# thomasdeppisch/eMagLS

Measured on AMD Instinct MI355X. Metric: eMagLS filter sets/s (N=4, 2702 dirs, 512 taps), higher is better.
Workload: dtype f64; 1 GPU; BASELINE config 3: getEMagLsFilters em32 r=4.2cm N=4 complex-SH, 2702 dirs, 512 taps, 48 kHz; one filter set per step, inputs resident in HBM; dirs=2702, taps=512, sim_order=19, bins=512, k_cut=43, designs_resident_per_gpu=128, designs_per_batch=32, batches_in_flight=4, distinct_hrir_sets_resident=20, parallelism=independent jobs per GPU, one RCCL gather

## Files before the change

emagls_amd/_lib.py:

```python
from __future__ import annotations

import ctypes as C
import os

_HERE = os.path.dirname(os.path.abspath(__file__))
LIB_PATH = os.environ.get("EMAGLS_LIB_PATH") or os.path.join(_HERE, "lib", "libemagls.so")

OK, ERR_ARG, ERR_UNSUPPORTED, ERR_HIP, ERR_NUMERIC = 0, 1, 2, 3, 4
BASIS = {"real": 0, "complex": 1}
KIND_LS, KIND_MAGLS, KIND_EMAGLS, KIND_EMAGLS2, KIND_FROM_ATF, KIND_EMA_CH, KIND_MAGLS_2D, KIND_EMA_SH = range(8)
RADIAL = {"tikhonov": 0, "softlimit": 1, "full": 2, "none": 3}
LAYOUT = {"sh": 0, "ch": 1}
MODEL = {"sh": 0, "emagls": 1, "emagls2": 2, "atf": 3, "ema_ch": 5, "ema_sh": 6}

c_dp = C.POINTER(C.c_double)
c_i64 = C.c_int64


class DesignDesc(C.Structure):
    _fields_ = [("kind", C.c_int), ("basis", C.c_int), ("order", C.c_int), ("fs", C.c_double), ("len", c_i64),
                ("nsamp", c_i64), ("ndirs", c_i64), ("mic_radius", C.c_double), ("nmics", c_i64),
                ("f_trans", C.c_double), ("atf_taps", c_i64), ("natf", c_i64), ("custom_basis", C.c_int),
                ("diffuseness", C.c_int), ("sim_order_pad", C.c_int)]

# ... 31 lines not shown
    "emagls_version": (C.c_int, []),
    "emagls_device_count": (C.c_int, [C.POINTER(C.c_int)]),
    "emagls_set_device": (C.c_int, [C.c_int]),
    "emagls_cache_clear": (C.c_int, []),
    "emagls_cache_release_designs": (C.c_int, []),
    "emagls_fp64_peak_tflops": (C.c_int, [C.c_int, C.POINTER(C.c_double)]),
    "emagls_fp64_peak_tflops_ex": (C.c_int, [C.c_int, C.c_int, C.POINTER(C.c_double), C.POINTER(C.c_double)]),
    "emagls_self_test": (C.c_int, [C.c_int, C.POINTER(C.c_double)]),
    "emagls_debug_synth_operand": (C.c_int, [C.c_void_p, C.c_int, C.c_int, C.c_void_p, c_i64, C.c_int, C.c_void_p, C.c_void_p]),
    "emagls_debug_synth_cosines": (C.c_int, [C.c_void_p, C.c_void_p, c_i64, C.c_void_p, C.c_void_p, C.c_int, C.c_void_p]),
    "emagls_debug_factor": (C.c_int, [C.POINTER(DebugFactorArgs)]),
    "emagls_debug_factor_gram": (C.c_int, [C.c_void_p, C.c_int, C.c_int, C.c_void_p, C.c_int, C.c_double, C.c_double, C.c_void_p, C.c_void_p,
                                           C.c_void_p, C.c_void_p]),
    "emagls_debug_twiddles": (C.c_int, [C.c_int, C.c_void_p]),
    "emagls_debug_filter_epilogue": (C.c_int, [C.c_void_p, C.c_int, C.c_int, C.c_int, C.c_void_p, C.c_int, C.c_int, C.c_int, C.c_int, C.c_int,
                                               C.c_double, C.c_void_p, C.c_void_p]),
    "emagls_debug_hrir_spectra": (C.c_int, [C.c_void_p, C.c_void_p, c_i64, c_i64, c_i64, C.c_void_p, C.c_int, C.c_int, C.c_int, C.c_int, C.c_void_p,
                                            c_i64, C.c_int, C.c_void_p, C.c_void_p, C.c_void_p, C.c_void_p, C.c_void_p]),
    "emagls_debug_real_spectra": (C.c_int, [C.c_void_p, c_i64, c_i64, c_i64, C.c_void_p, C.c_int, c_i64, c_i64, c_i64, C.c_void_p]),
    "emagls_sh_basis": (C.c_int, [C.c_int, c_i64, C.c_void_p, C.c_void_p, C.c_int, C.c_void_p]),
    "emagls_sh_basis_device": (C.c_int, [C.c_int, c_i64, C.c_void_p, C.c_void_p, C.c_int, C.c_void_p, C.c_void_p]),
    "emagls_modal_bn": (C.c_int, [C.c_int, c_i64, C.c_void_p, C.c_void_p]),
    "emagls_get_ls_filters": (C.c_int, [C.c_void_p, C.c_void_p, c_i64, c_i64, C.c_void_p, C.c_void_p, C.c_int, C.c_int,
                                        C.c_void_p, C.c_void_p]),
    "emagls_get_magls_filters": (C.c_int, [C.c_void_p, C.c_void_p, c_i64, c_i64, C.c_void_p, C.c_void_p, C.c_int,
                                           C.c_double, c_i64, C.c_int, C.c_void_p, C.c_void_p]),
    "emagls_get_emagls_filters": (C.c_int, [C.c_void_p, C.c_void_p, c_i64, c_i64, C.c_void_p, C.c_void_p, C.c_double,
                                            C.c_void_p, C.c_void_p, c_i64, C.c_int, C.c_double, c_i64, C.c_int,
                                            C.c_void_p, C.c_void_p]),
    "emagls_get_emagls2_filters": (C.c_int, [C.c_void_p, C.c_void_p, c_i64, c_i64, C.c_void_p, C.c_void_p, C.c_double,
                                             C.c_void_p, C.c_void_p, c_i64, C.c_int, C.c_double, c_i64, C.c_int,
                                             C.c_void_p, C.c_void_p]),
    "emagls_get_emagls_filters_ema_in_ch": (C.c_int, [C.c_void_p, C.c_void_p, c_i64, c_i64, C.c_void_p, C.c_void_p, C.c_double,
                                                      C.c_void_p, c_i64, C.c_int, C.c_double, c_i64, C.c_int, C.c_void_p, C.c_void_p]),
    "emagls_get_emagls_filters_ema_in_sh": (C.c_int, [C.c_void_p, C.c_void_p, c_i64, c_i64, C.c_void_p, C.c_void_p, C.c_double,
                                                      C.c_void_p, c_i64, C.c_int, C.c_double, c_i64, C.c_int, C.c_void_p, C.c_void_p]),
    "emagls_get_emagls_filters_from_atf": (C.c_int, [C.c_void_p, C.c_void_p, c_i64, c_i64, C.c_void_p, C.c_void_p,
                                                     C.c_void_p, c_i64, c_i64, c_i64, C.c_void_p, C.c_void_p,
                                                     C.c_double, c_i64, C.c_double, C.c_void_p, C.c_void_p,
                                                     C.POINTER(C.c_double)]),
    "emagls_simulation_order": (C.c_int, [C.c_int, C.c_int, C.c_double, C.c_double]),
    "emagls_get_ls_filters_with_basis": (C.c_int, [C.c_void_p, C.c_void_p, c_i64, c_i64, C.c_void_p, C.c_int, C.c_int, C.c_void_p, C.c_void_p]),
    "emagls_get_magls_filters_with_basis": (C.c_int, [C.c_void_p, C.c_void_p, c_i64, c_i64, C.c_void_p, C.c_int, C.c_double, c_i64, C.c_int,
                                                      C.c_void_p, C.c_void_p]),
    "emagls_get_emagls_filters_with_basis": (C.c_int, [C.c_void_p, C.c_void_p, c_i64, c_i64, C.c_void_p, C.c_double, C.c_void_p, c_i64, C.c_int,
                                                       C.c_double, c_i64, C.c_int, C.c_void_p, C.c_void_p]),
    "emagls_get_emagls2_filters_with_basis": (C.c_int, [C.c_void_p, C.c_void_p, c_i64, c_i64, C.c_void_p, C.c_double, C.c_void_p, c_i64, C.c_int,
                                                        C.c_double, c_i64, C.c_int, C.c_void_p, C.c_void_p]),
    "emagls_plan_set_basis": (C.c_int, [C.c_void_p, C.c_void_p, C.c_void_p]),
    "emagls_binaural_decode": (C.c_int, [C.c_void_p, c_i64, c_i64, C.c_void_p, C.c_void_p, c_i64, C.c_int, C.c_void_p]),
    "emagls_binaural_decode_complex": (C.c_int, [C.c_void_p, C.c_int, c_i64, c_i64, C.c_void_p, C.c_void_p, C.c_int, c_i64, C.c_int,
                                                 C.c_void_p, C.c_void_p]),
    "emagls_binaural_decode_device": (C.c_int, [C.c_void_p, C.c_int, c_i64, c_i64, C.c_void_p, C.c_void_p, C.c_int, c_i64, C.c_void_p,
                                                C.c_void_p, C.c_void_p]),
    "emagls_rotate_yaw": (C.c_int, [C.c_void_p, C.c_int, c_i64, c_i64, C.c_int, C.c_int, C.c_void_p, c_i64, C.c_void_p]),
    "emagls_binaural_decode_render": (C.c_int, [C.c_void_p, C.c_int, c_i64, c_i64, C.c_void_p, C.c_void_p, C.c_int, c_i64, C.c_int,
                                                C.c_int, C.c_int, C.c_void_p, c_i64, C.c_void_p, c_i64, C.c_void_p, C.c_void_p]),
    "emagls_binaural_decode_render_device": (C.c_int, [C.c_void_p, C.c_int, c_i64, c_i64, C.c_void_p, C.c_void_p, C.c_int, c_i64,
                                                       C.c_int, C.c_int, C.c_void_p, c_i64, C.c_void_p, c_i64, C.c_void_p, C.c_void_p,
                                                       C.c_void_p]),
    "emagls_sh_rotation_matrix": (C.c_int, [C.c_int, C.c_int, C.c_double, C.c_double, C.c_double, C.c_void_p]),
    "emagls_rotate_sh": (C.c_int, [C.c_void_p, C.c_int, c_i64, c_i64, C.c_int, C.c_void_p, c_i64, C.c_void_p, c_i64, C.c_void_p, c_i64,
                                   C.c_void_p]),
    "emagls_binaural_decode_render_ypr": (C.c_int, [C.c_void_p, C.c_int, c_i64, c_i64, C.c_void_p, C.c_void_p, C.c_int, c_i64, C.c_int,
                                                    C.c_int, C.c_int, C.c_void_p, c_i64, C.c_void_p, c_i64, C.c_void_p, c_i64,
                                                    C.c_void_p, c_i64, C.c_void_p, C.c_void_p]),
    "emagls_binaural_decode_render_ypr_device": (C.c_int, [C.c_void_p, C.c_int, c_i64, c_i64, C.c_void_p, C.c_void_p, C.c_int, c_i64,
                                                           C.c_int, C.c_int, C.c_void_p, c_i64, C.c_void_p, c_i64, C.c_void_p, c_i64,
                                                           C.c_void_p, c_i64, C.c_void_p, C.c_void_p, C.c_void_p]),
    "emagls_resample_length": (c_i64, [c_i64, c_i64, c_i64]),
    "emagls_resample": (C.c_int, [C.c_void_p, C.c_int, c_i64, c_i64, c_i64, c_i64, C.c_void_p]),
    "emagls_resample_device": (C.c_int, [C.c_void_p, C.c_int, c_i64, c_i64, c_i64, c_i64, C.c_void_p, C.c_void_p]),
    "emagls_binaural_decode_render_fs": (C.c_int, [C.c_void_p, C.c_int, c_i64, c_i64, C.c_void_p, C.c_void_p, C.c_int, c_i64, C.c_int,
                                                   C.c_int, C.c_int, C.c_void_p, c_i64, C.c_void_p, c_i64, C.c_void_p, c_i64,
                                                   C.c_void_p, c_i64, C.c_double, C.c_double, C.c_double, C.c_void_p, C.c_void_p]),
    "emagls_binaural_decode_render_fs_device": (C.c_int, [C.c_void_p, C.c_int, c_i64, c_i64, C.c_void_p, C.c_void_p, C.c_int, c_i64,
                                                          C.c_int, C.c_int, C.c_void_p, c_i64, C.c_void_p, c_i64, C.c_void_p, c_i64,
                                                          C.c_void_p, c_i64, C.c_double, C.c_double, C.c_double, C.c_void_p,
                                                          C.c_void_p, C.c_void_p]),
    "emagls_decode_stream_create": (C.c_int, [c_i64, C.c_void_p, C.c_void_p, C.c_int, c_i64, C.c_int, C.c_int, C.c_int, c_i64,
                                              C.POINTER(C.c_void_p)]),
    "emagls_decode_stream_push": (C.c_int, [C.c_void_p, C.c_void_p, c_i64, C.c_void_p, c_i64, C.c_void_p, c_i64, C.c_void_p, c_i64,
                                            C.c_void_p]),
    "emagls_decode_stream_push_device": (C.c_int, [C.c_void_p, C.c_void_p, c_i64, C.c_void_p, c_i64, C.c_void_p, c_i64, C.c_void_p, c_i64,
                                                   C.c_void_p, C.c_void_p]),
    "emagls_decode_stream_reset": (C.c_int, [C.c_void_p]),
    "emagls_decode_stream_info": (C.c_int, [C.c_void_p, C.POINTER(c_i64), C.POINTER(c_i64), C.POINTER(c_i64), C.POINTER(c_i64),
                                            C.POINTER(C.c_int)]),
    "emagls_decode_stream_destroy": (C.c_int, [C.c_void_p]),
    "emagls_decode_stream_create_bank": (C.c_int, [c_i64, c_i64, C.c_void_p, C.c_void_p, C.c_int, c_i64, C.c_int, C.c_int, C.c_int, c_i64,
                                                   C.POINTER(C.c_void_p)]),
    "emagls_decode_stream_push_sets": (C.c_int, [C.c_void_p, C.c_void_p, c_i64, C.c_void_p, c_i64, C.c_void_p, c_i64, C.c_void_p, c_i64,
                                                 C.c_void_p, c_i64, C.c_void_p]),
    "emagls_decode_stream_push_sets_device": (C.c_int, [C.c_void_p, C.c_void_p, c_i64, C.c_void_p, c_i64, C.c_void_p, c_i64, C.c_void_p,
                                                        c_i64, C.c_void_p, c_i64, C.c_void_p, C.c_void_p]),
    "emagls_decode_stream_sets": (C.c_int, [C.c_void_p, C.POINTER(c_i64)]),
    "emagls_decode_group_create": (C.c_int, [c_i64, c_i64, C.c_void_p, C.c_void_p, C.c_int, c_i64, C.c_int, C.c_int, C.c_int, c_i64, c_i64,
                                             C.POINTER(C.c_void_p)]),
    "emagls_decode_group_push": (C.c_int, [C.c_void_p, C.c_void_p, c_i64, C.c_void_p, c_i64, C.c_void_p, c_i64, C.c_void_p, c_i64,
                                           C.c_void_p, c_i64, C.c_void_p]),
    "emagls_decode_group_push_device": (C.c_int, [C.c_void_p, C.c_void_p, c_i64, C.c_void_p, c_i64, C.c_void_p, c_i64, C.c_void_p, c_i64,
                                                  C.c_void_p, c_i64, C.c_void_p, C.c_void_p]),
    "emagls_decode_group_reset": (C.c_int, [C.c_void_p, c_i64]),
    "emagls_decode_group_info": (C.c_int, [C.c_void_p, C.POINTER(c_i64), C.POINTER(c_i64), C.POINTER(c_i64), C.POINTER(c_i64),
                                           C.POINTER(c_i64), C.POINTER(C.c_int)]),
    "emagls_decode_group_destroy": (C.c_int, [C.c_void_p]),
    "emagls_decode_stream_create_encoded": (C.c_int, [c_i64, C.c_void_p, C.c_int, c_i64, c_i64, C.c_void_p, C.c_void_p, C.c_int, c_i64, C.c_int,
                                                      C.c_int, c_i64, C.POINTER(C.c_void_p)]),
    "emagls_decode_group_create_encoded": (C.c_int, [c_i64, C.c_void_p, C.c_int, c_i64, c_i64, C.c_void_p, C.c_void_p, C.c_int, c_i64, C.c_int,
                                                     C.c_int, c_i64, c_i64, C.POINTER(C.c_void_p)]),
    "emagls_field_stream_create": (C.c_int, [c_i64, c_i64, C.c_void_p, C.c_int, c_i64, c_i64, C.POINTER(C.c_void_p)]),
    "emagls_field_stream_push": (C.c_int, [C.c_void_p, C.c_void_p, c_i64, C.c_void_p]),
    "emagls_field_stream_push_device": (C.c_int, [C.c_void_p, C.c_void_p, c_i64, C.c_void_p, C.c_void_p]),
    "emagls_field_stream_reset": (C.c_int, [C.c_void_p]),
    "emagls_field_stream_info": (C.c_int, [C.c_void_p, C.POINTER(c_i64), C.POINTER(c_i64), C.POINTER(c_i64), C.POINTER(c_i64),
                                           C.POINTER(C.c_int)]),
    "emagls_field_stream_destroy": (C.c_int, [C.c_void_p]),
    "emagls_get_magls_filters_dc": (C.c_int, [C.c_void_p, C.c_void_p, c_i64, c_i64, C.c_void_p, C.c_void_p, C.c_int,
                                              C.c_double, c_i64, C.c_int, C.c_int, C.c_void_p, C.c_void_p]),
    "emagls_get_emagls_filters_dc": (C.c_int, [C.c_void_p, C.c_void_p, c_i64, c_i64, C.c_void_p, C.c_void_p, C.c_double,
                                               C.c_void_p, C.c_void_p, c_i64, C.c_int, C.c_double, c_i64, C.c_int, C.c_int,
                                               C.c_void_p, C.c_void_p]),
    "emagls_get_emagls2_filters_dc": (C.c_int, [C.c_void_p, C.c_void_p, c_i64, c_i64, C.c_void_p, C.c_void_p, C.c_double,
                                                C.c_void_p, C.c_void_p, c_i64, C.c_int, C.c_double, c_i64, C.c_int, C.c_int,
                                                C.c_void_p, C.c_void_p]),
    "emagls_get_magls_filters_2d": (C.c_int, [C.c_void_p, C.c_void_p, c_i64, c_i64, C.c_void_p, C.c_int, C.c_double, c_i64, C.c_int,
                                              C.c_void_p, C.c_void_p]),
    "emagls_get_radial_filter": (C.c_int, [C.c_int, C.c_double, C.c_double, c_i64, C.c_int, C.c_int, C.c_double, C.c_double, C.c_void_p]),
    "emagls_apply_radial_filter_rows": (c_i64, [c_i64, c_i64, C.c_int]),
    "emagls_apply_radial_filter": (C.c_int, [C.c_void_p, c_i64, C.c_int, C.c_double, C.c_double, c_i64, C.c_int, C.c_int, C.c_double,
                                             C.c_double, C.c_void_p]),
    "emagls_sh_encode": (C.c_int, [C.c_void_p, c_i64, c_i64, C.c_void_p, C.c_void_p, C.c_int, C.c_int, C.c_void_p]),
    "emagls_ch_basis": (C.c_int, [C.c_int, c_i64, C.c_void_p, C.c_int, C.c_void_p]),
    "emagls_get_smair_matrix": (C.c_int, [C.c_int, C.c_double, c_i64, C.c_int, C.c_double, C.c_void_p, C.c_void_p, c_i64, C.c_int, C.c_int,
                                          C.c_int, C.c_double, C.c_double, C.c_void_p, C.POINTER(C.c_int)]),
    "emagls_rendered_hrtfs": (C.c_int, [C.c_int, C.c_void_p, C.c_void_p, C.c_int, c_i64, c_i64, c_i64, C.c_void_p, C.c_void_p, c_i64, C.c_double,
                                        C.c_int, C.c_int, C.c_double, C.c_void_p, C.c_void_p, c_i64, C.c_void_p, c_i64, c_i64, C.c_void_p,
                                        C.c_void_p, c_i64, c_i64, C.c_void_p, C.c_void_p, C.c_void_p, C.c_void_p, C.c_void_p, C.c_void_p]),
    "emagls_eq_filter_nfft": (c_i64, [c_i64]),
    "emagls_get_magls_spherical_head_filter": (C.c_int, [C.c_double, C.c_int, C.c_double, c_i64, C.c_void_p, C.c_void_p]),
    "emagls_get_magls_array_diffuse_filter": (C.c_int, [C.c_double, C.c_void_p, C.c_void_p, c_i64, C.c_int, C.c_double, c_i64, C.c_int,
                                                        C.c_void_p, C.c_void_p]),
    "emagls_plan_create": (C.c_int, [C.POINTER(DesignDesc), C.POINTER(C.c_void_p)]),
    "emagls_plan_destroy": (C.c_int, [C.c_void_p]),
    "emagls_plan_set_hrir_grid": (C.c_int, [C.c_void_p, C.c_void_p, C.c_void_p]),
    "emagls_plan_set_mic_grid": (C.c_int, [C.c_void_p, C.c_void_p, C.c_void_p]),
    "emagls_plan_set_hrirs": (C.c_int, [C.c_void_p, C.c_void_p, C.c_void_p]),
    "emagls_plan_set_atfs": (C.c_int, [C.c_void_p, C.c_void_p, C.c_void_p, C.c_void_p]),
    "emagls_plan_execute": (C.c_int, [C.c_void_p]),
    "emagls_plan_synchronize": (C.c_int, [C.c_void_p]),
    "emagls_plan_get_filters": (C.c_int, [C.c_void_p, C.c_void_p, C.c_void_p]),
    "emagls_plan_get_info": (C.c_int, [C.c_void_p, C.POINTER(PlanInfo)]),
    "emagls_plan_sweep_form_in_batch": (C.c_int, [C.c_void_p, C.c_int, C.POINTER(C.c_int)]),
    "emagls_plan_set_profiling": (C.c_int, [C.c_void_p, C.c_int]),
    "emagls_plan_set_streams": (C.c_int, [C.c_void_p, C.c_int]),
    "emagls_plan_num_stages": (C.c_int, [C.c_void_p]),
    "emagls_plan_stage_name": (C.c_char_p, [C.c_void_p, C.c_int]),
    "emagls_plan_stage_times": (C.c_int, [C.c_void_p, c_dp, C.c_int]),
    "emagls_plan_sweep_kernel_time": (C.c_int, [C.c_void_p, c_dp, C.POINTER(C.c_int)]),
    "emagls_plan_debug_buffer": (C.c_int, [C.c_void_p, C.c_char_p, C.c_void_p, C.POINTER(C.c_size_t)]),
    "emagls_plan_stream": (C.c_void_p, [C.c_void_p]),
    "emagls_batch_create": (C.c_int, [C.POINTER(C.c_void_p), C.c_int, C.POINTER(C.c_void_p)]),
    "emagls_batch_execute": (C.c_int, [C.c_void_p]),
    "emagls_batch_synchronize": (C.c_int, [C.c_void_p]),
    "emagls_batch_get_filters": (C.c_int, [C.c_void_p, C.POINTER(C.c_void_p), C.POINTER(C.c_void_p)]),
    "emagls_batch_set_profiling": (C.c_int, [C.c_void_p, C.c_int]),
    "emagls_batch_lane_mode": (C.c_int, [C.c_void_p, C.POINTER(C.c_int)]),
    "emagls_batch_set_stream": (C.c_int, [C.c_void_p, C.c_void_p]),
    "emagls_set_batch_max": (C.c_int, [C.c_int, C.POINTER(C.c_int)]),
    "emagls_batch_shares_atf_side": (C.c_int, [C.c_void_p, C.POINTER(C.c_int)]),
    "emagls_design_hrir_sets": (C.c_int, [C.c_int, C.c_void_p, C.c_void_p, C.c_int64, C.c_int64, C.c_int64, C.c_void_p, C.c_void_p, C.c_double,
                                          C.c_void_p, C.c_void_p, C.c_int64, C.c_int, C.c_double, C.c_int64, C.c_int, C.c_void_p, C.c_void_p]),
    "emagls_from_atf_hrir_sets": (C.c_int, [C.c_void_p, C.c_void_p, C.c_int64, C.c_int64, C.c_int64, C.c_void_p, C.c_void_p, C.c_void_p, C.c_int64,
                                            C.c_int64, C.c_int64, C.c_void_p, C.c_void_p, C.c_double, C.c_int64, C.c_double, C.c_void_p, C.c_void_p,
                                            C.POINTER(C.c_double)]),
    "emagls_jobs_run": (C.c_int, [C.POINTER(Job), C.c_int64, C.c_int, C.c_int, C.c_int]),
    "emagls_design_out_shape": (C.c_int, [C.POINTER(DesignDesc), C.POINTER(c_i64), C.POINTER(c_i64), C.POINTER(C.c_int)]),
    "emagls_jobs_shard": (C.c_int, [C.POINTER(Job), C.c_int64, C.c_int, C.c_int, C.POINTER(C.c_int), C.POINTER(C.c_int), C.POINTER(C.c_int)]),
    "emagls_jobs_run_devices": (C.c_int, [C.POINTER(Job), C.c_int64, C.POINTER(C.c_int), C.c_int, C.c_int, C.c_int, C.c_int]),
    "emagls_jobs_set_profiling": (C.c_int, [C.c_int]),
    "emagls_jobs_sweep_times": (C.c_int, [C.POINTER(C.c_double), C.POINTER(C.c_int), C.c_int, C.POINTER(C.c_int)]),
    "emagls_batch_set_geometry_sharing": (C.c_int, [C.c_void_p, C.c_int]),
    "emagls_batch_shares_geometry": (C.c_int, [C.c_void_p, C.POINTER(C.c_int)]),
    "emagls_batch_geometry_runs": (C.c_int, [C.c_void_p, C.POINTER(C.c_longlong), C.POINTER(C.c_longlong)]),
    "emagls_jobs_geometry_runs": (C.c_int, [C.POINTER(C.c_longlong), C.POINTER(C.c_longlong), C.POINTER(C.c_longlong)]),
    "emagls_jobs_would_share_geometry": (C.c_int, [C.c_void_p, C.c_int, C.POINTER(C.c_int)]),
    "emagls_batch_set_side_stream": (C.c_int, [C.c_void_p, C.c_void_p]),
    "emagls_batch_set_streams": (C.c_int, [C.c_void_p, C.c_int]),
    "emagls_batch_set_stage_order": (C.c_int, [C.c_void_p, C.c_int]),
    "emagls_batch_sweep_time": (C.c_int, [C.c_void_p, C.POINTER(C.c_double)]),
    "emagls_batch_destroy": (C.c_int, [C.c_void_p]),
}


class EmaglsError(RuntimeError):
    def __init__(self, code, msg):
        super().__init__("emagls error %d: %s" % (code, msg))
        self.code = code


_lib = None


def load():
    global _lib
    if _lib is not None:
        return _lib
    if not os.path.exists(LIB_PATH):
        raise ImportError("HIP library not built: %s is missing (run `python -m emagls_amd.build`)" % LIB_PATH)
    lib = C.CDLL(LIB_PATH, mode=C.RTLD_GLOBAL)
    for name, (res, args) in SYMBOLS.items():
        fn = getattr(lib, name)
        fn.restype = res
        fn.argtypes = args
    _lib = lib
    return lib


def check(rc):
    if rc != OK:
        raise EmaglsError(rc, load().emagls_last_error().decode("utf-8", "replace"))
```

emagls_amd/csrc/batch_run.hip:

```cpp
#include "host_internal.hpp"

void emagls_batch_forget(emagls_batch* b, emagls_plan* p) {
    for (auto& q : b->plans) if (q == p) q = nullptr;
}

namespace {
void batch_sweep_stage(emagls_batch& b) {
    const int nb = (int)b.plans.size();
    std::vector<HalfSweepArgs> ha((size_t)nb);
    for (int j = 0; j < nb; ++j) ha[j] = emagls_half_args(*b.plans[j]);
    if (b.atf_share || b.geo_share)
        for (int j = 1; j < nb; ++j) {
            ha[j].G = ha[0].G; ha[j].Yri = ha[0].Yri; ha[j].Mw = ha[0].Mw; ha[j].cond_ok = ha[0].cond_ok;
            ha[j].bsc = ha[0].bsc; ha[j].smap = ha[0].smap;
            ha[j].skip_flag = ha[0].skip_flag;
        }
    const bool reg = b.plans[0]->sweep_persist && reg_sweep_wanted(b.plans.data(), nb);
    for (auto* q : b.plans) q->reg_sweep = reg;
    if (!reg && nb > SWEEP_MULTI_MAX) throw Error(EMAGLS_ERR_UNSUPPORTED, "internal: more than 16 designs in a batch need the register-resident sweep");
    HalfSweepMulti h{};
    h.n = std::min(nb, SWEEP_MULTI_MAX);
    for (int j = 0; j < h.n; ++j) h.a[j] = ha[j];
    emagls_plan& q0 = *b.plans[0];
    const int kk0 = std::max(q0.kcut0, 1);
    if (kk0 >= q0.P) return;
    if (q0.sweep_persist) {
        hipStream_t ss = b.stream;
        {
            SweepGate gate(ss, reg ? reg_sweep_gate_cost((int)q0.D, nb) : 0);
            if (b.lanes) { BatchScope sc(nb, b.stride); launch_zero(q0.get("ll"), q0.bufs["ll"].bytes, ss); }
            else for (auto* q : b.plans) launch_zero(q->get("ll"), q->bufs["ll"].bytes, ss);
            if (reg) {
                if (!b.sweep_args_dev) HIP_CHECK(hipMalloc(&b.sweep_args_dev, sizeof(HalfSweepArgs) * (size_t)REG_SWEEP_MAX));
                reg_args_upload(ha.data(), nb, b.sweep_args_dev, b.sweep_args_last, ss);
            }
            if (b.prof_level >= 1) HIP_CHECK(hipEventRecord(b.sweep_ev[0], ss));
            if (reg) launch_sweep_reg(static_cast<const HalfSweepArgs*>(b.sweep_args_dev), ha[0], nb, ss);
            else if (q0.synth) launch_sweep_synth(h, ss); else launch_sweep_persist(h, ss);
            if (b.prof_level >= 1) HIP_CHECK(hipEventRecord(b.sweep_ev[1], ss));
        }
        if (ss != b.stream) b.depend(b.stream, ss);
        return;
    }
    for (int kb = kk0; kb < q0.P; ++kb) launch_sweep_half(h, kb, b.stream);
    launch_sweep_half_finalize(h, q0.P - 1, b.stream);
}

bool batch_defers_hh(const emagls_batch& b) {
    if (!b.lanes || !(b.alone || sw_int<Sw::DEFER_HH>() == 2) || b.geo_share || b.atf_share) return false;
    for (const emagls_plan* p : b.plans) if (!p || !plan_defers_hh_route(*p)) return false;
    return true;
}
void batch_lanes_part(emagls_batch& b, int part, int first, int count, hipStream_t st, int group = 0) {
    emagls_plan& p0 = *b.plans[first];
    const int ns = (part == 0 && b.groups == 1) ? b.nstreams : 1;
    int order = 0;
    if (part == 0 && ns == 1 && sw_on<Sw::STAGGER>()) order = b.groups > 1 ? 1 + group % 2 : (b.order_hint ? 1 + (b.order_hint - 1) % 2 : 0);
    Scoped stream(p0.stream, st);
    Scoped nstreams(p0.nstreams, ns);
    Scoped stage_order(p0.stage_order, order);
    Scoped side0(p0.side[0], ns > 1 ? b.side[0] : p0.side[0]), side1(p0.side[1], ns > 1 ? b.side[1] : p0.side[1]),
        side2(p0.side[2], ns > 1 ? b.side[2] : p0.side[2]);
    Scoped pre_phase(p0.pre_phase, part == 3 ? 2 : (part == 0 && b.defer_hh) ? 1 : 0);
    BatchScope sc(count, b.stride);
    if (part == 0) plan_pre_stage(p0); else if (part == 3) emagls_pre_sweep(p0); else emagls_post_sweep(p0);
}
void mark_executed(emagls_batch& b, int launches) {
    for (auto* p : b.plans) { p->executed = true; p->sweep_launches = launches; }
}
int sweep_launch_count(const emagls_plan& p0) { return p0.sweep_persist ? 1 : p0.P - std::max(p0.kcut0, 1); }
int batch_group_first(const emagls_batch& b, int g) { const int n = (int)b.plans.size(), h = (n + b.groups - 1) / b.groups; return std::min(n, g * h); }
void batch_execute_lanes(emagls_batch& b) {
    const bool replay = b.use_graph && b.eager_runs >= 1 && !(b.groups == 1 && b.nstreams > 1);
    const int n = (int)b.plans.size();
    const int ng = b.groups;
    for (int g = 1; g < ng; ++g) if (!b.side[g - 1]) b.side[g - 1] = emagls::pool_stream_take();
    hipStream_t gs[4] = {b.stream, b.stream, b.stream, b.stream};
    for (int g = 1; g < ng; ++g) gs[g] = b.side[g - 1];
    if (!replay || !b.group[0]) b.defer_hh = batch_defers_hh(b);
    const bool defer = b.defer_hh;
    if (defer) for (int g = 0; g < ng; ++g) if (!b.hh_stream[g]) b.hh_stream[g] = emagls::pool_stream_take();
    if (replay && !b.group[0]) {
        for (int g = 0; g < ng; ++g) {
            const int f = batch_group_first(b, g), c = batch_group_first(b, g + 1) - f;
            b.group[g].capture(gs[g], [&] { batch_lanes_part(b, 0, f, c, gs[g], g); });
            if (defer) b.group_hh[g].capture(b.hh_stream[g], [&] { batch_lanes_part(b, 3, f, c, b.hh_stream[g], g); });
        }
        b.post.capture(b.stream, [&] { batch_lanes_part(b, 2, 0, n, b.stream); });
    }
    b.used = 0;
    for (int g = 1; g < ng; ++g) b.depend(gs[g], b.stream);
    if (replay && ng > 1) {
        hipError_t err[4] = {hipSuccess, hipSuccess, hipSuccess, hipSuccess};
        const int dev = b.device;
        std::vector<std::thread> th;
        for (int g = 1; g < ng; ++g)
            th.emplace_back([&, g] { err[g] = hipSetDevice(dev); if (err[g] == hipSuccess) err[g] = hipGraphLaunch(b.group[g].exec, gs[g]); });
        err[0] = hipGraphLaunch(b.group[0].exec, gs[0]);
        for (auto& t : th) t.join();
        for (int g = 0; g < ng; ++g) HIP_CHECK(err[g]);
    } else {
        for (int g = 0; g < ng; ++g) {
            const int f = batch_group_first(b, g), c = batch_group_first(b, g + 1) - f;
            if (replay) b.group[g].launch(gs[g]); else batch_lanes_part(b, 0, f, c, gs[g], g);
        }
    }
    if (defer) for (int g = 0; g < ng; ++g) b.depend(b.hh_stream[g], gs[g]);
    for (int g = 1; g < ng; ++g) b.depend(b.stream, gs[g]);
    batch_sweep_stage(b);
    if (defer) {
        for (int g = 0; g < ng; ++g) {
            const int f = batch_group_first(b, g), c = batch_group_first(b, g + 1) - f;
            if (replay) b.group_hh[g].launch(b.hh_stream[g]); else batch_lanes_part(b, 3, f, c, b.hh_stream[g], g);
            b.depend(b.stream, b.hh_stream[g]);
        }
    }
    if (replay) b.post.launch(b.stream); else batch_lanes_part(b, 2, 0, n, b.stream);
    mark_executed(b, sweep_launch_count(*b.plans[0]));
    if (!replay) ++b.eager_runs;
}

bool batch_inputs_same(emagls_batch& b, std::initializer_list<const char*> names, uint64_t& checked_version, bool& same) {
    uint64_t ver = 0;
    for (auto* p : b.plans) ver = ver * 1000003ull + p->atf_side_version;
    if (ver == checked_version) return same;
    if (!b.cmp_flag) HIP_CHECK(hipMalloc(&b.cmp_flag, 16));
    HIP_CHECK(hipStreamSynchronize(b.stream));
    HIP_CHECK(hipMemsetAsync(b.cmp_flag, 0, 16, b.stream));
    emagls_plan& p0 = *b.plans[0];
    for (size_t j = 1; j < b.plans.size(); ++j)
        for (const char* name : names) launch_compare_words(p0.get(name), b.plans[j]->get(name), p0.bufs[name].bytes, b.cmp_flag, b.stream);
    int differ = 0;
    HIP_CHECK(hipMemcpyAsync(&differ, b.cmp_flag, sizeof differ, hipMemcpyDeviceToHost, b.stream));
    HIP_CHECK(hipStreamSynchronize(b.stream));
    checked_version = ver;
    return same = differ == 0;
}
void batch_set_sharing(emagls_batch& b, bool& field, bool share) {
    if (share == field) return;
    for (auto* p : b.plans) drop_plan_graphs(*p);
    drop_batch_graphs(b);
    if (&field == &b.geo_share) batch_geo_forget(b);
    field = share;
}
void batch_run_two_graphs(emagls_batch& b, CapturedGraph& pre, void (*stage)(emagls_batch&, int), int pre_part, int launches) {
    const bool replay = b.use_graph && b.eager_runs >= 1;
    if (replay && !pre) pre.capture(b.stream, [&] { stage(b, pre_part); });
    if (replay && !b.post) b.post.capture(b.stream, [&] { stage(b, 2); });
    b.used = 0;
    if (replay) pre.launch(b.stream); else stage(b, pre_part);
    batch_sweep_stage(b);
    if (replay) b.post.launch(b.stream); else stage(b, 2);
    mark_executed(b, launches);
    if (!replay) ++b.eager_runs;
}
template <typename Pre> void batch_run_per_plan(emagls_batch& b, bool replay, Pre pre, void (*post)(emagls_plan&), int launches) {
    emagls_plan& p0 = *b.plans[0];
    if (replay && !p0.pre) {
        for (auto* p : b.plans) p->pre.capture(p->stream, [&] { pre(*p); });
        if (!p0.sweep_persist) b.group[0].capture(b.stream, [&] { batch_sweep_stage(b); });
    }
    b.used = 0;
    for (auto* p : b.plans) b.depend(p->stream, b.stream);
    for (auto* p : b.plans) {
        if (replay) p->pre.launch(p->stream); else pre(*p);
        b.depend(b.stream, p->stream);
    }
    if (b.atf_share)
        for (size_t j = 1; j < b.plans.size(); ++j) from_atf_ls_rows(*b.plans[j], p0, b.stream);
    if (p0.sweep_persist) batch_sweep_stage(b);
    else if (replay) b.group[0].launch(b.stream); else batch_sweep_stage(b);
    for (auto* p : b.plans) {
        b.depend(p->stream, b.stream);
        post(*p);
        b.depend(b.stream, p->stream);
    }
    mark_executed(b, launches);
    if (!replay) ++b.eager_runs;
}

void batch_atf_decide_sharing(emagls_batch& b) {
    const bool same = batch_inputs_same(b, {"atf", "atf_azi", "atf_zen", "hrir_azi", "hrir_zen"}, b.atf_checked_version, b.atf_inputs_same);
    bool routes_ok = true;
    for (auto* p : b.plans) routes_ok = routes_ok && p->gram_from == 1 && p->sweep_persist == b.plans[0]->sweep_persist;
    batch_set_sharing(b, b.atf_share, same && routes_ok && b.plans.size() > 1);
}
void from_atf_subject_pre_stage(emagls_plan& p) {
    subject_reset(p, p.stream);
    from_atf_subject_stage(p);
}
// ... 424 lines not shown
```

emagls_amd/csrc/capi.hip:

```cpp
#include "host_internal.hpp"

namespace {

struct CachedPlan {
    std::unique_ptr<emagls_plan> plan;
    emagls_design_desc desc{};
    int device = 0;
    bool busy = false;
    uint64_t last_use = 0;
};
std::mutex g_cache_mu;
std::vector<CachedPlan> g_cache;
uint64_t g_cache_tick = 0;

int one_shot(const emagls_design_desc& desc, const double* hL, const double* hR, const double* azi, const double* zen,
             const double* mic_azi, const double* mic_zen, const double* atf, const double* atf_azi, const double* atf_zen,
             void* wL, void* wR, double* mean_dev, const void* Y_hrir = nullptr, const void* Y_mic = nullptr) {
    return guarded([&] {
        int dev = 0;
        HIP_CHECK(hipGetDevice(&dev));
        emagls_plan* p = nullptr;
        std::unique_ptr<emagls_plan> fresh;
        bool cached = false;
        {
// ... 213 lines not shown
int emagls_modal_bn(int order, int64_t nfreq, const double* kr, void* bn) {
    return guarded([&] {
        if (order < 0 || nfreq < 0 || !kr || !bn) throw Error(EMAGLS_ERR_ARG, "invalid argument");
        if (nfreq == 0) return;
        double* d_kr = nullptr;
        void* d_bn = nullptr;
        auto cleanup = [&] { hipFree(d_kr); hipFree(d_bn); };
        try {
            HIP_CHECK(hipMalloc(&d_kr, sizeof(double) * nfreq));
            HIP_CHECK(hipMalloc(&d_bn, sizeof(cplx) * nfreq * (order + 1)));
            HIP_CHECK(hipMemcpy(d_kr, kr, sizeof(double) * nfreq, hipMemcpyDefault));
            launch_modal_bn(order, nfreq, d_kr, 1.0, 1.0, d_bn, 1, nfreq, nullptr);
            HIP_CHECK(hipDeviceSynchronize());
            HIP_CHECK(hipMemcpy(bn, d_bn, sizeof(cplx) * nfreq * (order + 1), hipMemcpyDefault));
        } catch (...) { cleanup(); throw; }
        cleanup();
    });
}

int emagls_plan_create(const emagls_design_desc* desc, emagls_plan** plan) {
    return guarded([&] {
        if (!desc || !plan) throw Error(EMAGLS_ERR_ARG, "null pointer");
        std::unique_ptr<emagls_plan> p(new emagls_plan);
        p->d = *desc;
        plan_setup(*p);
        *plan = p.release();
    });
}
int emagls_plan_destroy(emagls_plan* plan) {
    return guarded([&] {
        DeviceGuard dg(plan ? plan->device : -1);
        delete plan;
    });
}
int emagls_plan_set_hrir_grid(emagls_plan* p, const double* azi, const double* zen) {
    return guarded([&] {
        DeviceGuard dg(p ? p->device : -1);
        if (!p || !azi) throw Error(EMAGLS_ERR_ARG, "null pointer");
        std::vector<double> equator;
        if (p->d.kind == EMAGLS_KIND_MAGLS_2D) { equator.assign((size_t)p->d.ndirs, kPi / 2.0); zen = equator.data(); }
        if (!zen) throw Error(EMAGLS_ERR_ARG, "null pointer");
        p->upload("hrir_azi", azi, sizeof(double) * p->d.ndirs);
        p->upload("hrir_zen", zen, sizeof(double) * p->d.ndirs);
        HIP_CHECK(hipStreamSynchronize(p->stream));
        p->have_hrir_grid = true;
        ++p->atf_side_version;
    });
}
int emagls_plan_set_mic_grid(emagls_plan* p, const double* azi, const double* zen) {
    return guarded([&] {
        DeviceGuard dg(p ? p->device : -1);
        if (!p || !azi) throw Error(EMAGLS_ERR_ARG, "null pointer");
        if (!p->has("mic_azi")) throw Error(EMAGLS_ERR_ARG, "this design kind has no microphone grid");
        std::vector<double> equator;
        if (p->d.kind == EMAGLS_KIND_EMA_CH || p->d.kind == EMAGLS_KIND_EMA_SH) { equator.assign((size_t)p->d.nmics, kPi / 2.0); zen = equator.data(); }
        if (!zen) throw Error(EMAGLS_ERR_ARG, "null pointer");
        p->upload("mic_azi", azi, sizeof(double) * p->d.nmics);
        p->upload("mic_zen", zen, sizeof(double) * p->d.nmics);
        if (p->has("smap")) {
            int smap[34];
            synth_pairing(azi, zen, (int)p->d.nmics, smap);
            p->upload("smap", smap, sizeof smap);
            p->synth_units = smap[32] + smap[33];
            HIP_CHECK(hipStreamSynchronize(p->stream));
        }
        std::vector<double> kr(p->P);
        for (int k = 0; k < p->P; ++k) {
            const double f = (double)k * (p->d.fs / 2.0) / (double)(p->P - 1);
            kr[k] = 2.0 * kPi * f / C_SOUND * p->d.mic_radius;
        }
        p->upload("kr", kr.data(), sizeof(double) * p->P);
        HIP_CHECK(hipStreamSynchronize(p->stream));
        p->have_mic_grid = true;
        ++p->atf_side_version;
    });
}
int emagls_plan_set_basis(emagls_plan* p, const void* Y_hrir, const void* Y_mic) {
    return guarded([&] {
        DeviceGuard dg(p ? p->device : -1);
        if (!p || !Y_hrir) throw Error(EMAGLS_ERR_ARG, "null pointer");
        if (!p->custom_basis) throw Error(EMAGLS_ERR_ARG, "the plan was not created with custom_basis = 1");
        const size_t es = esz(p->cplx_basis);
        HIP_CHECK(hipMemcpy2DAsync(p->get("Ycm"), (size_t)p->ldD * es, Y_hrir, (size_t)p->D * es, (size_t)p->D * es, (size_t)p->S, hipMemcpyDefault,
                                   p->stream));
        if (array_kind(p->d.kind)) {
            if (!Y_mic) throw Error(EMAGLS_ERR_ARG, "the array designs need the SH matrix of the microphone grid too");
            p->upload("Ymic_cm", Y_mic, es * (size_t)p->S * p->d.nmics);
            std::vector<double> kr(p->P);
            for (int k = 0; k < p->P; ++k) kr[k] = 2.0 * kPi * ((double)k * (p->d.fs / 2.0) / (double)(p->P - 1)) / C_SOUND * p->d.mic_radius;
            p->upload("kr", kr.data(), sizeof(double) * p->P);
        }
        HIP_CHECK(hipStreamSynchronize(p->stream));
        p->have_basis = true;
    });
}
int emagls_plan_set_hrirs(emagls_plan* p, const double* hL, const double* hR) {
    return guarded([&] {
        DeviceGuard dg(p ? p->device : -1);
        if (!p || !hL || !hR) throw Error(EMAGLS_ERR_ARG, "null pointer");
        p->upload("hL", hL, sizeof(double) * p->d.nsamp * p->d.ndirs);
        p->upload("hR", hR, sizeof(double) * p->d.nsamp * p->d.ndirs);
        HIP_CHECK(hipStreamSynchronize(p->stream));
        p->have_hrirs = true;
    });
}
int emagls_plan_set_atfs(emagls_plan* p, const double* atf, const double* azi, const double* zen) {
    return guarded([&] {
        DeviceGuard dg(p ? p->device : -1);
        if (!p || !atf || !azi || !zen) throw Error(EMAGLS_ERR_ARG, "null pointer");
        if (!p->has("atf")) throw Error(EMAGLS_ERR_ARG, "this design kind has no ATFs");
        p->upload("atf", atf, sizeof(double) * p->d.atf_taps * p->d.nmics * p->d.natf);
        p->upload("atf_azi", azi, sizeof(double) * p->d.natf);
        p->upload("atf_zen", zen, sizeof(double) * p->d.natf);
        HIP_CHECK(hipStreamSynchronize(p->stream));
        p->have_atfs = true;
        ++p->atf_side_version;
    });
}
int emagls_plan_execute(emagls_plan* p) {
    return guarded([&] {
        DeviceGuard dg(p ? p->device : -1);
        if (!p) throw Error(EMAGLS_ERR_ARG, "null pointer");
        plan_execute(*p);
    });
}
int emagls_plan_synchronize(emagls_plan* p) {
    return guarded([&] {
        DeviceGuard dg(p ? p->device : -1);
        if (!p) throw Error(EMAGLS_ERR_ARG, "null pointer");
        HIP_CHECK(hipStreamSynchronize(p->sync_stream ? p->sync_stream : p->stream));
    });
}
int emagls_plan_get_filters(emagls_plan* p, void* wL, void* wR) {
    return guarded([&] {
        DeviceGuard dg(p ? p->device : -1);
        if (!p || !wL || !wR) throw Error(EMAGLS_ERR_ARG, "null pointer");
        if (!p->executed) throw Error(EMAGLS_ERR_ARG, "plan has not been executed");
        HIP_CHECK(hipStreamSynchronize(p->sync_stream ? p->sync_stream : p->stream));
        plan_check_flags(*p);
        const size_t bytes = (p->out_cplx ? sizeof(cplx) : sizeof(double)) * (size_t)p->out_rows * p->out_cols;
        HIP_CHECK(hipMemcpy(wL, p->get("wL"), bytes, hipMemcpyDefault));
        HIP_CHECK(hipMemcpy(wR, p->get("wR"), bytes, hipMemcpyDefault));
    });
}
int emagls_plan_sweep_form_in_batch(emagls_plan* p, int designs, int* form) {
    return guarded([&] {
        DeviceGuard dg(p ? p->device : -1);
        if (!p || !form || designs < 1 || designs > REG_SWEEP_MAX) throw Error(EMAGLS_ERR_ARG, "emagls_plan_sweep_form_in_batch: null pointer or designs outside 1..32");
        std::vector<emagls_plan*> same((size_t)designs, p);
        const bool reg = p->synth && reg_sweep_wanted(same.data(), designs);
        *form = p->d.kind == EMAGLS_KIND_LS ? 0 : (p->synth ? (reg ? 3 : 2) : (p->sweep_persist ? 1 : 0));
    });
}
int emagls_plan_get_info(emagls_plan* p, emagls_plan_info* info) {
    return guarded([&] {
        DeviceGuard dg(p ? p->device : -1);
        if (!p || !info) throw Error(EMAGLS_ERR_ARG, "null pointer");
        std::memset(info, 0, sizeof *info);
        info->nfft = p->nfft; info->num_pos_freqs = p->P; info->k_cut = p->k_cut; info->sim_order = p->simOrder;
        info->num_sh_sim = p->S; info->num_channels = p->C; info->out_is_complex = p->out_cplx;
        info->out_rows = p->out_rows; info->out_cols = p->out_cols; info->num_sweep_launches = p->sweep_launches;
        info->device_bytes = p->total_bytes;
        info->gram_from = p->gram_from; info->hh_end = p->hh_end; info->hh_orders = p->n_h + 1; info->g_first = p->g0;
        info->sim_order_own = array_kind(p->d.kind) ? p->simOrderOwn : p->simOrder;
        bool reg = false;
        if (p->synth) {
            bool whole = p->owner != nullptr;
            if (whole) for (auto* q : p->owner->plans) whole = whole && q != nullptr;
            reg = whole ? reg_sweep_wanted(p->owner->plans.data(), (int)p->owner->plans.size()) : reg_sweep_wanted(&p, 1);
        }
        info->sweep_form = p->d.kind == EMAGLS_KIND_LS ? 0 : (p->synth ? (reg ? 3 : 2) : (p->sweep_persist ? 1 : 0));
        info->sweep_units = p->synth ? p->synth_units : 0;
        if (p->executed) {
            HIP_CHECK(hipStreamSynchronize(p->stream));
            double g[2];
            HIP_CHECK(hipMemcpy(g, p->get("grpd"), sizeof g, hipMemcpyDeviceToHost));
            info->grp_delay_l = g[0]; info->grp_delay_r = g[1];
            if (p->has("mean_dev")) HIP_CHECK(hipMemcpy(&info->mean_grid_dev_deg, p->get("mean_dev"), sizeof(double), hipMemcpyDeviceToHost));
        }
    });
}
int emagls_plan_set_profiling(emagls_plan* p, int level) {
    return guarded([&] {
        DeviceGuard dg(p ? p->device : -1);
        if (!p) throw Error(EMAGLS_ERR_ARG, "null pointer");
        p->prof_level = level;
    });
}
int emagls_plan_set_streams(emagls_plan* p, int nstreams) {
    return guarded([&] {
        DeviceGuard dg(p ? p->device : -1);
        if (!p) throw Error(EMAGLS_ERR_ARG, "null pointer");
        if (nstreams < 1 || nstreams > 4) throw Error(EMAGLS_ERR_ARG, "nstreams must be 1..4");
        HIP_CHECK(hipStreamSynchronize(p->stream));
        drop_plan_graphs(*p);
        p->nstreams = nstreams;
    });
}
int emagls_plan_num_stages(emagls_plan* p) { return p ? (int)p->stage_names.size() : 0; }
const char* emagls_plan_stage_name(emagls_plan* p, int i) {
    if (!p || i < 0 || i >= (int)p->stage_names.size()) return "";
    return p->stage_names[i].c_str();
}
int emagls_plan_stage_times(emagls_plan* p, double* ms, int n) {
    return guarded([&] {
        DeviceGuard dg(p ? p->device : -1);
        if (!p || !ms) throw Error(EMAGLS_ERR_ARG, "null pointer");
        HIP_CHECK(hipStreamSynchronize(p->stream));
        const int ns = (int)p->stage_names.size();
        for (int i = 0; i < n; ++i) {
            ms[i] = 0.0;
            if (i >= 1 && i < ns) {
                float t = 0.f;
                HIP_CHECK(hipEventElapsedTime(&t, p->stage_events[i - 1], p->stage_events[i]));
                ms[i] = t;
            }
        }
    });
}
int emagls_plan_sweep_kernel_time(emagls_plan* p, double* total_ms, int* launches) {
    return guarded([&] {
        DeviceGuard dg(p ? p->device : -1);
        if (!p || !total_ms || !launches) throw Error(EMAGLS_ERR_ARG, "null pointer");
        HIP_CHECK(hipStreamSynchronize(p->stream));
        double tot = 0.0;
        int n = 0;
        if (p->prof_level >= 2) {
            for (int i = 0; i < p->sweep_launches && 2 * (size_t)i + 1 < p->sweep_events.size(); ++i) {
                float t = 0.f;
                HIP_CHECK(hipEventElapsedTime(&t, p->sweep_events[2 * i], p->sweep_events[2 * i + 1]));
                tot += t;
                ++n;
            }
        }
        *total_ms = tot;
        *launches = n;
    });
}
int emagls_plan_debug_buffer(emagls_plan* p, const char* name, void* dst, size_t* nbytes) {
    return guarded([&] {
        DeviceGuard dg(p ? p->device : -1);
        if (!p || !name || !nbytes) throw Error(EMAGLS_ERR_ARG, "null pointer");
        auto it = p->bufs.find(name);
        if (it == p->bufs.end()) throw Error(EMAGLS_ERR_ARG, std::string("unknown buffer ") + name);
        if (!dst) { *nbytes = it->second.bytes; return; }
        HIP_CHECK(hipStreamSynchronize(p->stream));
        const size_t n = std::min(*nbytes, it->second.bytes);
        HIP_CHECK(hipMemcpy(dst, it->second.p, n, hipMemcpyDeviceToHost));
        *nbytes = n;
    });
}
void* emagls_plan_stream(emagls_plan* p) { return p ? (void*)p->stream : nullptr; }

int emagls_batch_create(emagls_plan** plans, int nplans, emagls_batch** batch) {
    return guarded([&] {
        if (!plans || !batch || nplans < 1) throw Error(EMAGLS_ERR_ARG, "invalid argument");
        const int batch_max = std::max(g_batch_max.load(), g_batch_max_override);
        if (nplans > batch_max)
            throw Error(EMAGLS_ERR_UNSUPPORTED, batch_max >= REG_SWEEP_MAX ? "at most 32 designs per batch"
                                                                             : "at most 8 designs per batch (emagls_set_batch_max(16) / EMAGLS_BATCH_MAX=16 allows 16)");
        std::unique_ptr<emagls_batch> b(new emagls_batch);
        for (int j = 0; j < nplans; ++j) {
            emagls_plan* p = plans[j];
            if (!p) throw Error(EMAGLS_ERR_ARG, "null plan");
            if (!array_kind(p->d.kind) && p->d.kind != EMAGLS_KIND_FROM_ATF && !magls_kind(p->d.kind) && p->d.kind != EMAGLS_KIND_LS)
                throw Error(EMAGLS_ERR_UNSUPPORTED, "batches take eMagLS / eMagLS2 / EMAinCH / EMAinSH plans, LS / MagLS / MagLS-2D plans, or FromAtf plans "
                                                    "(subjects of one ATF set)");
            if ((p->d.kind == EMAGLS_KIND_LS) != (plans[0]->d.kind == EMAGLS_KIND_LS) ||
                (p->d.kind == EMAGLS_KIND_LS && (p->cplx_basis != plans[0]->cplx_basis || p->d.order != plans[0]->d.order || p->d.nsamp != plans[0]->d.nsamp)))
                throw Error(EMAGLS_ERR_ARG, "LS plans share a batch only with LS plans of the same order, basis and HRIR length");
            if ((p->d.kind == EMAGLS_KIND_FROM_ATF) != (plans[0]->d.kind == EMAGLS_KIND_FROM_ATF))
                throw Error(EMAGLS_ERR_ARG, "FromAtf plans cannot share a batch with array designs");
            if (magls_kind(p->d.kind) != magls_kind(plans[0]->d.kind) || (magls_kind(p->d.kind) && p->d.kind != plans[0]->d.kind))
                throw Error(EMAGLS_ERR_ARG, "MagLS plans share a batch only with MagLS plans of the same kind");
            if (magls_kind(p->d.kind) && (p->diffuse != plans[0]->diffuse || p->cplx_basis != plans[0]->cplx_basis || p->d.order != plans[0]->d.order))
                throw Error(EMAGLS_ERR_ARG, "all designs of a batch must have the same shape (order, basis, constraint)");
            if (p->wide) throw Error(EMAGLS_ERR_UNSUPPORTED, "designs with more than 32 channels run one at a time");
            if (p->owner) throw Error(EMAGLS_ERR_ARG, "a plan belongs to another batch (destroy that batch first)");
            if (p->device != plans[0]->device) throw Error(EMAGLS_ERR_ARG, "the plans of a batch must live on one device");
            for (int i = 0; i < j; ++i) if (plans[i] == p) throw Error(EMAGLS_ERR_ARG, "the same plan appears twice in the batch");
            const emagls_plan* q = plans[0];
            if (p->P != q->P || p->kcut0 != q->kcut0 || p->C != q->C || p->nWG_dense != q->nWG_dense || p->D != q->D || p->sweep_persist != q->sweep_persist ||
                p->Dm != q->Dm || p->d.natf != q->d.natf || p->d.atf_taps != q->d.atf_taps || p->d.len != q->d.len)
                throw Error(EMAGLS_ERR_ARG, "all designs of a batch must have the same shape (directions, channels, bins, k_cut)");
            b->plans.push_back(p);
        }
        b->device = b->plans[0]->device;
        DeviceGuard dg(b->device);
        b->stream = StreamPool::get().take();
        b->use_graph = !sw_on<Sw::NO_GRAPH>();
        const bool array_batch = b->plans[0]->d.kind != EMAGLS_KIND_FROM_ATF && !magls_kind(b->plans[0]->d.kind) && b->plans[0]->d.kind != EMAGLS_KIND_LS;
        for (auto* p : b->plans) HIP_CHECK(hipStreamSynchronize(p->stream));
        trace_mark("batch create: plans synchronised");
        if (array_batch) batch_unify_synth(*b);
        trace_mark("batch create: sweep form unified");
        batch_decide_residency(*b);
        trace_mark("batch create: residency decided");
        if (nplans > SWEEP_MULTI_MAX && !(b->plans[0]->synth && b->plans[0]->sweep_persist && reg_sweep_wanted(b->plans.data(), nplans)))
            throw Error(EMAGLS_ERR_UNSUPPORTED, "more than 16 designs per batch: only array designs that take the register-resident sweep (built-in SH basis, "
                                                "microphone grids set, at most 18 antipodal pairs + single microphones, a launch the device can hold)");
        for (auto* p : b->plans) {
            p->nstreams = 1;
            p->prof_level = 0;
            p->sync_stream = b->stream;
            p->owner = b.get();
        }
// ... 338 lines not shown
```

emagls_amd/csrc/host_internal.hpp:

```cpp
#pragma once
#include <atomic>
#include <chrono>
#include <cstdlib>
#include <cstring>
#include <deque>
#include <map>
#include <memory>
#include <mutex>
#include <shared_mutex>
#include <string>
#include <thread>
#include <utility>
#include <vector>

#include "../../include/emagls.h"
#include "kernels.hpp"

using namespace emagls;

struct emagls_batch;
void emagls_batch_forget(emagls_batch* b, emagls_plan* p);

namespace emagls {

// ... 203 lines not shown
    int64_t out_rows = 0, out_cols = 0;
    int nWG = 0, nWG_dense = 0;
    bool gram_route = true;
    int gram_from = 0, gram_floor = 0, hh_end = 0, n_h = 0, S_h = 0, ldS_h = 0, g0 = 0, nb_gram = 0;
    int nh_floor = 0;
    bool persist_suspended = false;
    bool sweep_persist = true;
    bool synth_want = false, synth = false;
    int synth_units = 0;
    bool reg_sweep = false;
    std::vector<char> sweep_args_last;
    bool synth_block = false;
    const emagls_plan* geo_from = nullptr;
    emagls_batch* owner = nullptr;
    bool have_hrir_grid = false, have_mic_grid = false, have_hrirs = false, have_atfs = false, have_basis = false;
    uint64_t atf_side_version = 0;
    bool diffuse = false;
    bool custom_basis = false;
    bool wide = false;
    int prof_level = 0;
    std::vector<std::string> stage_names;
    std::vector<hipEvent_t> stage_events;
    std::vector<double> stage_ms;
    std::vector<hipEvent_t> sweep_events;
    int sweep_launches = 0;
    bool executed = false;
    CapturedGraph graph;
    int eager_runs = 0;
    bool use_graph = true;
    CapturedGraph pre;
    int nstreams = 1;
    int stage_order = 0;
    int pre_phase = 0;
    bool geo_keep = false;
    bool geo_skip = false;
    uint64_t geo_done_version = ~0ull;
    uint64_t geo_run_version = ~0ull;
    uint64_t solo_runs = 0;
    bool defer_hh = false;
    bool alone = false;
    hipStream_t hh_stream = nullptr;
    hipStream_t sync_stream = nullptr;
    hipStream_t side[3] = {nullptr, nullptr, nullptr};
    bool owns_stream = true;
    void need_sides(int n) { for (int i = 0; i < n - 1 && i < 3; ++i) if (!side[i]) side[i] = StreamPool::get().take(); }
    std::vector<hipEvent_t> sync_events;
    size_t sync_used = 0;
    hipEvent_t next_sync_event() {
        if (sync_used == sync_events.size()) {
            hipEvent_t e;
            HIP_CHECK(hipEventCreateWithFlags(&e, hipEventDisableTiming));
            sync_events.push_back(e);
        }
        return sync_events[sync_used++];
    }
    void depend(hipStream_t waiter, hipStream_t signaller) {
        if (waiter == signaller) return;
        hipEvent_t e = next_sync_event();
        HIP_CHECK(hipEventRecord(e, signaller));
        HIP_CHECK(hipStreamWaitEvent(waiter, e, 0));
    }

    ~emagls_plan() {
        if (owner) emagls_batch_forget(owner, this);
        if (stream) hipStreamSynchronize(stream);
        for (auto st : side) if (st) hipStreamSynchronize(st);
        if (hh_stream) hipStreamSynchronize(hh_stream);
        (void)hipGetLastError();
        for (auto& kv : bufs) if (kv.second.p && kv.second.owned) hipFree(kv.second.p);
        release_slabs();
        for (auto e : stage_events) hipEventDestroy(e);
        for (auto e : sweep_events) hipEventDestroy(e);
        for (auto e : sync_events) hipEventDestroy(e);
        for (auto st : side) StreamPool::get().give(st);
        StreamPool::get().give(hh_stream);
        if (owns_stream) StreamPool::get().give(stream);
    }
    void* alloc(const std::string& name, size_t bytes, bool zero = true) {
        if (bytes == 0) bytes = 16;
        auto it = bufs.find(name);
        if (it != bufs.end()) {
            if (it->second.bytes >= bytes) {
                total_bytes -= (int64_t)(it->second.bytes - bytes);
                it->second.bytes = bytes;
                return it->second.p;
            }
            if (it->second.owned) HIP_CHECK(hipFree(it->second.p));
            total_bytes -= (int64_t)it->second.bytes;
        }
        DevBuf b;
        b.p = slab_take((bytes + 15) / 16 * 16);
        b.bytes = bytes;
        b.owned = false;
        if (zero && !slab_zeroed) HIP_CHECK(hipMemsetAsync(b.p, 0, bytes, stream));
        bufs[name] = b;
        total_bytes += (int64_t)bytes;
        return b.p;
    }
    template <typename T = void> T* get(const std::string& name) {
        auto it = bufs.find(name);
        if (it == bufs.end()) throw Error(EMAGLS_ERR_ARG, "internal: unknown buffer " + name);
        return reinterpret_cast<T*>(it->second.p);
    }
    bool has(const std::string& name) const { return bufs.count(name) != 0; }
    void upload(const std::string& name, const void* src, size_t bytes) {
        auto it = bufs.find(name);
        if (it == bufs.end() || it->second.bytes < bytes) throw Error(EMAGLS_ERR_ARG, "internal: upload size mismatch for " + name);
        HIP_CHECK(hipMemcpyAsync(it->second.p, src, bytes, hipMemcpyDefault, stream));
    }
    void mark(const char* name) {
        if (prof_level < 1) return;
        const size_t i = stage_names.size();
        stage_names.push_back(name);
        if (stage_events.size() <= i) {
            hipEvent_t e;
            HIP_CHECK(hipEventCreate(&e));
            stage_events.push_back(e);
        }
        HIP_CHECK(hipEventRecord(stage_events[i], stream));
    }
};

struct emagls_batch {
    std::vector<emagls_plan*> plans;
    int device = -1;
    bool lanes = false;
    size_t stride = 0;
    hipStream_t stream = nullptr;
    bool own_stream = true;
    bool atf = false, atf_share = false, atf_inputs_same = false;
    uint64_t atf_checked_version = ~0ull;
    bool magls = false;
    bool geo_want = false, geo_share = false, geo_inputs_same = false;
    uint64_t geo_checked_version = ~0ull;
    uint64_t geo_kept_version = ~0ull;
    uint64_t geo_ran_version = ~0ull;
    bool geo_cold_pending = false;
    CapturedGraph warm;
    int last_form = 0;
    long long geo_cold_runs = 0, geo_warm_runs = 0;
    int* cmp_flag = nullptr;
    int nstreams = 1;
    hipStream_t side[3] = {nullptr, nullptr, nullptr};
    CapturedGraph group[4];
    int prof_level = 0;
    hipEvent_t sweep_ev[2] = {nullptr, nullptr};
    CapturedGraph post;
    bool side0_external = false;
    int order_hint = 0;
    int groups = 1;
    CapturedGraph group_hh[4];
    hipStream_t hh_stream[4] = {nullptr, nullptr, nullptr, nullptr};
    bool defer_hh = false;
    bool alone = true;
    int eager_runs = 0;
    bool use_graph = true;
    void* sweep_args_dev = nullptr;
    std::vector<char> sweep_args_last;
    std::vector<hipEvent_t> events;
    size_t used = 0;
    hipEvent_t next_event() {
        if (used == events.size()) {
            hipEvent_t e;
            HIP_CHECK(hipEventCreateWithFlags(&e, hipEventDisableTiming));
            events.push_back(e);
        }
        return events[used++];
    }
    void depend(hipStream_t waiter, hipStream_t signaller) {
        hipEvent_t e = next_event();
        HIP_CHECK(hipEventRecord(e, signaller));
        HIP_CHECK(hipStreamWaitEvent(waiter, e, 0));
    }
    ~emagls_batch() {
        if (stream) hipStreamSynchronize(stream);
        for (auto e : events) hipEventDestroy(e);
        for (int i = 0; i < 4; ++i)
            if (hh_stream[i]) { hipStreamSynchronize(hh_stream[i]); emagls::pool_stream_give(hh_stream[i]); }
        for (auto e : sweep_ev) if (e) hipEventDestroy(e);
        if (stream && own_stream) emagls::pool_stream_give(stream);
        for (int i = 0; i < 3; ++i) if (side[i] && !(i == 0 && side0_external)) { hipStreamSynchronize(side[i]); emagls::pool_stream_give(side[i]); }
        if (cmp_flag) hipFree(cmp_flag);
        if (sweep_args_dev) hipFree(sweep_args_dev);
        for (auto* p : plans) if (p) { p->sync_stream = nullptr; p->owner = nullptr; }
    }
};

namespace emagls {

struct StreamLoan {
    const std::vector<emagls_plan*>& plans;
    std::vector<hipStream_t> keep;
    StreamLoan(const std::vector<emagls_plan*>& ps, hipStream_t st) : plans(ps) {
        keep.reserve(ps.size());
        for (auto* p : ps) { keep.push_back(p->stream); p->stream = st; }
    }
    StreamLoan(const StreamLoan&) = delete;
    StreamLoan& operator=(const StreamLoan&) = delete;
    ~StreamLoan() { for (size_t j = 0; j < keep.size(); ++j) plans[j]->stream = keep[j]; }
};

template <typename F> int guarded(F&& f) {
    return guarded_call([&] { f(); });
}

constexpr double GRAM_COND_EST = 3.0e3;

inline bool forks_streams(const emagls_plan& p) { return p.nstreams >= 2; }

extern thread_local hipStream_t g_plan_stream_shared;
void plan_routes(emagls_plan& p);
void synth_pairing(const double* azi, const double* zen, int M, int* smap);
void plan_alloc_routes(emagls_plan& p);
void plan_setup(emagls_plan& p);

void stage_prologue(emagls_plan& p, int mode, const int64_t* didx, int64_t Dh);
void execute_ls(emagls_plan& p);
void magls_post_sweep(emagls_plan& p);
bool plan_defers_hh_route(const emagls_plan& p);
void hrir_spectra(emagls_plan& h, const emagls_plan& g, hipStream_t st);
FactorArgs hh_factor_args(emagls_plan& h, emagls_plan& g, int* sweeps_out, double* cond_ok);
void hrir_hh_rows(emagls_plan& h, emagls_plan& g, hipStream_t st);
void hrir_hh_back(const FactorArgs& fa, const emagls_plan& g, hipStream_t st);
void hrir_gram_ls_rows(emagls_plan& h, emagls_plan& g, const emagls_plan& src, bool lanes_share, hipStream_t st);
void subject_reset(emagls_plan& p, hipStream_t st);
void emagls_pre_sweep(emagls_plan& p);
HalfSweepArgs emagls_half_args(emagls_plan& p);
struct SweepGate {
    struct Entry { hipEvent_t ev; int slots; };
    struct State { std::deque<Entry> inflight; std::vector<hipEvent_t> pool; int capacity = 0; };
    static std::mutex& mutex();
    static State& state();
    std::unique_lock<std::mutex> lock;
    hipStream_t st;
    int slots;
    SweepGate(hipStream_t s, int slots_per_xcd);
    ~SweepGate();
};
bool reg_sweep_wanted(emagls_plan* const* plans, int n);
void reg_args_upload(const HalfSweepArgs* host, int n, void* dev, std::vector<char>& last, hipStream_t st);
void emagls_post_sweep(emagls_plan& p);
void from_atf_subject_stage(emagls_plan& p);
void from_atf_ls_rows(emagls_plan& p, emagls_plan& sh, hipStream_t st);
void from_atf_post_sweep(emagls_plan& p);
void plan_pre_stage(emagls_plan& p);
void plan_execute(emagls_plan& p);
void drop_plan_graphs(emagls_plan& p);
bool plan_recover(emagls_plan& p, const int* flag, bool apply);
void throw_fatal_flags(const int* flag);

void batch_geo_forget(emagls_batch& b);
bool batch_geo_next_is_warm(const emagls_batch& b);
void batch_execute(emagls_batch& b);
void drop_batch_graphs(emagls_batch& b);
void batch_unify_synth(emagls_batch& b);
void batch_decide_residency(emagls_batch& b);
void batch_try_lanes(emagls_batch& b);
void batch_redo(emagls_batch& b, const std::vector<int>& flags);
void plan_check_flags(emagls_plan& p);

bool same_desc(const emagls_design_desc& a, const emagls_design_desc& b);
extern thread_local int g_batch_max_override;

}
```

emagls_amd/csrc/jobs.hip:

```cpp
#include "host_internal.hpp"

extern "C" {

namespace {
struct SetsCache {
    emagls_design_desc desc{};
    int device = -1, n = 0;
    std::vector<emagls_plan*> plans;
    emagls_batch* batch = nullptr;
    std::vector<double> grid[4];
    void release() {
        for (auto& g : grid) g.clear();
        if (batch) { emagls_batch_destroy(batch); batch = nullptr; }
        for (auto* p : plans) emagls_plan_destroy(p);
        plans.clear();
        n = 0; device = -1;
    }
};
std::mutex g_sets_mu;
SetsCache g_sets[3];
}
void emagls_sets_cache_clear_internal() {
    std::lock_guard<std::mutex> lk(g_sets_mu);
    for (auto& c : g_sets) c.release();
// ... 18 lines not shown
        Pending pend[3];
        size_t out_bytes = 0;
        auto collect = [&](Pending& q) {
            if (!q.c) return;
            SetsCache* c = q.c;
            q.c = nullptr;
            const int n = c->n;
            if (n == 1 || !c->batch) {
                for (int j = 0; j < n; ++j)
                    req(emagls_plan_get_filters(c->plans[(size_t)j], (char*)wL + (q.first + j) * out_bytes, (char*)wR + (q.first + j) * out_bytes));
            } else {
                std::vector<void*> pl((size_t)n), pr((size_t)n);
                for (int j = 0; j < n; ++j) { pl[(size_t)j] = (char*)wL + (q.first + j) * out_bytes; pr[(size_t)j] = (char*)wR + (q.first + j) * out_bytes; }
                req(emagls_batch_get_filters(c->batch, pl.data(), pr.data()));
            }
        };
        try {
            int64_t k = 0;
            for (int64_t first = 0; first < nsets; ++k) {
                const bool wide_kind = ((kind == EMAGLS_KIND_MAGLS_2D || kind == EMAGLS_KIND_EMA_CH) ? 2 * order + 1 : kind == EMAGLS_KIND_EMAGLS2 ? (int)nmics : (order + 1) * (order + 1)) > 32;
                const int chunk_max = wide_kind ? ((kind == EMAGLS_KIND_EMAGLS || kind == EMAGLS_KIND_EMAGLS2) ? 1 : 4) : kind == EMAGLS_KIND_EMA_SH ? 4 : SWEEP_MULTI_MAX;
                const int n = (int)std::min<int64_t>(chunk_max, nsets - first);
                const int slot = n == chunk_max ? (int)(k % 2) : 2;
                SetsCache* c = &g_sets[slot];
                collect(pend[slot]);
                if (!(c->n == n && c->device == dev && same_desc(c->desc, d))) {
                    c->release();
                    try {
                        for (int j = 0; j < n; ++j) {
                            emagls_plan* p = nullptr;
                            req(emagls_plan_create(&d, &p));
                            p->geo_keep = true;
                            c->plans.push_back(p);
                        }
                        if (n > 1 && !c->plans[0]->wide && kind != EMAGLS_KIND_EMA_SH) {
                            int r;
                            { Scoped limit(g_batch_max_override, SWEEP_MULTI_MAX); r = emagls_batch_create(c->plans.data(), n, &c->batch); }
                            req(r);
                            req(emagls_batch_set_geometry_sharing(c->batch, 1));
                        }
                    } catch (...) { c->release(); throw; }
                    c->desc = d; c->device = dev; c->n = n;
                }
                auto same = [](const std::vector<double>& have, const double* now, size_t cnt) {
                    return now ? (have.size() == cnt && std::memcmp(have.data(), now, cnt * sizeof(double)) == 0) : have.empty();
                };
                const bool hgrid_same = same(c->grid[0], hrir_azi, (size_t)ndirs) && same(c->grid[1], hrir_zen, (size_t)ndirs) && !c->grid[0].empty();
                const bool mgrid_same = !arr || (same(c->grid[2], mic_azi, (size_t)nmics) && same(c->grid[3], mic_zen, (size_t)nmics) && !c->grid[2].empty());
                for (int j = 0; j < n; ++j) {
                    emagls_plan* p = c->plans[(size_t)j];
                    if (!hgrid_same) req(emagls_plan_set_hrir_grid(p, hrir_azi, hrir_zen));
                    if (arr && !mgrid_same) req(emagls_plan_set_mic_grid(p, mic_azi, mic_zen));
                    req(emagls_plan_set_hrirs(p, hL + (first + j) * nsamp * ndirs, hR + (first + j) * nsamp * ndirs));
                }
                auto keep = [](std::vector<double>& dst, const double* src, size_t cnt) { if (src) dst.assign(src, src + cnt); else dst.clear(); };
                keep(c->grid[0], hrir_azi, (size_t)ndirs); keep(c->grid[1], hrir_zen, (size_t)ndirs);
                if (arr) { keep(c->grid[2], mic_azi, (size_t)nmics); keep(c->grid[3], mic_zen, (size_t)nmics); }
                emagls_plan_info info;
                req(emagls_plan_get_info(c->plans[0], &info));
                out_bytes = (info.out_is_complex ? sizeof(cplx) : sizeof(double)) * (size_t)info.out_rows * info.out_cols;
                if (n > 1 && c->batch) req(emagls_batch_execute(c->batch));
                else for (int j = 0; j < n; ++j) req(emagls_plan_execute(c->plans[(size_t)j]));
                pend[slot].c = c;
                pend[slot].first = first;
                first += n;
            }
            for (auto& q : pend) collect(q);
        } catch (...) {
            for (auto& c : g_sets) c.release();
            throw;
        }
    });
}

namespace {
std::mutex g_atfsets_mu;
SetsCache g_atfsets[2];
}
void emagls_atfsets_cache_clear_internal() {
    std::lock_guard<std::mutex> lk(g_atfsets_mu);
    for (auto& c : g_atfsets) c.release();
}

namespace {
struct JobSlot {
    std::string key;
    std::string shape;
    int device = -1;
    std::vector<emagls_plan*> plans;
    emagls_batch* batch = nullptr;
    std::vector<std::vector<double>> grids;
    uint64_t last_use = 0, last_call = 0;
    int runs = 0;
    hipStream_t stream = nullptr;
    ~JobSlot() {
        if (batch) emagls_batch_destroy(batch);
        for (auto* p : plans) emagls_plan_destroy(p);
        if (stream) emagls::pool_stream_give(stream);
    }
};
std::mutex g_jobs_mu;
std::vector<std::unique_ptr<JobSlot>> g_jobs_free;
std::atomic<int> g_jobs_prof{0};
std::shared_timed_mutex g_jobs_warm_mu;
uint64_t g_jobs_tick = 0;
std::atomic<size_t> g_jobs_resident_max{8 * REG_SWEEP_MAX};

void check_rc(int rc) { if (rc != EMAGLS_OK) throw Error(rc, g_last_error); }
bool is_device_pointer(const void* p) {
    hipPointerAttribute_t at{};
    if (!p || hipPointerGetAttributes(&at, p) != hipSuccess) { (void)hipGetLastError(); return false; }
    return at.type == hipMemoryTypeDevice;
}
void job_shape(const emagls_design_desc& d, std::string& out) {
    emagls_design_desc k = d;
    if (array_kind(d.kind) && d.sim_order_pad > 0) {
        const int own = std::max(d.kind == EMAGLS_KIND_EMAGLS2 ? SMAIR_DEFAULT_ORDER : d.order, (int)std::ceil(d.fs * kPi * d.mic_radius / C_SOUND));
        if (own <= d.sim_order_pad) k.mic_radius = 0.0;
    }
    out.assign(reinterpret_cast<const char*>(&k), sizeof k);
}
bool slot_will_capture(const JobSlot& s) {
    if (s.batch) {
        const emagls_batch& b = *s.batch;
        if (!b.use_graph || b.eager_runs < 1) return false;
        if (b.geo_share && !b.atf && !b.magls) return !b.post || !(batch_geo_next_is_warm(b) ? b.warm : b.group[0]);
        return !b.group[0] && !(b.plans.size() && b.plans[0]->pre);
    }
    for (const emagls_plan* p : s.plans)
        if (p->use_graph && p->prof_level == 0 && p->eager_runs >= 1 && !p->pre && !p->graph) return true;
    return false;
}
std::atomic<long long> g_jobs_geo_runs[3];
bool jobs_chunk_shares_geometry(const emagls_job* jobs, int n) {
    if (!jobs || n < 2) return false;
    const emagls_design_desc& d0 = jobs[0].desc;
    if (d0.kind != EMAGLS_KIND_EMAGLS && d0.kind != EMAGLS_KIND_EMAGLS2 && d0.kind != EMAGLS_KIND_EMA_CH) return false;
    if (d0.custom_basis || d0.diffuseness || d0.ndirs <= 0 || d0.nmics <= 0) return false;
    const int64_t ch = d0.kind == EMAGLS_KIND_EMAGLS2 ? d0.nmics : d0.kind == EMAGLS_KIND_EMA_CH ? 2 * (int64_t)d0.order + 1 : (int64_t)(d0.order + 1) * (d0.order + 1);
    if (ch > 32) return false;
    auto same = [](const double* a, const double* b, int64_t m) {
        if (a == b) return true;
        return a && b && memcmp(a, b, sizeof(double) * (size_t)m) == 0;
    };
    if (!jobs[0].hrir_azi || !jobs[0].mic_azi) return false;
    for (int j = 1; j < n; ++j) {
        const emagls_job& x = jobs[j];
        if (memcmp(&x.desc, &d0, sizeof d0) != 0) return false;
        if (!same(x.hrir_azi, jobs[0].hrir_azi, d0.ndirs) || !same(x.hrir_zen, jobs[0].hrir_zen, d0.ndirs) ||
            !same(x.mic_azi, jobs[0].mic_azi, d0.nmics) || !same(x.mic_zen, jobs[0].mic_zen, d0.nmics)) return false;
    }
    return true;
}
void jobs_run_chunk(const emagls_job* jobs, int n, int device, int flags, bool solo, uint64_t call) {
    DeviceGuard dg(device);
    const bool trace = sw_on<Sw::JOBS_TRACE>();
    const auto t_begin = std::chrono::steady_clock::now();
    auto lap = [&](const char* what) {
        if (trace) fprintf(stderr, "emagls jobs: chunk of %d, %s at %.3f ms\n", n, what,
                           std::chrono::duration<double, std::milli>(std::chrono::steady_clock::now() - t_begin).count());
    };
    std::string key(solo ? "S" : "P"), shape(solo ? "S" : "P"), one;
    for (int j = 0; j < n; ++j) {
        key.append(reinterpret_cast<const char*>(&jobs[j].desc), sizeof(emagls_design_desc));
        job_shape(jobs[j].desc, one);
        shape.append(one);
    }
    std::unique_ptr<JobSlot> slot, recycled;
    {
        std::lock_guard<std::mutex> lk(g_jobs_mu);
        for (size_t i = 0; i < g_jobs_free.size(); ++i)
            if (g_jobs_free[i]->device == device && g_jobs_free[i]->key == key) { slot = std::move(g_jobs_free[i]); g_jobs_free.erase(g_jobs_free.begin() + i); break; }
        if (!slot)
            for (size_t i = 0; i < g_jobs_free.size(); ++i)
                if (g_jobs_free[i]->device == device && g_jobs_free[i]->shape == shape && g_jobs_free[i]->last_call != call) {
                    recycled = std::move(g_jobs_free[i]); g_jobs_free.erase(g_jobs_free.begin() + i); break;
                }
    }
    recycled.reset();
    const bool was_resident = slot != nullptr;
    std::shared_lock<std::shared_timed_mutex> shared(g_jobs_warm_mu, std::defer_lock);
    std::unique_lock<std::shared_timed_mutex> alone(g_jobs_warm_mu, std::defer_lock);
    shared.lock();
    if (!slot) {
        slot.reset(new JobSlot);
        slot->key = key; slot->shape = shape; slot->device = device;
        slot->grids.resize((size_t)n);
        slot->stream = emagls::pool_stream_take();
        struct SharedStream { SharedStream(hipStream_t st) { g_plan_stream_shared = st; } ~SharedStream() { g_plan_stream_shared = nullptr; } } shared_stream(slot->stream);
        for (int j = 0; j < n; ++j) {
            emagls_plan* p = nullptr;
            check_rc(emagls_plan_create(&jobs[j].desc, &p));
            slot->plans.push_back(p);
            if (j == 0) lap("first plan created");
        }
        lap("plans created");
    }
    for (int j = 0; j < n; ++j) {
        const emagls_job& jb = jobs[j];
        emagls_plan* p = slot->plans[(size_t)j];
        const emagls_design_desc& d = jb.desc;
        std::vector<double> g;
        auto app = [&](const double* a, int64_t m) { if (a) g.insert(g.end(), a, a + m); else g.push_back(-1e300); };
        const bool has_mics = array_kind(d.kind);
        app(jb.hrir_azi, d.ndirs); app(jb.hrir_zen, d.ndirs);
        if (has_mics) { app(jb.mic_azi, d.nmics); app(jb.mic_zen, d.nmics); }
        if (g != slot->grids[(size_t)j]) {
            if (!jb.hrir_azi) throw Error(EMAGLS_ERR_ARG, "job without an HRIR grid");
            check_rc(emagls_plan_set_hrir_grid(p, jb.hrir_azi, jb.hrir_zen));
            if (has_mics) {
                if (!jb.mic_azi) throw Error(EMAGLS_ERR_ARG, "array design without a microphone grid");
                check_rc(emagls_plan_set_mic_grid(p, jb.mic_azi, jb.mic_zen));
            }
            slot->grids[(size_t)j] = std::move(g);
        }
        if (d.kind == EMAGLS_KIND_FROM_ATF) {
            if (!jb.atf || !jb.atf_azi || !jb.atf_zen) throw Error(EMAGLS_ERR_ARG, "FromAtf job without its ATF set");
            check_rc(emagls_plan_set_atfs(p, jb.atf, jb.atf_azi, jb.atf_zen));
        }
        if (!jb.hL || !jb.hR || !jb.wL || !jb.wR) throw Error(EMAGLS_ERR_ARG, "job without HRIRs or without room for its filters");
        if (!slot->batch && n > 1 && !slot->runs) check_rc(emagls_plan_set_hrirs(p, jb.hL, jb.hR));
    }
    lap("inputs set");
    if (n > 1 && !slot->batch && !slot->runs) {
        int rc;
        { Scoped limit(g_batch_max_override, REG_SWEEP_MAX); rc = emagls_batch_create(slot->plans.data(), n, &slot->batch); }
        if (rc != EMAGLS_OK && rc != EMAGLS_ERR_UNSUPPORTED) check_rc(rc);
        if (rc != EMAGLS_OK) slot->batch = nullptr;
        if (slot->batch && solo && slot->batch->lanes) {
            if (const int fork = sw_int<Sw::JOBS_FORK>(); fork >= 2) {
                if (slot->batch->groups != 1) { HIP_CHECK(hipStreamSynchronize(slot->batch->stream)); drop_batch_graphs(*slot->batch); slot->batch->groups = 1; }
                check_rc(emagls_batch_set_streams(slot->batch, fork));
            }
        }
        if (slot->batch) {
            slot->batch->alone = solo;
            if (!solo && slot->batch->group[0]) { HIP_CHECK(hipStreamSynchronize(slot->batch->stream)); drop_batch_graphs(*slot->batch); }
        }
        lap("batch created");
    } else if (slot->batch) {
        bool gathered = false;
        if (2 * n <= 64) {
            bool all_dev = true;
            for (int j = 0; j < n && all_dev; ++j) all_dev = is_device_pointer(jobs[j].hL) && is_device_pointer(jobs[j].hR);
            if (all_dev) {
                LanePtrs src{}, dst{};
                const emagls_plan& q0 = *slot->plans[0];
                const size_t bytes = sizeof(double) * (size_t)q0.d.nsamp * (size_t)q0.d.ndirs;
                for (int j = 0; j < n; ++j) {
                    emagls_plan& q = *slot->plans[(size_t)j];
                    src.p[2 * j] = const_cast<double*>(jobs[j].hL); src.p[2 * j + 1] = const_cast<double*>(jobs[j].hR);
                    dst.p[2 * j] = q.get("hL"); dst.p[2 * j + 1] = q.get("hR");
                    q.have_hrirs = true;
                }
                launch_gather_buffers(src, dst, 2 * n, bytes, slot->batch->stream);
                gathered = true;
            }
        }
        for (int j = 0; j < n && !gathered; ++j) {
            emagls_plan& q = *slot->plans[(size_t)j];
            const size_t bytes = sizeof(double) * (size_t)q.d.nsamp * (size_t)q.d.ndirs;
            int src = -1;
            for (int i = 0; i < j && src < 0; ++i)
                if (jobs[i].hL == jobs[j].hL && jobs[i].hR == jobs[j].hR && slot->plans[(size_t)i]->d.nsamp == q.d.nsamp && slot->plans[(size_t)i]->d.ndirs == q.d.ndirs) src = i;
            const void* sl = src >= 0 ? slot->plans[(size_t)src]->get("hL") : jobs[j].hL;
            const void* sr = src >= 0 ? slot->plans[(size_t)src]->get("hR") : jobs[j].hR;
            HIP_CHECK(hipMemcpyAsync(q.get("hL"), sl, bytes, hipMemcpyDefault, slot->batch->stream));
            HIP_CHECK(hipMemcpyAsync(q.get("hR"), sr, bytes, hipMemcpyDefault, slot->batch->stream));
            q.have_hrirs = true;
        }
    } else {
        for (int j = 0; j < n; ++j) check_rc(emagls_plan_set_hrirs(slot->plans[(size_t)j], jobs[j].hL, jobs[j].hR));
    }
    if (slot->batch) {
        const int kind = jobs[0].desc.kind;
        bool want = false;
        if (flags & EMAGLS_JOBS_SHARE_GEOMETRY) want = kind != EMAGLS_KIND_FROM_ATF && kind != EMAGLS_KIND_EMA_SH;
        else if (sw_on<Sw::JOBS_AUTO_SHARE>() && !(flags & EMAGLS_JOBS_INDEPENDENT)) want = jobs_chunk_shares_geometry(jobs, n);
        if (want != slot->batch->geo_want) check_rc(emagls_batch_set_geometry_sharing(slot->batch, want ? 1 : 0));
    }
    if (!slot->batch) for (auto* q : slot->plans) q->geo_keep = (flags & EMAGLS_JOBS_SHARE_GEOMETRY) != 0;
    const bool capturing = was_resident && slot_will_capture(*slot);
    {
        if (slot->batch) {
            std::vector<void*> wl((size_t)n), wr((size_t)n);
            for (int j = 0; j < n; ++j) { wl[(size_t)j] = jobs[j].wL; wr[(size_t)j] = jobs[j].wR; }
            if (slot->batch->prof_level != g_jobs_prof.load()) check_rc(emagls_batch_set_profiling(slot->batch, g_jobs_prof.load()));
            if (capturing) { shared.unlock(); alone.lock(); }
            check_rc(emagls_batch_execute(slot->batch));
            if (capturing) { alone.unlock(); shared.lock(); }
            ++g_jobs_geo_runs[slot->batch->last_form];
            check_rc(emagls_batch_get_filters(slot->batch, wl.data(), wr.data()));
        } else {
            ++g_jobs_geo_runs[0];
            if (capturing) { shared.unlock(); alone.lock(); }
            for (int j = 0; j < n; ++j) check_rc(emagls_plan_execute(slot->plans[(size_t)j]));
            if (capturing) { alone.unlock(); shared.lock(); }
            for (int j = 0; j < n; ++j) check_rc(emagls_plan_get_filters(slot->plans[(size_t)j], jobs[j].wL, jobs[j].wR));
        }
        ++slot->runs;
    }
    lap("executed and collected");
    std::lock_guard<std::mutex> lk(g_jobs_mu);
    slot->last_use = ++g_jobs_tick;
    slot->last_call = call;
    g_jobs_free.push_back(std::move(slot));
    size_t resident = 0;
    for (auto& f : g_jobs_free) resident += f->plans.size();
    while (resident > g_jobs_resident_max.load() && g_jobs_free.size() > 1) {
        size_t old = 0;
        for (size_t i = 1; i < g_jobs_free.size(); ++i) if (g_jobs_free[i]->last_use < g_jobs_free[old]->last_use) old = i;
        resident -= g_jobs_free[old]->plans.size();
        g_jobs_free.erase(g_jobs_free.begin() + old);
    }
}
}
void emagls_jobs_cache_clear_internal() {
    std::lock_guard<std::mutex> lk(g_jobs_mu);
    g_jobs_free.clear();
    for (auto& c : g_jobs_geo_runs) c.store(0);
}
int emagls_jobs_geometry_runs(long long* independent, long long* cold, long long* warm) {
    return guarded([&] {
        if (!independent || !cold || !warm) throw Error(EMAGLS_ERR_ARG, "null pointer");
        *independent = g_jobs_geo_runs[0].load(); *cold = g_jobs_geo_runs[1].load(); *warm = g_jobs_geo_runs[2].load();
    });
}
int emagls_jobs_would_share_geometry(const emagls_job* jobs, int njobs, int* share) {
    return guarded([&] {
        if (!jobs || !share || njobs < 0) throw Error(EMAGLS_ERR_ARG, "invalid argument");
        *share = jobs_chunk_shares_geometry(jobs, njobs) ? 1 : 0;
    });
}

int emagls_jobs_set_profiling(int level) {
    return guarded([&] { g_jobs_prof.store(level > 0 ? 1 : 0); });
}
int emagls_jobs_sweep_times(double* ms, int* designs, int capacity, int* count) {
    return guarded([&] {
        if (!count || capacity < 0 || (capacity > 0 && (!ms || !designs))) throw Error(EMAGLS_ERR_ARG, "invalid argument");
        std::lock_guard<std::mutex> lk(g_jobs_mu);
        int n = 0;
        for (auto& f : g_jobs_free) {
            if (!f->batch || f->batch->prof_level < 1 || !f->batch->sweep_ev[0] || f->batch->eager_runs < 1) continue;
            if (n < capacity) {
                DeviceGuard dg(f->device);
                float t = 0.f;
                if (hipEventElapsedTime(&t, f->batch->sweep_ev[0], f->batch->sweep_ev[1]) != hipSuccess) { (void)hipGetLastError(); continue; }
                ms[n] = t; designs[n] = (int)f->plans.size();
            }
            ++n;
        }
        *count = n;
    });
}

int emagls_jobs_run(const emagls_job* jobs, int64_t njobs, int batch_size, int in_flight, int flags) {
    return guarded([&] {
        if (!jobs || njobs < 0) throw Error(EMAGLS_ERR_ARG, "invalid argument");
        if (njobs == 0) return;
        if (batch_size <= 0) batch_size = REG_SWEEP_MAX;
        if (in_flight <= 0) in_flight = 4;
        batch_size = std::min(batch_size, REG_SWEEP_MAX);
        g_jobs_resident_max.store(std::max((size_t)8 * REG_SWEEP_MAX, (size_t)2 * batch_size * (size_t)in_flight));
        if (const int v = sw_int<Sw::JOBS_RESIDENT>(); v > 0) g_jobs_resident_max.store((size_t)v);
        int device = 0;
        HIP_CHECK(hipGetDevice(&device));
        std::vector<std::pair<int64_t, int>> chunks;
        for (int64_t first = 0; first < njobs;) {
            std::string shape, other;
            job_shape(jobs[first].desc, shape);
            int cap = array_kind(jobs[first].desc.kind) && !jobs[first].desc.custom_basis && !jobs[first].desc.diffuseness ? batch_size
                                                                                                                            : std::min(batch_size, SWEEP_MULTI_MAX);
            {
                const emagls_design_desc& d0 = jobs[first].desc;
                const int64_t ch = d0.kind == EMAGLS_KIND_EMAGLS2 ? d0.nmics : (int64_t)(d0.order + 1) * (d0.order + 1);
                if ((flags & EMAGLS_JOBS_SHARE_GEOMETRY) && (d0.kind == EMAGLS_KIND_EMAGLS || d0.kind == EMAGLS_KIND_EMAGLS2) && ch > 32) cap = 1;
            }
            int n = 1;
            while (first + n < njobs && n < cap && (job_shape(jobs[first + n].desc, other), other == shape)) ++n;
            chunks.emplace_back(first, n);
            first += n;
        }
        static std::atomic<uint64_t> g_jobs_call{0};
        const uint64_t call = ++g_jobs_call;
        std::atomic<size_t> next{0};
        std::mutex err_mu;
        int err_code = EMAGLS_OK;
        std::string err_msg;
        auto work = [&] {
            for (;;) {
                const size_t c = next.fetch_add(1);
                if (c >= chunks.size()) return;
                {
                    std::lock_guard<std::mutex> lk(err_mu);
                    if (err_code != EMAGLS_OK) return;
                }
                try {
                    try {
                        jobs_run_chunk(jobs + chunks[c].first, chunks[c].second, device, flags, chunks.size() == 1, call);
                    } catch (const Error& e) {
                        if (chunks[c].second <= SWEEP_MULTI_MAX || e.code != EMAGLS_ERR_UNSUPPORTED || !strstr(e.what(), "more than 16 designs")) throw;
                        const int h = (chunks[c].second + 1) / 2;
                        jobs_run_chunk(jobs + chunks[c].first, h, device, flags, false, call);
                        jobs_run_chunk(jobs + chunks[c].first + h, chunks[c].second - h, device, flags, false, call);
                    }
                } catch (const Error& e) {
                    std::lock_guard<std::mutex> lk(err_mu);
                    if (err_code == EMAGLS_OK) { err_code = e.code; err_msg = e.what(); }
                } catch (const std::exception& e) {
                    std::lock_guard<std::mutex> lk(err_mu);
                    if (err_code == EMAGLS_OK) { err_code = EMAGLS_ERR_HIP; err_msg = e.what(); }
                }
            }
        };
        const int nthreads = (int)std::min<size_t>((size_t)in_flight, chunks.size());
        std::vector<std::thread> th;
        for (int t = 1; t < nthreads; ++t) th.emplace_back(work);
        work();
        for (auto& t : th) t.join();
        if (err_code != EMAGLS_OK) throw Error(err_code, err_msg);
    });
}
namespace {
double shard_batch_cost(int n, int sim_order) {
    const double S = (double)(sim_order + 1) * (sim_order + 1), g = n / 8.0;
    if (sim_order < 19) return 5.6 + 7.2 * g;
    return (6.4 + 2.4 * g) + (1.67 + 1.93 * g) * 1e-3 * S;
}
std::vector<std::pair<int, int>> shard_padded_batches(const std::vector<int>& so_sorted, int max_batch) {
    const int n = (int)so_sorted.size();
    const int nb = (n + max_batch - 1) / max_batch;
    std::vector<std::pair<int, int>> out;
    if (nb <= 1) { out.emplace_back(0, n); return out; }
    auto cut = [&](double T, std::vector<std::pair<int, int>>& chunks) {
        chunks.clear();
        int pos = 0;
        while (pos < n) {
            if (shard_batch_cost(1, so_sorted[pos]) > T) return false;
            int size = 1;
            while (pos + size < n && size < 32 && shard_batch_cost(size + 1, so_sorted[pos + size]) <= T) ++size;
            chunks.emplace_back(pos, size);
            pos += size;
        }
        return true;
    };
    double lo = 0.0, hi = shard_batch_cost(32, so_sorted.back()) + 1.0;
    std::vector<std::pair<int, int>> c;
    for (int it = 0; it < 40; ++it) {
        const double mid = 0.5 * (lo + hi);
        if (cut(mid, c) && (int)c.size() <= nb) hi = mid; else lo = mid;
    }
    cut(hi, out);
    return out;
}
struct ShardUnit { std::vector<int> jobs; int pad = 0; double cost = 1.0; };
void shard_units(const emagls_job* jobs, int64_t njobs, int max_batch, std::vector<ShardUnit>& units) {
    std::map<std::string, std::vector<int>> fam;
    std::vector<std::string> fam_order;
    for (int64_t j = 0; j < njobs; ++j) {
        emagls_design_desc k = jobs[j].desc;
        const bool radius_family = (k.kind == EMAGLS_KIND_EMAGLS || k.kind == EMAGLS_KIND_EMAGLS2 || k.kind == EMAGLS_KIND_EMA_CH) && !k.custom_basis && k.nmics <= 32;
        if (radius_family) { k.mic_radius = 0.0; k.sim_order_pad = 0; }
        std::string key(reinterpret_cast<const char*>(&k), sizeof k);
        key.push_back(radius_family ? 'R' : 'E');
        if (!fam.count(key)) fam_order.push_back(key);
        fam[key].push_back((int)j);
    }
    for (const std::string& key : fam_order) {
        const std::vector<int>& idx = fam[key];
        if (key.back() == 'R' && idx.size() > 1) {
            std::vector<int> order(idx.size());
            for (size_t i = 0; i < idx.size(); ++i) order[i] = (int)i;
            auto so_of = [&](int i) { const emagls_design_desc& d = jobs[idx[(size_t)i]].desc; return emagls_simulation_order(d.kind, d.order, d.fs, d.mic_radius); };
            std::stable_sort(order.begin(), order.end(), [&](int a, int b) { return so_of(a) < so_of(b); });
            std::vector<int> so_sorted(order.size());
            for (size_t i = 0; i < order.size(); ++i) so_sorted[i] = so_of(order[i]);
            if (so_sorted.front() == so_sorted.back()) {
                for (int j : idx) { ShardUnit u; u.jobs.push_back(j); u.cost = 1.0; units.push_back(std::move(u)); }
                continue;
            }
            for (auto& fs : shard_padded_batches(so_sorted, max_batch)) {
                ShardUnit u;
                for (int i = fs.first; i < fs.first + fs.second; ++i) { u.jobs.push_back(idx[(size_t)order[(size_t)i]]); u.pad = std::max(u.pad, so_sorted[(size_t)i]); }
                u.cost = shard_batch_cost((int)u.jobs.size(), u.pad);
                units.push_back(std::move(u));
            }
        } else {
            for (int j : idx) { ShardUnit u; u.jobs.push_back(j); u.cost = 1.0; units.push_back(std::move(u)); }
        }
    }
}
}

int emagls_jobs_shard(const emagls_job* jobs, int64_t njobs, int world, int max_batch, int* rank_of_job, int* order_in_rank, int* sim_order_pad) {
    return guarded([&] {
        if (!jobs || njobs < 0 || world < 1 || !rank_of_job) throw Error(EMAGLS_ERR_ARG, "invalid argument");
        if (max_batch <= 0) max_batch = 16;
        if (max_batch > 32) throw Error(EMAGLS_ERR_ARG, "a batch holds 1..32 designs");
        std::vector<ShardUnit> units;
        shard_units(jobs, njobs, max_batch, units);
        std::vector<int> by_cost(units.size());
        for (size_t i = 0; i < units.size(); ++i) by_cost[i] = (int)i;
        std::stable_sort(by_cost.begin(), by_cost.end(), [&](int a, int b) { return units[(size_t)a].cost > units[(size_t)b].cost; });
        std::vector<double> load((size_t)world, 0.0);
        std::vector<std::vector<int>> mine((size_t)world);
        for (int u : by_cost) {
            int r = 0;
            for (int q = 1; q < world; ++q) if (load[(size_t)q] < load[(size_t)r]) r = q;
            mine[(size_t)r].push_back(u);
            load[(size_t)r] += units[(size_t)u].cost;
        }
        for (int r = 0; r < world; ++r) {
            std::stable_sort(mine[(size_t)r].begin(), mine[(size_t)r].end(), [&](int a, int b) {
                return units[(size_t)a].cost < units[(size_t)b].cost || (units[(size_t)a].cost == units[(size_t)b].cost && a < b); });
            int pos = 0;
            for (int u : mine[(size_t)r])
                for (int j : units[(size_t)u].jobs) {
                    rank_of_job[j] = r;
                    if (order_in_rank) order_in_rank[j] = pos;
                    if (sim_order_pad) sim_order_pad[j] = units[(size_t)u].pad;
                    ++pos;
                }
        }
    });
}

int emagls_jobs_run_devices(const emagls_job* jobs, int64_t njobs, const int* devices, int ndevices, int batch_size, int in_flight, int flags) {
    return guarded([&] {
        if (!jobs || njobs < 0 || !devices || ndevices < 1) throw Error(EMAGLS_ERR_ARG, "invalid argument");
        int avail = 0;
        HIP_CHECK(hipGetDeviceCount(&avail));
        for (int i = 0; i < ndevices; ++i) if (devices[i] < 0 || devices[i] >= avail) throw Error(EMAGLS_ERR_ARG, "no such device");
        if (njobs == 0) return;
        std::vector<int> rank((size_t)njobs), pos((size_t)njobs), pad((size_t)njobs);
        check_rc(emagls_jobs_shard(jobs, njobs, ndevices, std::min(batch_size > 0 ? batch_size : 16, 16), rank.data(), pos.data(), pad.data()));
        std::vector<std::vector<emagls_job>> share((size_t)ndevices);
        for (int r = 0; r < ndevices; ++r) {
            int64_t cnt = 0;
            for (int64_t j = 0; j < njobs; ++j) cnt += rank[(size_t)j] == r;
            share[(size_t)r].resize((size_t)cnt);
        }
        for (int64_t j = 0; j < njobs; ++j) {
            emagls_job jb = jobs[j];
            if (pad[(size_t)j] > 0 && jb.desc.sim_order_pad == 0) jb.desc.sim_order_pad = pad[(size_t)j];
            share[(size_t)rank[(size_t)j]][(size_t)pos[(size_t)j]] = jb;
        }
        std::vector<int> rc((size_t)ndevices, EMAGLS_OK);
        std::vector<std::string> msg((size_t)ndevices);
        auto work = [&](int r) {
            if (share[(size_t)r].empty()) return;
            if (hipSetDevice(devices[r]) != hipSuccess) { rc[(size_t)r] = EMAGLS_ERR_HIP; msg[(size_t)r] = "hipSetDevice failed"; return; }
            rc[(size_t)r] = emagls_jobs_run(share[(size_t)r].data(), (int64_t)share[(size_t)r].size(), batch_size > 0 ? batch_size : 32, in_flight, flags);
            if (rc[(size_t)r] != EMAGLS_OK) msg[(size_t)r] = g_last_error;
        };
        std::vector<std::thread> th;
        for (int r = 1; r < ndevices; ++r) th.emplace_back(work, r);
        int keep = 0;
// ... 78 lines not shown
```

emagls_amd/csrc/kernels.hpp:

```cpp
#pragma once
#include <algorithm>
#include <functional>

#include "common.hpp"

namespace emagls {

void launch_zero(void* p, size_t bytes, hipStream_t st);
void launch_compare_words(const void* a, const void* b, size_t bytes, int* differ, hipStream_t st);
void launch_broadcast_lanes(const void* src, size_t bytes, size_t stride, int nlanes, hipStream_t st);
struct LanePtrs { void* p[64]; };
void launch_scatter_lanes(const void* srcL, const void* srcR, size_t stride, size_t bytes, int n, const LanePtrs& dst, hipStream_t st);
void launch_gather_buffers(const LanePtrs& src, const LanePtrs& dst, int nbuf, size_t bytes, hipStream_t st);
struct BufferMoves { const void* src[96]; void* dst[96]; size_t bytes[96]; int n; };
void launch_move_buffers(const BufferMoves& m, hipStream_t st);
void launch_ch_basis(int N, int M, const double* azi, bool cplx_basis, void* out, int ld, hipStream_t st, bool out_real = false);
void launch_sh_coeff(int N, double* tab, hipStream_t st);
inline size_t esz(bool c) { return c ? sizeof(cplx) : sizeof(double); }
inline size_t sh_coeff_count(int N) { return (size_t)2 * (N + 1) * (N + 1) + 2 * (N + 1); }
void launch_sh_basis(int N, int64_t D, const double* azi, const double* zen, const double* tab, bool cplx_basis,
                     void* Y, int64_t ld, hipStream_t st);
void launch_transpose_conj(const void* Y, int64_t D, int64_t S, int64_t ldY, void* Yt, int64_t Dpad, int64_t ldYt,
                           bool is_cplx, bool conj_it, hipStream_t st);

void launch_modal_bn(int N, int64_t nfreq, const double* kr, double kr_scale, double out_scale, void* bn,
                     int64_t stride_k, int64_t stride_n, hipStream_t st, const int* n_valid = nullptr);

void launch_twiddles(int nfft, void* tw, hipStream_t st);
int hrir_dirsum_chunks(int64_t D);
void launch_hrir_grpdelay(const double* hL, const double* hR, int64_t L, int64_t D, int nfft, const void* tw,
                          double* partial, double* grpd, hipStream_t st);
void launch_hrir_fft(const double* hL, const double* hR, int64_t L, int64_t D, const int64_t* didx, int nfft,
                     const void* tw, const double* grpd, int mode, int n_c, int kabs0, void* Hc, double* Habs,
                     int64_t ldD, hipStream_t st, double* HcT = nullptr, int ldT = 0);
void launch_real_fft_gather(const double* x, int64_t L, int64_t ncols, const int64_t* colidx, int nfft, const void* tw,
                            void* out, int64_t ldo, int64_t inner, int64_t ld_inner, hipStream_t st);
void launch_filter_epilogue(const void* W, int C, int nfft, int len, const void* tw, const double* grpd, int conj_mode,
                            int dc_rule, int shift_mode, int out_cplx, void* outL, void* outR, hipStream_t st, int n_ears = 2,
                            double fade_rel = 0.15);
void twiddles_debug(int nfft, void* tw);
void filter_epilogue_debug(const void* W, int C, int nfft, int len, const double* grpd, int conj_mode, int dc_rule, int shift_mode, int out_cplx,
                           int n_ears, double fade_rel, void* outL, void* outR);
void hrir_spectra_debug(const double* hL, const double* hR, int64_t L, int64_t D_src, int64_t D, const int64_t* didx, int nfft, int mode, int n_c, int kabs0,
                        const double* grpd_in, int64_t ldD, int ldT, double* grpd_out, void* phs, void* Hc, double* Habs, double* HcT);
void real_spectra_debug(const double* x, int64_t L, int64_t ncols_src, int64_t ncols, const int64_t* colidx, int nfft, int64_t ldo, int64_t inner,
                        int64_t ld_inner, void* out);

int gram_ksplit(int64_t D, int S);
int64_t gram_dpad(int64_t D, int S);
void launch_gram(const void* Yc, int64_t D, int S, int64_t ld, bool is_cplx, void* Gp, void* G, void* R, int Sh, hipStream_t st);
void launch_cholesky(void* G, int S, bool is_cplx, int* flag, hipStream_t st);
void launch_qform(const void* Yc, const void* R, void* Rinv, int S, int64_t D, int64_t ld, bool is_cplx, void* Q, hipStream_t st);
void launch_zsolve_flagged(void* Z, int ldS, const void* R, const void* Rinv, const double* cond_ok, int S, int C, int P, int k0,
                           hipStream_t st);
void launch_tn(const void* R, const void* E, int S, int C, int ldE, int nOrders, bool is_cplx, void* Tn, int64_t ldS,
               hipStream_t st);
void launch_small_gemm(const void* A, int lda, bool a_cplx, const void* B, int ldb, bool b_cplx, void* Cm, int ldc,
                       bool c_cplx, int M, int N, int K, hipStream_t st);

void launch_magls_m(const void* R, int C, bool is_cplx, int P, void* Mw, double* cond_ok, int* status, hipStream_t st);

struct FactorArgs;
void launch_factor(const FactorArgs& a, int nbins, bool tn_cplx, hipStream_t st, int phases = 3);
void launch_factor_jacobi_gram(const FactorArgs& a, int nbins, hipStream_t st);

void launch_gram_kmat(const void* Gy, const void* E, int S, int ldE, int C, int nOrd, bool is_cplx, void* F, int64_t ldF, double* Kmat, int ldK,
                      hipStream_t st);
void launch_gram_gemm(const void* bn, int nOrd, int P, int kb0, int nbins, double* Cf, int ldC, const double* Kmat, int ldK, int C, double* Apk,
                      int ldA, hipStream_t st);
void launch_gram_solve(const double* Apk, int ldA, int C, int kb0, int nbins, double reg_c, void* Mw, void* R2w, double* sv, int* route,
                       int* sweeps_out, hipStream_t st);
size_t hy_mfma_workspace_doubles(int n_c, int S, bool y_cplx);
int hy_mfma_kpad(int D);
void launch_hy_conj_mfma(const double* HcT, int ldT, int n_c, const void* Yc, int64_t ldY, bool y_cplx, int D, int S, double* Pw, void* out,
                         int ldS, hipStream_t st);
void launch_ls_gram(const void* Hc, int64_t ldH, int n_c, const void* G, int64_t g_stride, int64_t ldD, const void* Mw, int D, int C, int P,
                    int kb_lo, int kb_hi, void* W, hipStream_t st);

struct DenseSweepArgs;
struct HalfSweepArgs;
struct HalfSweepMulti;
void launch_sweep_dense(const DenseSweepArgs& a, int kb, bool x_cplx, hipStream_t st);
int dense_sweep_nwg(int D, int C);
void launch_sweep_half(const HalfSweepMulti& m, int kb, hipStream_t st);
void launch_sweep_half_finalize(const HalfSweepMulti& m, int kb_last, hipStream_t st);
int persist_sweep_nwg(int D);
bool persist_sweep_supported(int D, int C);
size_t persist_sweep_ll_bytes(int D, int C);
void launch_sweep_persist(const HalfSweepMulti& m, hipStream_t st);
int persist_sweep_dpw(int D);
int sweep_cu_budget();
bool persist_sweep_fits(int D, int C, int ndesigns);
bool synth_sweep_fits(int D, int nmics, int nOrd, int ndesigns);
bool synth_sweep_supported(int D, int nmics, int nOrd);
int synth_nord_pad(int nOrd);
void launch_synth_prepare(const void* bn, int nOrd, int P, void* bsc, const void* Zlo, int ldZ, int nOut, int M, const int* smap, double* Pm, hipStream_t st);
void launch_synth_mt(const void* Mw, const double* Pm, int nOut, int M, int k0, int P, const void* W, void* Mt, void* Winit, hipStream_t st);
void launch_synth_winit(const void* W, const void* Pm, int nOut, int M, int k0, int P, void* Winit, hipStream_t st, bool shared_geometry);
void launch_synth_rows(const void* U, int nchunks, const void* Pm, const void* Mw, int nOut, int M, int k_lo, int k_hi, int P, void* W, hipStream_t st,
                       bool shared_geometry = false);
int synth_ls_chunks(int D);
void launch_synth_ls(const void* Hc, int64_t ldH, int n_c, const void* bsc, int nord_pad, const double* dir_azi, const double* dir_zen, const double* mic_azi,
                     const double* mic_zen, const int* smap, int D, int M, int P, int kb_lo, int kb_hi, void* Upart, hipStream_t st, bool shared_geometry = false);
void launch_sweep_synth(const HalfSweepMulti& m, hipStream_t st);
void synth_cosines_debug(const double* dir_azi, const double* dir_zen, int64_t ndirs, const double* mic_azi, const double* mic_zen, int nmics, double* x2);
void synth_operand_debug(const void* bsc, int nbins, int nord_pad, const double* x, int64_t nx, int gs, void* g_plus, void* g_minus);
int reg_sweep_max_units();
bool reg_sweep_supported(int D, int nmics, int nunits, int nOrd);
size_t reg_sweep_ll_bytes(int D, int nmics);
int reg_sweep_capacity(int D);
int reg_sweep_slots_per_xcd();
int reg_sweep_pick_waves(int D, int ndesigns);
int reg_sweep_gate_cost(int D, int ndesigns);
bool reg_sweep_fits(int D, int nmics, int nunits, int nOrd, int ndesigns);
void launch_sweep_reg(const HalfSweepArgs* args_dev, const HalfSweepArgs& a0, int n, hipStream_t st);
double reg_contract_selftest();
double gram_tile_selftest(bool four);
void store_sweep_args(const HalfSweepArgs* host, int n, HalfSweepArgs* dev, hipStream_t st);
void launch_sweep_finalize(const void* Wpart, void* W, int nWG, int C, int P, int kb_last, hipStream_t st);
void launch_hy_conj(const void* Hc, int64_t ldD, int nrows, const void* Yc, int64_t ldY, bool y_cplx, int D, int S, void* Pw, void* out,
                    int ldS, hipStream_t st);
size_t hy_workspace_elems(int nrows, int ldS);
void launch_ypinv(const void* Q, int64_t ldQ, bool q_cplx, const void* Zb, int ldS, int D, int S, int C, void* Ypinv,
                  int64_t ldD, hipStream_t st);
void launch_ls_apply(const void* Hc, int64_t ldH, int n_c, const void* Zf, bool z_cplx, int64_t ldD, int D, int C, int P,
                     int kb_lo, int kb_hi, void* W, hipStream_t st);
void launch_ls_filters(const double* hL, const double* hR, int64_t L, int D, const void* Yp, bool cplx_basis, int64_t ldD,
                       int C, void* wL, void* wR, hipStream_t st);
void launch_conj_copy(const void* in, void* out, int64_t n, bool is_cplx, hipStream_t st);
void launch_sh_rows_to_complex(void* W, int C, int nrows, int order, hipStream_t st);
void launch_widen(const void* in, int64_t ldi, bool in_cplx, void* out, int64_t ldo, int rows, int cols, bool transpose,
                  bool upper_only, hipStream_t st);

void launch_gram_inverse(const void* R, int S, bool is_cplx, void* M, int* status, hipStream_t st, void* work = nullptr);
void launch_ypinv_gram(const void* Ycm, int64_t ldD, bool is_cplx, const void* M, int S, int D, void* Ypinv, hipStream_t st);
void launch_sweep_wide(const DenseSweepArgs& a, int kb, bool x_cplx, hipStream_t st);
void launch_sweep_wide_finalize(const void* Wpart, void* W, int nWG, int C, int P, int kb_last, hipStream_t st);

void launch_wa_assemble(const void* Tn, const void* bn, int nOrd, int S, int C, int ldS, int P, int kb0, int nbins, void* B, hipStream_t st);
void launch_wa_factor(void* B, void* Vw, int S, int C, int ldS, int nbins, double reg_c, double* tauw, void* R2w, void* Nw, double* sv, int* sweeps,
                      void* Z, hipStream_t st);
struct WaTiling { int leaves, leaf_h, ldT; size_t off_stack, off_vt, off_zt, off_tau, bytes; };
WaTiling wa_tiling(int S, int C, int nbins);
void launch_wa_factor_tiled(void* B, void* Vw, int S, int C, int ldS, int nbins, double reg_c, double* tauw, void* R2w, void* Nw, double* sv,
                            int* sweeps, void* Z, void* ws, hipStream_t st);
void launch_wa_yri(const void* Q, int64_t ldQ, const void* Z, int S, int C, int ldS, int D, int64_t ldD, int nbins, void* Yri, hipStream_t st);
void launch_wa_ls(const void* Hc, int64_t ldH, int n_c, const void* Yri, int64_t ldD, int D, int C, int P, int kb_first, int kb_end, void* W, hipStream_t st);
void launch_wa_lo_gram(const void* Ycm, int M, int nOut, double* Ag, hipStream_t st);
void launch_wa_e(const void* Ycm, int M, int nOut, int S, const void* Minv, void* E, int ldE, hipStream_t st);

void launch_qt(const void* Yc, int64_t ldY, const void* E, int ldE, int D, int S, int C, int nOrders, bool is_cplx, void* QT,
               int64_t ldD, hipStream_t st);
void launch_dspace_g(const void* QT, int64_t ldD, bool is_cplx, const void* bn, int nOrders, int D, int C, int P, int k0, void* G,
                     hipStream_t st, int real_mode = 0, int sh_order = -1, int k_end = -1);
void launch_cond_flags(const double* sv, int C, int P, int hh_end, double* cond_ok, hipStream_t st);
void launch_yri_accurate(const void* Q, int64_t ldQ, bool is_cplx, const void* Z, int ldS, const double* cond_ok, int D, int S,
                         int C, int P, int k0, void* Yri, int64_t ldD, hipStream_t st, const void* Ycm = nullptr, int64_t ldYcm = 0);

void launch_grid_match(const double* aziA, const double* zenA, int64_t nA, const double* aziB, const double* zenB,
                       int64_t nB, double* cartB, int64_t* idx, double* dev_deg, double* mean_dev, hipStream_t st);
void launch_atf_colidx(const int64_t* idx, int64_t nA, int M, int64_t* colidx, hipStream_t st);

double measure_fp64_peak(int which, int reps, bool burst = false, double* mhz = nullptr);

void binaural_decode_real(const double* sig, int64_t n, int C, const double* wL, const double* wR, int64_t len,
                          double* out , hipStream_t st,
                          const cplx* sigc = nullptr );
bool decode_wave_form(int64_t len);
void binaural_decode_complex(const void* sig, bool sig_cplx, int64_t n, int C, const void* wL, const void* wR, bool w_cplx, int64_t len,
                             double* sig2, double* w2L, double* w2R, double* out, double* imag_abs, double* d_tmp, hipStream_t st,
                             int64_t imag_skip = 0 );
void decode_cache_clear();
void launch_abs_sum_cols(const double* x, int64_t n, int64_t skip, int ncols, double* out, hipStream_t st);

int rotate_order(int layout, int64_t C);
void launch_rotate_yaw(const void* in, bool in_cplx, int64_t n, int C, int layout, bool cplx_basis, const double* yaw, bool per_sample,
                       bool transpose, void* out, hipStream_t st, int64_t ld_in = 0, int64_t ld_out = 0, int L = 1, int64_t la = 0,
                       int64_t lo = 0);
int rotate3_max_order();
void launch_rotate3(const void* in, bool in_cplx, int64_t n, int C, bool cplx_basis, const double* yaw, bool yaw_ps, const double* pitch,
                    bool pitch_ps, const double* roll, bool roll_ps, bool transpose, void* out, hipStream_t st, int64_t ld_in = 0,
                    int64_t ld_out = 0, int L = 1, const int64_t* la = nullptr, int64_t lo = 0);
void launch_rotate3_matrix(int N, bool cplx_basis, double yaw, double pitch, double roll, void* out, hipStream_t st);
void rotate3_cache_clear();
struct EncodeBlock { const double* enc; bool enc_cplx; int M; const double* x; int64_t ldx; };
void launch_rotate_yaw_encoded(const EncodeBlock& e, int64_t n, int C, int layout, bool cplx_basis, const double* yaw, bool per_sample, void* out,
                               hipStream_t st, int64_t ld_out = 0, int L = 1, int64_t la = 0, int64_t lo = 0);
void launch_rotate3_encoded(const EncodeBlock& e, int64_t n, int C, bool cplx_basis, const double* yaw, bool yaw_ps, const double* pitch, bool pitch_ps,
                            const double* roll, bool roll_ps, void* out, hipStream_t st, int64_t ld_out = 0, int L = 1, const int64_t* la = nullptr,
                            int64_t lo = 0);
void launch_encode_block(const EncodeBlock& e, int64_t n, int C, void* out, int64_t ld_out, hipStream_t st);
constexpr int64_t kResampleMaxRatio = 65536;
int64_t resample_length(int64_t n, int64_t p, int64_t q);
void launch_resample(const void* in, bool cplx_in, int64_t n, int64_t nch, int64_t p, int64_t q, void* out, hipStream_t st);
void resample_cache_clear();

struct DecodeStreamState {
    int C = 0;
    bool planes2 = false;
    int B = 0, P = 0;
    int S = 1;
    int L = 1;
    cplx* Wf = nullptr;
    cplx* ring = nullptr;
    void* hist = nullptr;
    int* pos = nullptr;
};
bool decode_stream_block_ok(int64_t B);
void launch_decode_stream_filters(const double* wpl, int Cp, int64_t len, int B, int P, int64_t S, cplx* Wf, hipStream_t st);
void launch_partition_spectra(const double* wpl, int Cp, int64_t len, int B, int P, int64_t Z, cplx* Wf, hipStream_t st);
void launch_decode_stream_block(const DecodeStreamState& s, const void* x, bool x_cplx, int64_t ldx, const int* set, int standing, double* out,
                                int64_t ldo, hipStream_t st, int64_t lsx = 0, int lset = 0, int64_t lso = 0);

struct FieldStreamState {
    int nsrc = 0;
    int planes = 0;
    bool out_c = false;
    int B = 0, P = 0;
    cplx* Rf = nullptr;
    cplx* ring = nullptr;
    double* hist = nullptr;
    int* pos = nullptr;
};
void launch_field_stream_block(const FieldStreamState& s, const double* src, int64_t lds, void* out, int64_t ldo, hipStream_t st);
constexpr int kFieldStreamLaunches = 2;

void decode_family_cache_clear();

void filter_channels_by_order(const double* sig, int64_t n_in, int64_t n, int C, const double* ir , int nOrd, int64_t len,
                              int64_t skip, double* out , hipStream_t st);

void launch_ema_sh_e0(const void* Ech, int ldS, const void* Ypts, int C, int S, bool cb, void* E0, hipStream_t st);
void launch_rot_points(const double* azi, const double* zen, int D, int npts, double* azr, double* znr, hipStream_t st);
void launch_rot_from_points(const void* A, int64_t ldA, const void* Z, int ldP, int C, int npts, const double* zen, int D, bool cb, void* Rot,
                            hipStream_t st);
void launch_qt_rotate(void* QT, int64_t ldD, int nOrd, int C, int N, int D, const void* Rot, bool cb, hipStream_t st);
void launch_gram_from_g(const void* G, int64_t g_stride, int64_t ldD, int D, int C, int kb0, int nbins, int g0, double* Apk, int ldK,
                        hipStream_t st);

void launch_radial_filter(const void* bn, int nOrd, int P, int type, double regul, double g, bool nyq_abs, bool zero_nan,
                          void* out_kn, void* out_cm, hipStream_t st);
void launch_diffuse_field(const void* bn, int nOrd, int n_lo, int P, double* df_hi, double* df_lo, hipStream_t st);
void launch_array_diffuse(const void* bn, int nOrd, const void* Y, bool y_cplx, int ldY, int S, int M, int nOut, int P,
                          double* df_lo, hipStream_t st);
void launch_eq_spectrum(const double* df_hi, const double* df_lo, const double* df_arr, int P, int mode, void* W, double* W_full,
                        hipStream_t st);
void launch_diffuse_constraint(void* W, const void* G, bool g_cplx, int64_t g_stride, int g0, const void* H, int D, int C, int64_t ldD,
                               int P, hipStream_t st);
void launch_smair(const void* E, bool e_cplx, int ldS, const void* bn, int nOrd, const void* rad, int nRad, int rows, int S, int P, void* out,
                  hipStream_t st);
void launch_sh_encode(const double* sig, int64_t n, int M, const void* Z, int ldZ, int nOut, bool out_cplx, void* out, hipStream_t st);

int rh_num_metrics();
int rh_bins_padded(int P);
int rh_gemm_tiles(int64_t D);
int rh_atf_tiles(int64_t D);
void launch_rh_split(const void* in, int64_t ncols, int64_t len, double* out, hipStream_t st);
void launch_rh_join(const void* F, int64_t n, void* W, hipStream_t st);
void launch_rh_modes(const void* W, int C, int P, int nsets, const void* A, bool a_cplx, int ldA, const void* bn, int nOrd, int S, bool y_cplx,
                     double* Tt, int64_t ldR, hipStream_t st);
void launch_rh_order_rows(const void* W, int C, int P, int nsets, const void* bn, int nOrd, bool q_cplx, double* Tt, int64_t ldR, hipStream_t st);
void launch_rh_interleave(const void* Y, int64_t ldi, int S, int64_t D, double* Yk, int64_t ldo, hipStream_t st);
struct RhOut {
    const void* H = nullptr;
    int64_t hset_stride = 0;
    const double* w = nullptr;
    void* Hhat = nullptr;
    double* partial = nullptr;
// ... 14 lines not shown
```

emagls_amd/csrc/sweep_reg.hip:

```cpp
#include "kernels.hpp"
#include "persist_common.hpp"
#include "synth_common.hpp"

#include <algorithm>
#include <map>
#include <mutex>

namespace emagls {

namespace {

constexpr int RG_MLD = 36;

constexpr int DPP_ROR4 = 0x124, DPP_ROR8 = 0x128;
__device__ __forceinline__ int rg_slot_set(int i, int x) { return i < 4 ? 0 : i < 8 ? 1 : x >> 1; }
__device__ __forceinline__ int rg_slot_unit(int i, int x) { return i < 8 ? 4 * (i & 3) + x : 16 + (x & 1); }

template <int NUL>
__device__ __forceinline__ void rg_contract(const cplx (&E)[NUL], const cplx (&O)[NUL], const cplx (&ts)[2], int lane, bool slot8, double* wp) {
    static_assert(NUL == 9, "quad layout of 18 units");
    const int x = lane & 3;
    double ar[2], ai[2];
#pragma unroll
    for (int s = 0; s < 2; ++s) { ar[s] = (x & 1) ? ts[s].y : ts[s].x; ai[s] = (x & 1) ? -ts[s].x : ts[s].y; }
    double aE[5], aO[5];
#pragma unroll
    for (int r = 0; r < 5; ++r) { aE[r] = 0.0; aO[r] = 0.0; }
#pragma unroll
    for (int s = 0; s < 2; ++s)
#pragma unroll
        for (int c = 0; c < 2; ++c) {
            const double a = c ? ai[s] : ar[s];
#pragma unroll
            for (int r = 0; r < 4; ++r) {
                aE[r] = __builtin_amdgcn_mfma_f64_4x4x4f64(a, c ? E[4 * s + r].y : E[4 * s + r].x, aE[r], 0, 0, 0);
                aO[r] = __builtin_amdgcn_mfma_f64_4x4x4f64(a, c ? O[4 * s + r].y : O[4 * s + r].x, aO[r], 0, 0, 0);
            }
        }
    if (slot8) {
#pragma unroll
        for (int s = 0; s < 2; ++s) {
            const bool mine = (x >> 1) == s;
#pragma unroll
            for (int c = 0; c < 2; ++c) {
                const double a = c ? ai[s] : ar[s];
                aE[4] = __builtin_amdgcn_mfma_f64_4x4x4f64(a, mine ? (c ? E[8].y : E[8].x) : 0.0, aE[4], 0, 0, 0);
                aO[4] = __builtin_amdgcn_mfma_f64_4x4x4f64(a, mine ? (c ? O[8].y : O[8].x) : 0.0, aO[4], 0, 0, 0);
            }
        }
    }
    const int nacc = slot8 ? 5 : 4;
#pragma unroll
    for (int r = 0; r < 5; ++r) {
        if (r >= nacc) break;
        aE[r] += dpp_d<DPP_ROR4>(aE[r]); aE[r] += dpp_d<DPP_ROR8>(aE[r]);
        aO[r] += dpp_d<DPP_ROR4>(aO[r]); aO[r] += dpp_d<DPP_ROR8>(aO[r]);
    }
    if (slot8) { aE[4] += dpp_d<DPP_XOR2>(aE[4]); aO[4] += dpp_d<DPP_XOR2>(aO[4]); }
    if ((lane & 12) == 0) {
        const int y = lane >> 4;
#pragma unroll
        for (int r = 0; r < 4; ++r) { wp[8 * (4 * r + x) + y] = aE[r]; wp[8 * (4 * r + x) + 4 + y] = aO[r]; }
        if (slot8 && x < 2) { wp[8 * (16 + x) + y] = aE[4]; wp[8 * (16 + x) + 4 + y] = aO[4]; }
    }
}

template <int U0, int GS, int NUL, int NT>
__device__ __forceinline__ void synth_units(const double* xcol, cplx (&E)[NUL], cplx (&O)[NUL], const cplx* bs, int nord_pad) {
    double x2[GS], pa[GS], pb[GS];
#pragma unroll
    for (int i = 0; i < GS; ++i) x2[i] = xcol[(U0 + i) * NT];
#pragma unroll
    for (int i = 0; i < GS; ++i) { pa[i] = 1.0; pb[i] = 0.5 * x2[i]; E[U0 + i] = mk(0.0, 0.0); O[U0 + i] = mk(0.0, 0.0); }
    const unsigned bs0 = lds_addr(bs);
    d2_t b0, b1, c0, c1;
    auto request = [&](int n, d2_t& q0, d2_t& q1) __attribute__((always_inline)) {
        const int nn = n < nord_pad ? n : nord_pad - 2;
        lds_read16_async(q0, bs0 + 16 * nn, pa[0]); lds_read16_async(q1, bs0 + 16 * nn + 16, pa[0]);
    };
    auto pass = [&](const d2_t& q0, const d2_t& q1) __attribute__((always_inline)) {
#pragma unroll
        for (int i = 0; i < GS; ++i) {
            E[U0 + i].x = fma(q0.x, pa[i], E[U0 + i].x); E[U0 + i].y = fma(q0.y, pa[i], E[U0 + i].y);
            O[U0 + i].x = fma(q1.x, pb[i], O[U0 + i].x); O[U0 + i].y = fma(q1.y, pb[i], O[U0 + i].y);
            pa[i] = fma(x2[i], pb[i], -pa[i]);
            pb[i] = fma(x2[i], pa[i], -pb[i]);
        }
    };
    request(0, b0, b1);
    lds_wait2(b0, b1, pa[0]);
    for (int n = 0; n < nord_pad; n += 4) {
        request(n + 2, c0, c1);
        pass(b0, b1);
        lds_wait2(c0, c1, pb[GS - 1]);
        if (n + 2 >= nord_pad) break;
        request(n + 4, b0, b1);
        pass(c0, c1);
        lds_wait2(b0, b1, pb[GS - 1]);
    }
}

__device__ __forceinline__ int launder(int v) { asm volatile("" : "+v"(v)); return v; }

#define RG_GLOBAL(T, p) ((T __attribute__((address_space(1)))*)(p))
typedef const double __attribute__((address_space(1)))* gcd_t;
typedef const cplx __attribute__((address_space(1)))* gcc_t;
typedef u64 __attribute__((address_space(1)))* gu64_t;
typedef unsigned u32x4_t __attribute__((ext_vector_type(4)));
__device__ __forceinline__ cplx ldg(gcc_t p) { return mk(p->x, p->y); }
__device__ __forceinline__ u64 gll_load(gu64_t p) { return __hip_atomic_load(p, __ATOMIC_RELAXED, __HIP_MEMORY_SCOPE_AGENT); }
__device__ __forceinline__ void gll_put(gu64_t dst, u64 word, bool local) {
    if (local) __hip_atomic_store(dst, word, __ATOMIC_RELAXED, __HIP_MEMORY_SCOPE_WORKGROUP);
    else __hip_atomic_store(dst, word, __ATOMIC_RELAXED, __HIP_MEMORY_SCOPE_AGENT);
}
__device__ __forceinline__ void gll_load16_async(u32x4_t& out, gu64_t p) { asm volatile("global_load_dwordx4 %0, %1, off sc1" : "=v"(out) : "v"(p) : "memory"); }

constexpr int RG_POLL = 12;
__device__ __forceinline__ void rg_wait_loads(u32x4_t (&g)[RG_POLL]) {
    asm volatile("s_waitcnt vmcnt(0)" : "+v"(g[0]), "+v"(g[1]), "+v"(g[2]), "+v"(g[3]), "+v"(g[4]), "+v"(g[5]), "+v"(g[6]), "+v"(g[7]), "+v"(g[8]), "+v"(g[9]),
                 "+v"(g[10]), "+v"(g[11]) :: "memory");
}
constexpr int RG_NUL = 9;
constexpr int RG_NEX = 4 * PS_CMAX;
constexpr int RG_SVC = 256;

template <int NUL, int NW>
__global__ void __launch_bounds__(64 * NW) __attribute__((amdgpu_waves_per_eu(3))) sweep_reg_kernel(const HalfSweepArgs* __restrict__ args, int n, int nWG, int spread, int prio) {
    constexpr int NT = 64 * NW, DPW = 32 * NW;
    constexpr int NU2 = 2 * NUL;
    constexpr int NVW = 8 * NU2;
    constexpr int GA = (NUL + 1) / 2, GB = NUL - GA;
    static_assert(GB >= 1 && NW % 2 == 0 && NT >= RG_SVC, "layout");
    extern __shared__ __attribute__((aligned(16))) char dyn[];
    cplx* ring = reinterpret_cast<cplx*>(dyn);
    cplx* ms = ring + 2 * SY_NORD;
    cplx* WE = ms + PS_CMAX * RG_MLD;
    cplx* WO = WE + 2 * NU2;
    double* vt = reinterpret_cast<double*>(WO + 2 * NU2);
    double* wpart = vt + 2 * RG_NEX;
    double* xs = wpart + NW * NVW;
    __shared__ int s_abort, s_local;

    int design, member;
    if (spread) {
        design = (int)blockIdx.x / nWG;
        member = (int)blockIdx.x - design * nWG;
    } else {
        const int xcd = blockIdx.x & 7, rest = blockIdx.x >> 3;
        const int sub = rest / nWG;
        member = rest - sub * nWG;
        design = xcd + 8 * sub;
    }
    if (design >= n) return;
    if (prio) __builtin_amdgcn_s_setprio(3);
    const HalfSweepArgs& a = args[design];
    const int tid = threadIdx.x;
    const int C = a.C, P = a.P, D = a.D, kfirst = a.kfirst, kabs0 = a.kabs0;
    const int64_t ldH = a.ldH;
    const int nord_pad = a.nord_pad;
    const gcd_t Habs = RG_GLOBAL(const double, a.Habs);
    const gcc_t Mw = RG_GLOBAL(const cplx, a.Mw);
    const gcc_t bsc = RG_GLOBAL(const cplx, a.bsc);
    const gcd_t Winit = RG_GLOBAL(const double, a.Winit);
    cplx __attribute__((address_space(1)))* const Uout = RG_GLOBAL(cplx, a.U);
    long long* const timing = a.timing;
    int* const abort_flag = a.abort_flag;
    const long long wait_ticks = a.wait_ticks;
    const int* smap = a.smap;
    const int npr = smap[32], nsg = smap[33], nun = npr + nsg;
    const gu64_t part_ll = RG_GLOBAL(u64, a.ll);
    const gu64_t xcc_ll = part_ll + (size_t)2 * nWG * RG_NEX * 2;
    if (tid == 0) { s_abort = 0; s_local = 0; }
    const int d0 = member * DPW;
    auto dir_of = [&](int t, int s) __attribute__((always_inline)) { return d0 + 32 * (t >> 6) + 16 * s + ((t & 63) >> 2); };

    {
        const size_t ncplx = (size_t)2 * SY_NORD + PS_CMAX * RG_MLD + 4 * NU2;
        for (size_t i = tid; i < ncplx; i += NT) ring[i] = mk(0, 0);
        for (int i = tid; i < 2 * RG_NEX + NW * NVW; i += NT) vt[i] = 0.0;
        double sd[2], cd[2], daz[2];
#pragma unroll
        for (int s = 0; s < 2; ++s) {
            const int dgi = dir_of(tid, s) < D ? dir_of(tid, s) : D - 1;
            synth_zen(a.dir_zen[dgi], sd[s], cd[s]);
            daz[s] = a.dir_azi[dgi];
        }
#pragma unroll 1
        for (int i = 0; i < NUL; ++i) {
            const int u = rg_slot_unit(i, tid & 3), s = rg_slot_set(i, tid & 3);
            double v = 0.0;
            if (u < nun) {
                const int jm = smap[u < npr ? 2 * u : 2 * npr + (u - npr)];
                double sm, cm;
                synth_zen(a.mic_zen ? a.mic_zen[jm] : 1.5707963267948966, sm, cm);
                v = synth_x2(s ? sd[1] : sd[0], s ? cd[1] : cd[0], sm, cm, (s ? daz[1] : daz[0]) - a.mic_azi[jm]);
            }
            xs[i * NT + tid] = v;
        }
    }
    __syncthreads();

    if (tid < nord_pad) {
        ring[(kfirst & 1) * SY_NORD + tid] = ldg(bsc + (int64_t)kfirst * nord_pad + tid);
        const int k1 = kfirst + 1 < P ? kfirst + 1 : P - 1;
        ring[((kfirst + 1) & 1) * SY_NORD + tid] = ldg(bsc + (int64_t)k1 * nord_pad + tid);
    }
    constexpr int NLM = 4;
    cplx mReg[NLM];
    auto fetch_m = [&](int kbm, int t) __attribute__((always_inline)) {
        const int r = t >> 3, c0 = (t & 7) * 4;
        const gcc_t M = Mw + (int64_t)kbm * C * C + r * C + c0;
#pragma unroll
        for (int i = 0; i < NLM; ++i) mReg[i] = ldg(M + i);
    };
    auto stage_m = [&](int t) __attribute__((always_inline)) {
        const int r = t >> 3, c0 = (t & 7) * 4;
#pragma unroll
        for (int i = 0; i < NLM; ++i) ms[r * RG_MLD + c0 + i] = (r < C && c0 + i < C) ? mReg[i] : mk(0, 0);
    };
    double hCur[2], hNext[2] = {0.0, 0.0};
    auto fetch_h = [&](int kb, double (&h)[2], int t) __attribute__((always_inline)) {
        const int kbg = (kb < P ? kb : P - 1) - kabs0;
        const gcd_t He = Habs + ((int64_t)((t >> 1) & 1) * (P - kabs0) + kbg) * ldH;
#pragma unroll
        for (int s = 0; s < 2; ++s) h[s] = He[dir_of(t, s) < D ? dir_of(t, s) : D - 1];
    };
    fetch_h(kfirst, hCur, tid);
    if (tid < RG_SVC) { fetch_m(kfirst, tid); stage_m(tid); }

    if (tid < 64) {
        const int lane = tid;
        const unsigned xcc = read_xcc_id();
        const unsigned tag0 = 0x58434300u;
        if (lane == 0) gll_put(xcc_ll + member, ((u64)tag0 << 32) | xcc, false);
        bool alive = true, same = true;
        for (int base = 0; base < nWG && alive; base += 64) {
            u64 w = 0;
            alive = ll_wait([&] {
                if (base + lane >= nWG) return true;
                w = gll_load(xcc_ll + base + lane);
                return ll_ok(w, tag0);
            }, abort_flag, wait_ticks);
            same = same && __builtin_amdgcn_ballot_w64(base + lane < nWG && (unsigned)w != xcc) == 0;
        }
        if (lane == 0) {
            s_local = alive && same && a.force_global == 0;
            if (!alive) s_abort = 1;
            if (timing && member == 1) timing[15] = s_local;
        }
    }
    __syncthreads();
    const bool local = s_local != 0;
    if (s_abort) return;

    const bool slot8 = nun > 16 || GB < 2;
    cplx E[NUL], O[NUL];
#pragma unroll
    for (int u = 0; u < NUL; ++u) { E[u] = mk(0, 0); O[u] = mk(0, 0); }

#define RSTAMP(i) do { if (timing && member == 1 && tid == 0 && kb < P) timing[(int64_t)kb * 16 + (i)] = (long long)wall_clock64(); } while (0)
    for (int kb = kfirst; kb <= P; ++kb) {
        const bool first = (kb == kfirst);
        const bool last = (kb == P);
        const bool nyq = (kb == P - 1);
        RSTAMP(7);
        if (!last) {
            const cplx* bs = ring + (kb & 1) * SY_NORD;
            const double* xcol = xs + launder(tid);
            synth_units<0, GA, NUL, NT>(xcol, E, O, bs, nord_pad);
            __builtin_amdgcn_sched_barrier(0);
            if (slot8) synth_units<GA, GB, NUL, NT>(xcol, E, O, bs, nord_pad);
            else synth_units<GA, GB - 1, NUL, NT>(xcol, E, O, bs, nord_pad);
            __builtin_amdgcn_sched_barrier(0);
        }
        RSTAMP(0);
        if (launder(tid) < RG_SVC) {
            const int t = launder(tid);
            const int j = t & (RG_NEX - 1), half = t >> 7;
            if (first) {
                vt[t] = half == 0 ? Winit[j] : 0.0;
            } else {
                const unsigned tag = (unsigned)(kb - 1);
                const gu64_t src = part_ll + ((size_t)((kb - 1) & 1) * nWG * RG_NEX + j) * 2;
                double sum = 0.0;
                const bool alive = ll_wait([&] {
                    bool ok = true;
                    double s = 0.0;
                    for (int base = half; base < nWG; base += 2 * RG_POLL) {
                        u32x4_t g[RG_POLL];
#pragma unroll
                        for (int i = 0; i < RG_POLL; ++i) {
                            const int w = base + 2 * i < nWG ? base + 2 * i : half;
                            gll_load16_async(g[i], src + (size_t)w * RG_NEX * 2);
                        }
                        rg_wait_loads(g);
#pragma unroll
                        for (int i = 0; i < RG_POLL; ++i) {
                            ok = ok && g[i].y == tag && g[i].w == tag;
                            if (base + 2 * i < nWG) s += __hiloint2double((int)g[i].z, (int)g[i].x);
                        }
                    }
                    sum = s;
                    return ok;
                }, abort_flag, wait_ticks);
                vt[t] = sum;
                if (!alive && (t & 63) == 0) s_abort = 1;
            }
        }
        RSTAMP(2);
        __syncthreads();
        if (s_abort) break;
        if (launder(tid) < RG_SVC) {
            const int t = launder(tid);
            const int part = t & 3, pair = t >> 2, e = pair >> 5, c = pair & 31;
            const cplx* vc = reinterpret_cast<const cplx*>(vt) + e * PS_CMAX;
            cplx acc = mk(0, 0);
            if (first) {
                if (part == 0) acc = vc[c];
            } else {
#pragma unroll
                for (int i = 0; i < PS_CMAX / 4; ++i)
                    cfma(acc, vc[part + 4 * i] + vc[RG_NEX / 2 + part + 4 * i], conj(ms[(part + 4 * i) * RG_MLD + c]));
            }
            acc = group_sum<4>(acc);
            const cplx other = shfl_xor_c(acc, 4);
            if (part == 0 && c < C) {
                if (c < 2 * npr) {
                    if ((c & 1) == 0) { WE[e * NU2 + (c >> 1)] = acc + other; WO[e * NU2 + (c >> 1)] = acc - other; }
                } else {
                    WE[e * NU2 + npr + (c - 2 * npr)] = acc; WO[e * NU2 + npr + (c - 2 * npr)] = acc;
                }
                if (member == 0 && !first) {
                    cplx __attribute__((address_space(1)))* dst = Uout + ((int64_t)e * P + (kb - 1)) * PS_CMAX + c;
                    const cplx v = vc[c] + vc[RG_NEX / 2 + c];
                    dst->x = v.x; dst->y = v.y;
                }
            }
        }
        if (last) break;
        __syncthreads();
        RSTAMP(3);
        const bool svc = launder(tid) < RG_SVC;
        if (svc) fetch_m(kb, launder(tid));
        cplx ts[2];
        {
            const int t = launder(tid);
            const int x = t & 3;
            cplx p[2][2];
#pragma unroll
            for (int s = 0; s < 2; ++s) { p[s][0] = mk(0, 0); p[s][1] = mk(0, 0); }
#pragma unroll
            for (int r = 0; r < 4; ++r) {
                const int u = 4 * r + x;
                const cplx we0 = WE[u], wo0 = WO[u], we1 = WE[NU2 + u], wo1 = WO[NU2 + u];
#pragma unroll
                for (int s = 0; s < 2; ++s) {
                    cfma(p[s][0], we0, E[4 * s + r]); cfma(p[s][0], wo0, O[4 * s + r]);
                    cfma(p[s][1], we1, E[4 * s + r]); cfma(p[s][1], wo1, O[4 * s + r]);
                }
            }
            if (slot8) {
                const int u = 16 + (x & 1);
                cplx q0 = mk(0, 0), q1 = mk(0, 0);
                cfma(q0, WE[u], E[8]); cfma(q0, WO[u], O[8]);
                cfma(q1, WE[NU2 + u], E[8]); cfma(q1, WO[NU2 + u], O[8]);
                const bool s1 = (x & 2) != 0;
                const cplx z = mk(0, 0);
                p[0][0] = p[0][0] + (s1 ? z : q0); p[0][1] = p[0][1] + (s1 ? z : q1);
                p[1][0] = p[1][0] + (s1 ? q0 : z); p[1][1] = p[1][1] + (s1 ? q1 : z);
            }
            if (svc) stage_m(t);
            RSTAMP(8);
#pragma unroll
            for (int s = 0; s < 2; ++s) {
                const cplx pe0 = group_sum<4>(p[s][0]), pe1 = group_sum<4>(p[s][1]);
                const cplx pe = (x & 2) ? pe1 : pe0;
                ts[s] = dir_of(t, s) < D ? unit_phase(hCur[s], pe, nyq) : mk(0, 0);
            }
        }
        __builtin_amdgcn_sched_barrier(0);
        {
            const int t = launder(tid);
            rg_contract<NUL>(E, O, ts, t & 63, slot8, wpart + (t >> 6) * NVW);
        }
        {
            const int t = launder(tid);
            fetch_h(kb + 1, hNext, t);
            if (t < nord_pad) ring[(kb & 1) * SY_NORD + t] = ldg(bsc + (int64_t)(kb + 2 < P ? kb + 2 : P - 1) * nord_pad + t);
        }
        __syncthreads();
        RSTAMP(4);
        if (launder(tid) < RG_NEX) {
            const int t = launder(tid);
            const int xe = t >> 6, xr = (t >> 1) & 31, xri = t & 1;
            double v = 0.0;
            if (xr < C) {
                const int xu = xr < 2 * npr ? (xr >> 1) : npr + (xr - 2 * npr);
                const bool xneg = xr < 2 * npr && (xr & 1);
                const double* wE = wpart + 8 * xu + 2 * xe + xri;
                double sE = 0.0, sO = 0.0;
#pragma unroll
                for (int w = 0; w < NW; ++w) { sE += wE[w * NVW]; sO += wE[w * NVW + 4]; }
                v = xneg ? sE - sO : sE + sO;
            }
            const gu64_t dst = part_ll + (((size_t)(kb & 1) * nWG + member) * RG_NEX + t) * 2;
            const u64 bits = (u64)__double_as_longlong(v), tg = (u64)(unsigned)kb << 32;
            gll_put(dst, tg | (bits & 0xffffffffull), local);
            gll_put(dst + 1, tg | (bits >> 32), local);
        }
        RSTAMP(5);
        hCur[0] = hNext[0]; hCur[1] = hNext[1];
    }
#undef RSTAMP
}

__global__ void __launch_bounds__(64) reg_contract_selftest_kernel(const cplx* __restrict__ t, const cplx* __restrict__ g, double* __restrict__ out) {
    const int lane = threadIdx.x, x = lane & 3;
    cplx E[RG_NUL], O[RG_NUL], ts[2];
#pragma unroll
    for (int i = 0; i < RG_NUL; ++i) {
        const int d = 16 * rg_slot_set(i, x) + (lane >> 2), u = rg_slot_unit(i, x);
        E[i] = ldc(g + (d * 18 + u) * 2);
        O[i] = ldc(g + (d * 18 + u) * 2 + 1);
    }
#pragma unroll
    for (int s = 0; s < 2; ++s) ts[s] = ldc(t + (16 * s + (lane >> 2)) * 2 + (x >> 1));
    rg_contract<RG_NUL>(E, O, ts, lane, true, out);
}

__global__ void __launch_bounds__(64) store_args_kernel(HalfSweepMulti m, HalfSweepArgs* dst) {
    const int nw = (int)(sizeof(HalfSweepArgs) / 8);
    for (int j = 0; j < m.n; ++j) {
        const unsigned long long* src = reinterpret_cast<const unsigned long long*>(&m.a[j]);
        unsigned long long* d = reinterpret_cast<unsigned long long*>(dst + j);
        for (int i = threadIdx.x; i < nw; i += 64) d[i] = src[i];
    }
}
static_assert(sizeof(HalfSweepArgs) % 8 == 0, "argument block in whole words");

size_t reg_dyn_bytes(int nul, int nw) {
    const size_t nu2 = 2 * (size_t)nul, nvw = 8 * nu2;
    return sizeof(cplx) * ((size_t)2 * SY_NORD + PS_CMAX * RG_MLD + 4 * nu2) +
           sizeof(double) * (2 * RG_NEX + (size_t)nw * nvw + (size_t)nul * 64 * nw);
}
constexpr int RG_WAVES[] = {4, 6, 8, 10, 12};
const void* reg_kernel_ptr(int nw) {
    switch (nw) {
        case 4: return reinterpret_cast<const void*>(sweep_reg_kernel<RG_NUL, 4>);
        case 6: return reinterpret_cast<const void*>(sweep_reg_kernel<RG_NUL, 6>);
        case 8: return reinterpret_cast<const void*>(sweep_reg_kernel<RG_NUL, 8>);
        case 10: return reinterpret_cast<const void*>(sweep_reg_kernel<RG_NUL, 10>);
        default: return reinterpret_cast<const void*>(sweep_reg_kernel<RG_NUL, 12>);
    }
}
void reg_set_attributes() {
    static PerDeviceOnce attr_once;
    if (attr_once.first())
        for (int nw : RG_WAVES) HIP_CHECK(hipFuncSetAttribute(reg_kernel_ptr(nw), hipFuncAttributeMaxDynamicSharedMemorySize, 150 * 1024));
}
int reg_nwg(int D, int nw) { return (int)ceil_div(D, 32 * nw); }
int reg_occupancy(int nw) {
    static std::mutex mu;
    static std::map<std::pair<int, int>, int> cache;
    int dev = 0;
    HIP_CHECK(hipGetDevice(&dev));
    std::lock_guard<std::mutex> lk(mu);
    auto it = cache.find({dev, nw});
    if (it != cache.end()) return it->second;
    reg_set_attributes();
    int nb = 0;
    if (hipOccupancyMaxActiveBlocksPerMultiprocessor(&nb, reg_kernel_ptr(nw), 64 * nw, reg_dyn_bytes(RG_NUL, nw)) != hipSuccess) { (void)hipGetLastError(); nb = 0; }
    cache[{dev, nw}] = nb;
    return nb;
}
int reg_wg_cost(int nw) { return nw == 4 ? 1 : 3; }

}

int reg_sweep_max_units() { return 2 * RG_NUL; }
bool reg_sweep_supported(int D, int nmics, int nunits, int nOrd) {
    return nmics >= 2 && nmics <= PS_CMAX && nunits >= 1 && nunits <= 2 * RG_NUL && D >= 1 && reg_nwg(D, 12) <= 32 && nOrd <= SY_NORD;
}
size_t reg_sweep_ll_bytes(int D, int nmics) {
    const size_t nwg = (size_t)reg_nwg(D, 4);
    (void)nmics;
    return sizeof(u64) * ((size_t)2 * nwg * RG_NEX * 2 + nwg + 64);
}
int reg_sweep_slots_per_xcd() { return 3 * (sweep_cu_budget() / 8); }
int reg_sweep_pick_waves(int D, int ndesigns) {
    if (ndesigns < 1 || ndesigns > REG_SWEEP_MAX) return 0;
    const int nsub = (int)ceil_div(ndesigns, 8), cus = sweep_cu_budget() / 8;
    if (const int nw = sw_int<Sw::REG_WAVES>()) {
        if ((nw == 4 || nw == 6 || nw == 8 || nw == 10 || nw == 12) && nsub * reg_nwg(D, nw) * reg_wg_cost(nw) <= 3 * cus && reg_occupancy(nw) >= (nw == 4 ? 3 : 1)) return nw;
    }
    for (int nw : RG_WAVES) if (nsub * reg_nwg(D, nw) <= cus && reg_occupancy(nw) >= 1) return nw;
    return (nsub * reg_nwg(D, 4) <= 3 * cus && reg_occupancy(4) >= 3) ? 4 : 0;
}
int reg_sweep_spread_waves(int D, int ndesigns) {
    const int mode = sw_int<Sw::REG_SPREAD>();
    if (mode == 0 || ndesigns < 1 || ndesigns > REG_SWEEP_MAX || sw_int<Sw::REG_WAVES>() != 0) return 0;
    const int cus = sweep_cu_budget(), local = reg_sweep_pick_waves(D, ndesigns);
    for (int nw : RG_WAVES)
        if (ndesigns * reg_nwg(D, nw) <= cus && reg_occupancy(nw) >= 1) return (mode == 1 || local == 0 || nw < local) ? nw : 0;
    return 0;
}
int reg_sweep_gate_cost(int D, int ndesigns) {
    if (const int ns = reg_sweep_spread_waves(D, ndesigns)) return (int)ceil_div((int64_t)ndesigns * reg_nwg(D, ns), 8) * reg_wg_cost(ns);
    const int nw = reg_sweep_pick_waves(D, ndesigns);
    return nw ? (int)ceil_div(ndesigns, 8) * reg_nwg(D, nw) * reg_wg_cost(nw) : 0;
}
int reg_sweep_capacity(int D) {
    int n = 0;
    for (int k = 8; k <= REG_SWEEP_MAX; k += 8) if (reg_sweep_pick_waves(D, k)) n = k;
    return n;
}
bool reg_sweep_fits(int D, int nmics, int nunits, int nOrd, int ndesigns) {
    return reg_sweep_supported(D, nmics, nunits, nOrd) && reg_sweep_pick_waves(D, ndesigns) != 0;
}

void launch_sweep_reg(const HalfSweepArgs* args_dev, const HalfSweepArgs& a0, int n, hipStream_t st) {
    const int ns = reg_sweep_spread_waves(a0.D, n);
    const int nw = ns ? ns : reg_sweep_pick_waves(a0.D, n);
    if (!nw) throw Error(2, "register-resident sweep: the launch cannot be resident");
    const int nWG = reg_nwg(a0.D, nw), spread = ns ? 1 : 0;
    const unsigned nblocks = spread ? (unsigned)(n * nWG) : 8u * (unsigned)nWG * (unsigned)ceil_div(n, 8);
    const size_t dyn = reg_dyn_bytes(RG_NUL, nw);
    reg_set_attributes();
    const int prio = sw_int<Sw::REG_PRIO>();
    switch (nw) {
        case 4: sweep_reg_kernel<RG_NUL, 4><<<dim3(nblocks), 256, dyn, st>>>(args_dev, n, nWG, spread, prio); break;
        case 6: sweep_reg_kernel<RG_NUL, 6><<<dim3(nblocks), 384, dyn, st>>>(args_dev, n, nWG, spread, prio); break;
        case 8: sweep_reg_kernel<RG_NUL, 8><<<dim3(nblocks), 512, dyn, st>>>(args_dev, n, nWG, spread, prio); break;
        case 10: sweep_reg_kernel<RG_NUL, 10><<<dim3(nblocks), 640, dyn, st>>>(args_dev, n, nWG, spread, prio); break;
        default: sweep_reg_kernel<RG_NUL, 12><<<dim3(nblocks), 768, dyn, st>>>(args_dev, n, nWG, spread, prio); break;
    }
    KERNEL_CHECK();
}

double reg_contract_selftest() {
    constexpr int ND = 32, NU = 2 * RG_NUL, NO = 8 * NU;
    cplx h_t[ND * 2], h_g[ND * NU * 2];
    double h_out[NO], want[NO] = {0};
    unsigned long long x = 88172645463325252ull;
    auto rnd = [&] { x ^= x << 13; x ^= x >> 7; x ^= x << 17; return (double)(x % 2000001ull) / 1000000.0 - 1.0; };
    for (cplx& v : h_t) { v.x = rnd(); v.y = rnd(); }
    for (cplx& v : h_g) { v.x = rnd(); v.y = rnd(); }
    for (int d = 0; d < ND; ++d)
        for (int u = 0; u < NU; ++u)
            for (int eo = 0; eo < 2; ++eo)
                for (int e = 0; e < 2; ++e) {
                    const cplx tv = h_t[d * 2 + e], gv = h_g[(d * NU + u) * 2 + eo];
                    want[8 * u + 4 * eo + 2 * e] += tv.x * gv.x + tv.y * gv.y;
                    want[8 * u + 4 * eo + 2 * e + 1] += tv.y * gv.x - tv.x * gv.y;
                }
    cplx *d_t = nullptr, *d_g = nullptr;
    double* d_out = nullptr;
    HIP_CHECK(hipMalloc(&d_t, sizeof h_t));
    HIP_CHECK(hipMalloc(&d_g, sizeof h_g));
    HIP_CHECK(hipMalloc(&d_out, sizeof h_out));
    HIP_CHECK(hipMemcpy(d_t, h_t, sizeof h_t, hipMemcpyHostToDevice));
    HIP_CHECK(hipMemcpy(d_g, h_g, sizeof h_g, hipMemcpyHostToDevice));
    HIP_CHECK(hipMemset(d_out, 0, sizeof h_out));
    reg_contract_selftest_kernel<<<1, 64>>>(d_t, d_g, d_out);
    KERNEL_CHECK();
    HIP_CHECK(hipMemcpy(h_out, d_out, sizeof h_out, hipMemcpyDeviceToHost));
    HIP_CHECK(hipFree(d_t));
    HIP_CHECK(hipFree(d_g));
    HIP_CHECK(hipFree(d_out));
    double err = 0.0;
    for (int i = 0; i < NO; ++i) err = std::max(err, std::fabs(h_out[i] - want[i]));
    return err;
}

void store_sweep_args(const HalfSweepArgs* host, int n, HalfSweepArgs* dev, hipStream_t st) {
    for (int first = 0; first < n; first += SWEEP_MULTI_MAX) {
        HalfSweepMulti m{};
        m.n = std::min(SWEEP_MULTI_MAX, n - first);
        for (int j = 0; j < m.n; ++j) m.a[j] = host[first + j];
        store_args_kernel<<<1, 64, 0, st>>>(m, dev + first);
        KERNEL_CHECK();
    }
}

}
```

emagls_amd/csrc/switches.hpp:

```cpp
#pragma once
#include <climits>
#include <cmath>

namespace emagls {

#define EMAGLS_SWITCHES(X) \
    X(PLAN_CACHE,        INT,  4,     0, INT_MAX,   PROCESS, "shapes the one-shot entry points keep alive (0 = off)") \
    X(BATCH_MAX,         INT,  8,     1, 32,        PROCESS, "initial limit of designs per batch, read at load time (emagls_set_batch_max changes it at run time; the job scheduler sets it per chunk)") \
    X(BATCH_GROUPS,      INT,  2,     1, 4,         CALL,    "lane groups of a batch of more than 8 designs before its sweep (1 = one launch sequence)") \
    X(BATCH_LANES,       ON0,  1,     0, 1,         CALL,    "=0: batches in stream mode (per-plan pipelines) instead of lane mode") \
    X(DEBUG_LANES,       ON1,  0,     0, 1,         CALL,    "=1: why a batch was refused lane mode or common routes, on stderr") \
    X(STAGGER,           ON0,  1,     0, 1,         PROCESS, "=0: both lane groups of a batch issue the stages before the sweep in one order (default: complementary orders)") \
    X(DEFER_HH,          INT,  1,     0, 2,         PROCESS, "the orthonormal route of the low bins next to the sweep: 0 never, 1 batches and designs that have the device to themselves, 2 every lane batch") \
    X(GEO_KEEP,          ON0,  1,     0, 1,         PROCESS, "=0: sharing batches run their geometry stages on every execute") \
    X(GRAM_LDS,          ON0,  1,     0, 1,         PROCESS, "=0: lane batches take the K-split Gram kernel + reduce instead of the LDS-staged one") \
    X(GRAM_MFMA4,        ON1,  0,     0, 1,         CALL,    "=1: the Gram tile on the 4 x 4 x 4 MFMA shape (measured slower; the tests' second form)") \
    X(XCD_RUNS,          ON0,  1,     0, 1,         PROCESS, "=0: gram_lds, gemm_tn_f64, synth_ls take their tiles in dispatch order instead of XCD-aware runs") \
    X(GRAM_ROUTE,        ON0,  1,     0, 1,         CALL,    "=0: no Gram route (all bins Householder + Jacobi)") \
    X(GRAM_COND_EST,     REAL, 3e3,   -HUGE_VAL, HUGE_VAL, CALL, "conditioning estimate below which the Gram route starts (the device check stays at 3e4)") \
    X(JACOBI_RUN,        INT,  0,     1, INT_MAX,   PROCESS, "bins per Jacobi workgroup on the Gram route (0: single bins where the stages are forked, runs of 2 in lane groups)") \
    X(REAL_INTERNAL,     ON0,  1,     0, 1,         CALL,    "=0: complex-basis eMagLS / eMagLS2 designs on the complex-arithmetic pipeline") \
    X(NO_GRAPH,          ON1,  0,     0, 1,         CALL,    "=1: eager launches instead of hipGraph replay (plans and batches, when they are created)") \
    X(STREAMS,           INT,  0,     1, 4,         CALL,    "streams of a single plan (0: one, until emagls_plan_set_streams)") \
    X(ONESHOT_STREAMS,   INT,  1,     1, 3,         CALL,    "streams of the one-shot plans of array designs") \
    X(SWEEP_PERSIST,     ON0,  1,     0, 1,         CALL,    "=0: launch-per-bin sweep instead of the persistent one") \
    X(PERSIST_GLOBAL,    ON1,  0,     0, 1,         CALL,    "=1: write-through granules even when a design sits on one XCD") \
    X(SWEEP_SYNTH,       ON0,  1,     0, 1,         CALL,    "=0: array designs on materialised operands instead of the synthesising sweep (when a plan is created)") \
    X(SWEEP_TWIN,        ON0,  1,     0, 1,         CALL,    "=0: launches of 9-16 designs as two independent workgroups per CU instead of twin workgroups") \
    X(SWEEP_REG,         INT,  1,     0, 2,         CALL,    "register-resident sweep: 0 never (the slab form), 1 for launches of more than 8 designs, 2 always") \
    X(REG_WAVES,         INT,  0,     INT_MIN, INT_MAX, CALL, "waves per workgroup of the register-resident sweep (4, 6, 8, 10, 12 whenever it fits; 0: the smallest count with which every workgroup owns a CU)") \
    X(REG_SPREAD,        INT,  2,     0, 2,         CALL,    "a launch's designs spread over all XCDs: 0 never, 1 whenever it fits, 2 when it needs fewer waves per workgroup than the one-XCD layout") \
    X(REG_PRIO,          INT,  1,     INT_MIN, INT_MAX, PROCESS, "=0: the register-resident sweep's waves at the default issue priority") \
    X(SWEEP_FETCH,       INT,  0,     0, 4,         PROCESS, "where the persistent sweep requests the next bin's operands") \
    X(SWEEP_WAIT_MS,     INT,  20,    1, INT_MAX,   PROCESS, "wall-clock limit of a wait for peers inside a resident sweep, in ms") \
    X(SWEEP_TIMING,      ON1,  0,     0, 1,         CALL,    "=1: in-kernel wall-clock stamps of the persistent sweep (when a plan is created)") \
    X(CU_BUDGET,         INT,  0,     0, INT_MAX,   CALL,    "CUs the resident sweeps may count on when their residency is decided (0: the device's)") \
    X(SYNTH_PAIRS,       ON0,  1,     0, 1,         PROCESS, "=0: synthesising sweep without antipodal microphone pairs") \
    X(SYNTH_SPLIT,       INT,  67,    INT_MIN, INT_MAX, PROCESS, "synthesising sweep: per cent of the producers' unit groups evaluated before barrier B1") \
    X(SYNTH_PRIO,        INT,  5,     0, 5,         PROCESS, "synthesising sweep: issue priorities (5: the chains of the two designs of an XCD tilted against the age order; 0: all chains 3, producers 0)") \
    X(STREAM_POOL,       ON0,  1,     0, 1,         PROCESS, "=0: destroy streams instead of recycling them (exposes a HIP runtime crash in long sessions)") \
    X(STREAM_WARM,       INT,  8,     0, INT_MAX,   PROCESS, "streams the pool parks before it hands the first one out") \
    X(POOL_GB,           INT,  128,   0, INT_MAX,   PROCESS, "device memory the block pool keeps for the next plans and arenas, in GB") \
    X(JOBS_FORK,         INT,  3,     1, 4,         PROCESS, "job scheduler: streams of a job list that is a single chunk (1 = lane groups as for chunks in flight)") \
    X(JOBS_RESIDENT,     INT,  0,     0, INT_MAX,   CALL,    "job scheduler: designs whose plans and batches stay resident between calls (0: max(256, 2 x batch x in flight))") \
    X(JOBS_AUTO_SHARE,   ON0,  1,     0, 1,         PROCESS, "=0: job scheduler shares no geometry unless the caller asks") \
    X(JOBS_TRACE,        ON1,  0,     0, 1,         PROCESS, "=1: time stamps of every chunk's steps and of block pool misses on stderr") \
    X(HRIR_FFT_WAVE,     ON0,  1,     0, 1,         CALL,    "=0: the HRIR prologue at nfft = 1024 on the LDS radix-2^2 transform instead of wave-private transforms") \
    X(HRIR_FFT_LDS_KB,   INT,  0,     40, 158,      CALL,    "LDS budget of the LDS-form HRIR transform's sub-tiles (0: 83, 110 at nfft = 2048)") \
    X(DECODE_FUSED,      ON0,  1,     0, 1,         CALL,    "=0: binauralDecode on the hipFFT passes for every filter length") \
    X(DECODE_REGFFT,     ON0,  1,     0, 1,         CALL,    "=0: the fused decode kernel on LDS transform passes also up to 512 taps") \
    X(DECODE_WAVE,       ON0,  1,     0, 1,         CALL,    "=0: the half-wave two-factor decode form also at 257-512 taps") \
    X(DECODE_FILTER_FFT, ONH,  0,     0, 1,         CALL,    "=hipfft: the filter side of the decode's wave form through hipFFT") \
    X(WA_REG,            ON0,  1,     0, 1,         CALL,    "=0: the 33-64-channel path's Householder kernels walk the columns through L2") \
    X(WA_TALL,           ON0,  1,     0, 1,         CALL,    "=0: the plain Householder kernels for problems of more than 448 rows instead of the LDS-reflector forms") \
    X(WA_YRI_MFMA,       ON0,  1,     0, 1,         CALL,    "=0: the 33-64-channel path's Y_reg_inv_k product on the vector pipe") \
    X(WA_JACOBI_FLAG,    REAL, 1e-14, -HUGE_VAL, HUGE_VAL, PROCESS, "the 33-64-channel path's Jacobi: another sweep follows one in which some rotation had |gamma| > x sqrt(alpha beta)") \
    X(WA_LEAF_ROWS,      INT,  0,     INT_MIN, INT_MAX, PROCESS, "tiled QR: upper bound of the leaf height, 1024 .. 4096 (anything else: 3072)")

enum class Sw : int {
#define X(name, kind, def, lo, hi, when, doc) name,
    EMAGLS_SWITCHES(X)
#undef X
    COUNT
};
enum class SwKind { ON0, ON1, ONH, INT, REAL };
constexpr SwKind sw_kind(Sw s) {
    constexpr SwKind kinds[] = {
#define X(name, kind, def, lo, hi, when, doc) SwKind::kind,
        EMAGLS_SWITCHES(X)
#undef X
    };
    return kinds[(int)s];
}

double sw_value(Sw s);

template <Sw S> inline bool sw_on() {
    static_assert(sw_kind(S) == SwKind::ON0 || sw_kind(S) == SwKind::ON1 || sw_kind(S) == SwKind::ONH, "not a flag");
    return sw_value(S) != 0.0;
}
template <Sw S> inline int sw_int() { static_assert(sw_kind(S) == SwKind::INT, "not an integer switch"); return (int)sw_value(S); }
template <Sw S> inline double sw_real() { static_assert(sw_kind(S) == SwKind::REAL, "not a real switch"); return sw_value(S); }

}
```

include/emagls.h:

```cpp
#ifndef EMAGLS_H
#define EMAGLS_H

#include <stddef.h>
#include <stdint.h>

#ifdef __cplusplus
extern "C" {
#endif

#define EMAGLS_OK 0
#define EMAGLS_ERR_ARG 1
#define EMAGLS_ERR_UNSUPPORTED 2
#define EMAGLS_ERR_HIP 3
#define EMAGLS_ERR_NUMERIC 4

#define EMAGLS_BASIS_REAL 0
#define EMAGLS_BASIS_COMPLEX 1

#define EMAGLS_KIND_LS 0
#define EMAGLS_KIND_MAGLS 1
#define EMAGLS_KIND_EMAGLS 2
#define EMAGLS_KIND_EMAGLS2 3
#define EMAGLS_KIND_FROM_ATF 4
#define EMAGLS_KIND_EMA_CH 5
// ... 171 lines not shown
                                     void* stream);

int emagls_decode_stream_reset(emagls_decode_stream* s);

int emagls_decode_stream_info(const emagls_decode_stream* s, int64_t* block, int64_t* partitions, int64_t* state_bytes,
                              int64_t* filter_bytes, int* launches_per_block);

int emagls_decode_stream_destroy(emagls_decode_stream* s);

int emagls_decode_stream_create_bank(int64_t nch, int64_t n_sets, const void* wL, const void* wR, int filters_are_complex, int64_t len,
                                     int in_is_complex, int layout, int basis, int64_t block, emagls_decode_stream** s);

int emagls_decode_stream_push_sets(emagls_decode_stream* s, const void* in, int64_t nsamp, const int32_t* set, int64_t n_set,
                                   const double* yaw, int64_t n_yaw, const double* pitch, int64_t n_pitch, const double* roll,
                                   int64_t n_roll, double* out);

int emagls_decode_stream_push_sets_device(emagls_decode_stream* s, const void* d_in, int64_t nsamp, const int32_t* d_set, int64_t n_set,
                                          const double* d_yaw, int64_t n_yaw, const double* d_pitch, int64_t n_pitch,
                                          const double* d_roll, int64_t n_roll, double* d_out, void* stream);

int emagls_decode_stream_sets(const emagls_decode_stream* s, int64_t* n_sets);

typedef struct emagls_decode_group emagls_decode_group;
int emagls_decode_group_create(int64_t nch, int64_t n_sets, const void* wL, const void* wR, int filters_are_complex, int64_t len,
                               int in_is_complex, int layout, int basis, int64_t block, int64_t n_listeners, emagls_decode_group** g);

int emagls_decode_group_push(emagls_decode_group* g, const void* in, int64_t nsamp, const int32_t* set, int64_t n_set, const double* yaw,
                             int64_t n_yaw, const double* pitch, int64_t n_pitch, const double* roll, int64_t n_roll, double* out);

int emagls_decode_group_push_device(emagls_decode_group* g, const void* d_in, int64_t nsamp, const int32_t* d_set, int64_t n_set,
                                    const double* d_yaw, int64_t n_yaw, const double* d_pitch, int64_t n_pitch, const double* d_roll,
                                    int64_t n_roll, double* d_out, void* stream);

int emagls_decode_group_reset(emagls_decode_group* g, int64_t listener);

int emagls_decode_group_info(const emagls_decode_group* g, int64_t* block, int64_t* partitions, int64_t* listeners, int64_t* state_bytes,
                             int64_t* filter_bytes, int* launches_per_block);

int emagls_decode_group_destroy(emagls_decode_group* g);

int emagls_decode_stream_create_encoded(int64_t nmics, const void* enc, int enc_is_complex, int64_t nch, int64_t n_sets, const void* wL,
                                        const void* wR, int filters_are_complex, int64_t len, int layout, int basis, int64_t block,
                                        emagls_decode_stream** s);
int emagls_decode_group_create_encoded(int64_t nmics, const void* enc, int enc_is_complex, int64_t nch, int64_t n_sets, const void* wL,
                                       const void* wR, int filters_are_complex, int64_t len, int layout, int basis, int64_t block,
                                       int64_t n_listeners, emagls_decode_group** g);

typedef struct emagls_field_stream emagls_field_stream;
int emagls_field_stream_create(int64_t nsrc, int64_t nch, const void* rir, int rir_is_complex, int64_t nr, int64_t block,
                               emagls_field_stream** f);

int emagls_field_stream_push(emagls_field_stream* f, const double* src, int64_t nsamp, void* out);

int emagls_field_stream_push_device(emagls_field_stream* f, const double* d_src, int64_t nsamp, void* d_out, void* stream);

int emagls_field_stream_reset(emagls_field_stream* f);

int emagls_field_stream_info(const emagls_field_stream* f, int64_t* block, int64_t* partitions, int64_t* state_bytes,
                             int64_t* response_bytes, int* launches_per_block);

int emagls_field_stream_destroy(emagls_field_stream* f);

int emagls_get_magls_filters_dc(const double* hL, const double* hR, int64_t nsamp, int64_t ndirs, const double* azi, const double* zen,
                                int order, double fs, int64_t len, int apply_diffuseness_const, int basis, void* wL, void* wR);
int emagls_get_emagls_filters_dc(const double* hL, const double* hR, int64_t nsamp, int64_t ndirs, const double* azi, const double* zen,
                                 double mic_radius, const double* mic_azi, const double* mic_zen, int64_t nmics, int order, double fs,
                                 int64_t len, int apply_diffuseness_const, int basis, void* wL, void* wR);
int emagls_get_emagls2_filters_dc(const double* hL, const double* hR, int64_t nsamp, int64_t ndirs, const double* azi, const double* zen,
                                  double mic_radius, const double* mic_azi, const double* mic_zen, int64_t nmics, int order, double fs,
                                  int64_t len, int apply_diffuseness_const, int basis, void* wL, void* wR);


int emagls_get_magls_filters_2d(const double* hL, const double* hR, int64_t nsamp, int64_t ndirs, const double* hrir_azi,
                                int order, double fs, int64_t len, int basis, void* wL, void* wR);

#define EMAGLS_RADIAL_TIKHONOV 0
#define EMAGLS_RADIAL_SOFTLIMIT 1
#define EMAGLS_RADIAL_FULL 2
#define EMAGLS_RADIAL_NONE 3
int emagls_get_radial_filter(int order, double fs, double sma_radius, int64_t ir_len, int oversampling, int filter_type,
                             double regul_const, double noise_gain_db, void* rad);
int64_t emagls_apply_radial_filter_rows(int64_t nsamp, int64_t ir_len, int oversampling);
int emagls_apply_radial_filter(const double* sig, int64_t nsamp, int order, double fs, double sma_radius, int64_t ir_len,
                               int oversampling, int filter_type, double regul_const, double noise_gain_db, double* out);
int emagls_sh_encode(const double* sig, int64_t nsamp, int64_t nmics, const double* mic_azi, const double* mic_zen, int order,
                     int basis, void* out);
int emagls_ch_basis(int order, int64_t ndirs, const double* azi, int basis, void* Y);
int emagls_get_smair_matrix(int order, double fs, int64_t ir_len, int oversampling, double sma_radius, const double* mic_azi,
                            const double* mic_zen, int64_t nmics, int basis, int return_raw_mic_sigs, int radial_filter_type,
                            double regul_const, double noise_gain_db, void* smair, int* sim_order);
int64_t emagls_eq_filter_nfft(int64_t len);
int emagls_get_magls_spherical_head_filter(double mic_radius, int order, double fs, int64_t len, double* w_shf, double* W_shf);
int emagls_get_magls_array_diffuse_filter(double mic_radius, const double* mic_azi, const double* mic_zen, int64_t nmics, int order,
                                          double fs, int64_t len, int basis, const void* Y_hi, double* w_adf);

#define EMAGLS_MODEL_SH 0
#define EMAGLS_MODEL_EMAGLS 1
#define EMAGLS_MODEL_EMAGLS2 2
#define EMAGLS_MODEL_ATF 3
#define EMAGLS_MODEL_EMA_CH 5
#define EMAGLS_MODEL_EMA_SH 6
int emagls_rendered_hrtfs(int model, const void* wL, const void* wR, int w_is_complex, int64_t len, int64_t nchan, int64_t nsets,
                          const double* dir_azi, const double* dir_zen, int64_t ndirs, double fs, int order, int basis,
                          double mic_radius, const double* mic_azi, const double* mic_zen, int64_t nmics, const double* atf,
                          int64_t atf_taps, int64_t nfft, const double* hL, const double* hR, int64_t nsamp, int64_t nhrir_sets,
                          const double* weights, void* Hhat, double* mag_err_db, double* ild_err_db, double* cov_hat, double* cov_ref);


typedef struct emagls_plan emagls_plan;

typedef struct emagls_design_desc {
    int kind;
    int basis;
    int order;
    double fs;
    int64_t len;
    int64_t nsamp;
    int64_t ndirs;
    double mic_radius;
    int64_t nmics;
    double f_trans;
    int64_t atf_taps;
    int64_t natf;
    int custom_basis;
    int diffuseness;
    int sim_order_pad;
} emagls_design_desc;

typedef struct emagls_plan_info {
    int nfft, num_pos_freqs, k_cut , sim_order, num_sh_sim, num_channels;
    int out_is_complex;
    int64_t out_rows, out_cols;
    double grp_delay_l, grp_delay_r;
    double mean_grid_dev_deg;
    int num_sweep_launches;
    int64_t device_bytes;
    int gram_from, hh_end, hh_orders, g_first;
    int sim_order_own;
    int sweep_form, sweep_units;
} emagls_plan_info;

int emagls_plan_create(const emagls_design_desc* desc, emagls_plan** plan);
int emagls_plan_destroy(emagls_plan* plan);
int emagls_plan_set_hrir_grid(emagls_plan* plan, const double* azi, const double* zen);
int emagls_plan_set_mic_grid(emagls_plan* plan, const double* azi, const double* zen);
int emagls_plan_set_hrirs(emagls_plan* plan, const double* hL, const double* hR);
int emagls_plan_set_basis(emagls_plan* plan, const void* Y_hrir, const void* Y_mic);
int emagls_plan_set_atfs(emagls_plan* plan, const double* atf_irs, const double* atf_azi, const double* atf_zen);
int emagls_plan_execute(emagls_plan* plan);
int emagls_plan_synchronize(emagls_plan* plan);
int emagls_plan_get_filters(emagls_plan* plan, void* wL, void* wR);
int emagls_plan_get_info(emagls_plan* plan, emagls_plan_info* info);
int emagls_plan_sweep_form_in_batch(emagls_plan* plan, int designs, int* form);
int emagls_plan_set_streams(emagls_plan* plan, int nstreams);
int emagls_plan_set_profiling(emagls_plan* plan, int level);
int emagls_plan_num_stages(emagls_plan* plan);
const char* emagls_plan_stage_name(emagls_plan* plan, int stage);
int emagls_plan_stage_times(emagls_plan* plan, double* ms, int n);
int emagls_plan_sweep_kernel_time(emagls_plan* plan, double* total_ms, int* launches);
int emagls_plan_debug_buffer(emagls_plan* plan, const char* name, void* dst, size_t* nbytes);
void* emagls_plan_stream(emagls_plan* plan);

typedef struct emagls_batch emagls_batch;
int emagls_batch_create(emagls_plan** plans, int nplans, emagls_batch** batch);
int emagls_set_batch_max(int max_designs, int* previous);
int emagls_batch_set_geometry_sharing(emagls_batch* batch, int enable);
int emagls_batch_shares_geometry(emagls_batch* batch, int* shared);
int emagls_batch_geometry_runs(emagls_batch* batch, long long* cold, long long* warm);
typedef struct emagls_job {
    emagls_design_desc desc;
    const double* hL;
    const double* hR;
    const double* hrir_azi;
    const double* hrir_zen;
    const double* mic_azi;
    const double* mic_zen;
    const double* atf;
    const double* atf_azi;
    const double* atf_zen;
    void* wL;
    void* wR;
} emagls_job;
#define EMAGLS_JOBS_SHARE_GEOMETRY 1
#define EMAGLS_JOBS_INDEPENDENT 2
int emagls_jobs_run(const emagls_job* jobs, int64_t njobs, int batch_size, int in_flight, int flags);
int emagls_jobs_shard(const emagls_job* jobs, int64_t njobs, int world, int max_batch, int* rank_of_job, int* order_in_rank, int* sim_order_pad);
int emagls_jobs_run_devices(const emagls_job* jobs, int64_t njobs, const int* devices, int ndevices, int batch_size, int in_flight, int flags);
int emagls_design_out_shape(const emagls_design_desc* desc, int64_t* rows, int64_t* cols, int* is_complex);
int emagls_jobs_set_profiling(int level);
int emagls_jobs_sweep_times(double* ms, int* designs, int capacity, int* count);
int emagls_jobs_geometry_runs(long long* independent, long long* cold, long long* warm);
int emagls_jobs_would_share_geometry(const emagls_job* jobs, int njobs, int* share);

int emagls_design_hrir_sets(int kind, const double* hL, const double* hR, int64_t nsamp, int64_t ndirs, int64_t nsets,
                            const double* hrir_azi, const double* hrir_zen, double mic_radius, const double* mic_azi, const double* mic_zen,
                            int64_t nmics, int order, double fs, int64_t len, int basis, void* wL, void* wR);
int emagls_from_atf_hrir_sets(const double* hL, const double* hR, int64_t nsamp, int64_t ndirs, int64_t nsets, const double* hrir_azi,
                              const double* hrir_zen, const double* atf_irs, int64_t atf_taps, int64_t nmics, int64_t natf, const double* atf_azi,
                              const double* atf_zen, double fs, int64_t filter_len, double f_trans, double* wL, double* wR, double* mean_dev);
int emagls_batch_shares_atf_side(emagls_batch* batch, int* shared);
int emagls_batch_execute(emagls_batch* batch);
int emagls_batch_synchronize(emagls_batch* batch);
int emagls_batch_get_filters(emagls_batch* batch, void* const* wL, void* const* wR);
int emagls_batch_set_profiling(emagls_batch* batch, int level);
int emagls_batch_lane_mode(emagls_batch* batch, int* lanes);
int emagls_batch_set_stream(emagls_batch* batch, void* hip_stream);
int emagls_batch_set_side_stream(emagls_batch* batch, void* hip_stream);
int emagls_batch_sweep_time(emagls_batch* batch, double* ms);
int emagls_batch_set_streams(emagls_batch* batch, int nstreams);
int emagls_batch_set_stage_order(emagls_batch* batch, int order);
int emagls_batch_destroy(emagls_batch* batch);

#ifdef __cplusplus
}
#endif
#endif
```

Measured before the change: 3930 filter sets/s.

## Process multiple HRIR sets per workgroup group in register-resident sweep

```diff
diff --git a/emagls_amd/_lib.py b/emagls_amd/_lib.py
--- a/emagls_amd/_lib.py
+++ b/emagls_amd/_lib.py
@@ -207,6 +207,8 @@
     "emagls_plan_get_filters": (C.c_int, [C.c_void_p, C.c_void_p, C.c_void_p]),
     "emagls_plan_get_info": (C.c_int, [C.c_void_p, C.POINTER(PlanInfo)]),
     "emagls_plan_sweep_form_in_batch": (C.c_int, [C.c_void_p, C.c_int, C.POINTER(C.c_int)]),
+    "emagls_reg_sweep_layout": (C.c_int, [C.c_int] * 9 + [C.POINTER(C.c_int)]),
+    "emagls_reg_sweep_launch_counts": (C.c_int, [C.POINTER(C.c_longlong)]),
     "emagls_plan_set_profiling": (C.c_int, [C.c_void_p, C.c_int]),
     "emagls_plan_set_streams": (C.c_int, [C.c_void_p, C.c_int]),
     "emagls_plan_num_stages": (C.c_int, [C.c_void_p]),
diff --git a/emagls_amd/csrc/batch_run.hip b/emagls_amd/csrc/batch_run.hip
--- a/emagls_amd/csrc/batch_run.hip
+++ b/emagls_amd/csrc/batch_run.hip
@@ -17,6 +17,7 @@
         }
     const bool reg = b.plans[0]->sweep_persist && reg_sweep_wanted(b.plans.data(), nb);
     for (auto* q : b.plans) q->reg_sweep = reg;
+    const int hint = (reg && b.geo_share && b.plans[0]->synth) ? std::max(1, b.side_by_side) : 0;
     if (!reg && nb > SWEEP_MULTI_MAX) throw Error(EMAGLS_ERR_UNSUPPORTED, "internal: more than 16 designs in a batch need the register-resident sweep");
     HalfSweepMulti h{};
     h.n = std::min(nb, SWEEP_MULTI_MAX);
@@ -27,7 +28,7 @@
     if (q0.sweep_persist) {
         hipStream_t ss = b.stream;
         {
-            SweepGate gate(ss, reg ? reg_sweep_gate_cost((int)q0.D, nb) : 0);
+            SweepGate gate(ss, reg ? reg_sweep_gate_cost((int)q0.D, nb, hint) : 0);
             if (b.lanes) { BatchScope sc(nb, b.stride); launch_zero(q0.get("ll"), q0.bufs["ll"].bytes, ss); }
             else for (auto* q : b.plans) launch_zero(q->get("ll"), q->bufs["ll"].bytes, ss);
             if (reg) {
@@ -35,7 +36,7 @@
                 reg_args_upload(ha.data(), nb, b.sweep_args_dev, b.sweep_args_last, ss);
             }
             if (b.prof_level >= 1) HIP_CHECK(hipEventRecord(b.sweep_ev[0], ss));
-            if (reg) launch_sweep_reg(static_cast<const HalfSweepArgs*>(b.sweep_args_dev), ha[0], nb, ss);
+            if (reg) launch_sweep_reg(static_cast<const HalfSweepArgs*>(b.sweep_args_dev), ha[0], nb, ss, hint);
             else if (q0.synth) launch_sweep_synth(h, ss); else launch_sweep_persist(h, ss);
             if (b.prof_level >= 1) HIP_CHECK(hipEventRecord(b.sweep_ev[1], ss));
         }
diff --git a/emagls_amd/csrc/capi.hip b/emagls_amd/csrc/capi.hip
--- a/emagls_amd/csrc/capi.hip
+++ b/emagls_amd/csrc/capi.hip
@@ -389,6 +389,26 @@
         *form = p->d.kind == EMAGLS_KIND_LS ? 0 : (p->synth ? (reg ? 3 : 2) : (p->sweep_persist ? 1 : 0));
     });
 }
+int emagls_reg_sweep_layout(int ndirs, int designs, int hint, int sets, int waves, int spread, int cus, int wg_per_cu_four, int wg_per_cu_large, int* out) {
+    return guarded([&] {
+        if (!out) throw Error(EMAGLS_ERR_ARG, "emagls_reg_sweep_layout: null pointer");
+        RegSweepEnv e{};
+        e.cus = cus; e.waves = waves; e.spread = spread; e.sets = sets;
+        for (int i = 0; i < 3; ++i)
+            for (int j = 0; j < 5; ++j) e.occ[i][j] = (i > 0 && (j == 1 || j == 3)) ? 0 : (j == 0 ? wg_per_cu_four : wg_per_cu_large);
+        const RegSweepForm f = reg_sweep_layout(e, ndirs, designs, hint);
+        const int v[8] = {f.ns, f.nw, f.spread, f.groups, f.nwg, f.wg_per_xcd, f.blocks, f.gate};
+        for (int i = 0; i < 8; ++i) out[i] = v[i];
+    });
+}
+int emagls_reg_sweep_launch_counts(long long* counts) {
+    return guarded([&] {
+        if (!counts) throw Error(EMAGLS_ERR_ARG, "emagls_reg_sweep_launch_counts: null pointer");
+        long long c[3];
+        reg_sweep_launch_counts(c);
+        for (int i = 0; i < 3; ++i) counts[i] = c[i];
+    });
+}
 int emagls_plan_get_info(emagls_plan* p, emagls_plan_info* info) {
     return guarded([&] {
         DeviceGuard dg(p ? p->device : -1);
diff --git a/emagls_amd/csrc/host_internal.hpp b/emagls_amd/csrc/host_internal.hpp
--- a/emagls_amd/csrc/host_internal.hpp
+++ b/emagls_amd/csrc/host_internal.hpp
@@ -379,6 +379,7 @@
     CapturedGraph group_hh[4];
     hipStream_t hh_stream[4] = {nullptr, nullptr, nullptr, nullptr};
     bool defer_hh = false;
+    int side_by_side = 1;
     bool alone = true;
     int eager_runs = 0;
     bool use_graph = true;
diff --git a/emagls_amd/csrc/jobs.hip b/emagls_amd/csrc/jobs.hip
--- a/emagls_amd/csrc/jobs.hip
+++ b/emagls_amd/csrc/jobs.hip
@@ -194,7 +194,7 @@
     }
     return true;
 }
-void jobs_run_chunk(const emagls_job* jobs, int n, int device, int flags, bool solo, uint64_t call) {
+void jobs_run_chunk(const emagls_job* jobs, int n, int device, int flags, bool solo, int side_by_side, uint64_t call) {
     DeviceGuard dg(device);
     const bool trace = sw_on<Sw::JOBS_TRACE>();
     const auto t_begin = std::chrono::steady_clock::now();
@@ -264,7 +264,8 @@
         if (!slot->batch && n > 1 && !slot->runs) check_rc(emagls_plan_set_hrirs(p, jb.hL, jb.hR));
     }
     lap("inputs set");
-    if (n > 1 && !slot->batch && !slot->runs) {
+    const bool create = n > 1 && !slot->batch && !slot->runs;
+    if (create) {
         int rc;
         { Scoped limit(g_batch_max_override, REG_SWEEP_MAX); rc = emagls_batch_create(slot->plans.data(), n, &slot->batch); }
         if (rc != EMAGLS_OK && rc != EMAGLS_ERR_UNSUPPORTED) check_rc(rc);
@@ -280,7 +281,9 @@
             if (!solo && slot->batch->group[0]) { HIP_CHECK(hipStreamSynchronize(slot->batch->stream)); drop_batch_graphs(*slot->batch); }
         }
         lap("batch created");
-    } else if (slot->batch) {
+    }
+    if (slot->batch) slot->batch->side_by_side = side_by_side;
+    if (!create && slot->batch) {
         bool gathered = false;
         if (2 * n <= 64) {
             bool all_dev = true;
@@ -430,6 +433,7 @@
         std::mutex err_mu;
         int err_code = EMAGLS_OK;
         std::string err_msg;
+        const int side = (int)std::min<size_t>((size_t)in_flight, chunks.size());
         auto work = [&] {
             for (;;) {
                 const size_t c = next.fetch_add(1);
@@ -440,12 +444,12 @@
                 }
                 try {
                     try {
-                        jobs_run_chunk(jobs + chunks[c].first, chunks[c].second, device, flags, chunks.size() == 1, call);
+                        jobs_run_chunk(jobs + chunks[c].first, chunks[c].second, device, flags, chunks.size() == 1, side, call);
                     } catch (const Error& e) {
                         if (chunks[c].second <= SWEEP_MULTI_MAX || e.code != EMAGLS_ERR_UNSUPPORTED || !strstr(e.what(), "more than 16 designs")) throw;
                         const int h = (chunks[c].second + 1) / 2;
-                        jobs_run_chunk(jobs + chunks[c].first, h, device, flags, false, call);
-                        jobs_run_chunk(jobs + chunks[c].first + h, chunks[c].second - h, device, flags, false, call);
+                        jobs_run_chunk(jobs + chunks[c].first, h, device, flags, false, side, call);
+                        jobs_run_chunk(jobs + chunks[c].first + h, chunks[c].second - h, device, flags, false, side, call);
                     }
                 } catch (const Error& e) {
                     std::lock_guard<std::mutex> lk(err_mu);
diff --git a/emagls_amd/csrc/kernels.hpp b/emagls_amd/csrc/kernels.hpp
--- a/emagls_amd/csrc/kernels.hpp
+++ b/emagls_amd/csrc/kernels.hpp
@@ -111,9 +111,14 @@
 int reg_sweep_capacity(int D);
 int reg_sweep_slots_per_xcd();
 int reg_sweep_pick_waves(int D, int ndesigns);
-int reg_sweep_gate_cost(int D, int ndesigns);
+struct RegSweepForm { int ns, nw, spread, groups, nwg, wg_per_xcd, blocks, gate; };
+struct RegSweepEnv { int cus, occ[3][5], waves, spread, sets; };
+RegSweepForm reg_sweep_layout(const RegSweepEnv& e, int D, int ndesigns, int hint);
+RegSweepForm reg_sweep_form(int D, int ndesigns, int hint);
+int reg_sweep_gate_cost(int D, int ndesigns, int hint = 0);
 bool reg_sweep_fits(int D, int nmics, int nunits, int nOrd, int ndesigns);
-void launch_sweep_reg(const HalfSweepArgs* args_dev, const HalfSweepArgs& a0, int n, hipStream_t st);
+void launch_sweep_reg(const HalfSweepArgs* args_dev, const HalfSweepArgs& a0, int n, hipStream_t st, int hint = 0);
+void reg_sweep_launch_counts(long long (&out)[3]);
 double reg_contract_selftest();
 double gram_tile_selftest(bool four);
 void store_sweep_args(const HalfSweepArgs* host, int n, HalfSweepArgs* dev, hipStream_t st);
diff --git a/emagls_amd/csrc/sweep_reg.hip b/emagls_amd/csrc/sweep_reg.hip
--- a/emagls_amd/csrc/sweep_reg.hip
+++ b/emagls_amd/csrc/sweep_reg.hip
@@ -3,6 +3,7 @@
 #include "synth_common.hpp"
 
 #include <algorithm>
+#include <atomic>
 #include <map>
 #include <mutex>
 
@@ -120,16 +121,21 @@
     asm volatile("s_waitcnt vmcnt(0)" : "+v"(g[0]), "+v"(g[1]), "+v"(g[2]), "+v"(g[3]), "+v"(g[4]), "+v"(g[5]), "+v"(g[6]), "+v"(g[7]), "+v"(g[8]), "+v"(g[9]),
                  "+v"(g[10]), "+v"(g[11]) :: "memory");
 }
+constexpr int RG_POLL_SETS = 6;
+__device__ __forceinline__ void rg_wait_loads(u32x4_t (&g)[RG_POLL_SETS]) {
+    asm volatile("s_waitcnt vmcnt(0)" : "+v"(g[0]), "+v"(g[1]), "+v"(g[2]), "+v"(g[3]), "+v"(g[4]), "+v"(g[5]) :: "memory");
+}
 constexpr int RG_NUL = 9;
 constexpr int RG_NEX = 4 * PS_CMAX;
 constexpr int RG_SVC = 256;
 
-template <int NUL, int NW>
+template <int NUL, int NW, int NS>
 __global__ void __launch_bounds__(64 * NW) __attribute__((amdgpu_waves_per_eu(3))) sweep_reg_kernel(const HalfSweepArgs* __restrict__ args, int n, int nWG, int spread, int prio) {
     constexpr int NT = 64 * NW, DPW = 32 * NW;
     constexpr int NU2 = 2 * NUL;
     constexpr int NVW = 8 * NU2;
     constexpr int GA = (NUL + 1) / 2, GB = NUL - GA;
+    constexpr int NPOLL = NS == 1 ? RG_POLL : RG_POLL_SETS;
     static_assert(GB >= 1 && NW % 2 == 0 && NT >= RG_SVC, "layout");
     extern __shared__ __attribute__((aligned(16))) char dyn[];
     cplx* ring = reinterpret_cast<cplx*>(dyn);
@@ -151,24 +157,25 @@
         member = rest - sub * nWG;
         design = xcd + 8 * sub;
     }
-    if (design >= n) return;
+    if (design * NS >= n) return;
+    const int g0 = design * NS, nset = NS == 1 ? 1 : (n - g0 < NS ? n - g0 : NS);
     if (prio) __builtin_amdgcn_s_setprio(3);
-    const HalfSweepArgs& a = args[design];
+    const HalfSweepArgs& a = args[g0];
     const int tid = threadIdx.x;
     const int C = a.C, P = a.P, D = a.D, kfirst = a.kfirst, kabs0 = a.kabs0;
     const int64_t ldH = a.ldH;
     const int nord_pad = a.nord_pad;
-    const gcd_t Habs = RG_GLOBAL(const double, a.Habs);
+    gcd_t Habs = RG_GLOBAL(const double, a.Habs);
     const gcc_t Mw = RG_GLOBAL(const cplx, a.Mw);
     const gcc_t bsc = RG_GLOBAL(const cplx, a.bsc);
-    const gcd_t Winit = RG_GLOBAL(const double, a.Winit);
-    cplx __attribute__((address_space(1)))* const Uout = RG_GLOBAL(cplx, a.U);
-    long long* const timing = a.timing;
-    int* const abort_flag = a.abort_flag;
+    gcd_t Winit = RG_GLOBAL(const double, a.Winit);
+    cplx __attribute__((address_space(1)))* Uout = RG_GLOBAL(cplx, a.U);
+    long long* timing = a.timing;
+    int* abort_flag = a.abort_flag;
     const long long wait_ticks = a.wait_ticks;
     const int* smap = a.smap;
     const int npr = smap[32], nsg = smap[33], nun = npr + nsg;
-    const gu64_t part_ll = RG_GLOBAL(u64, a.ll);
+    gu64_t part_ll = RG_GLOBAL(u64, a.ll);
     const gu64_t xcc_ll = part_ll + (size_t)2 * nWG * RG_NEX * 2;
     if (tid == 0) { s_abort = 0; s_local = 0; }
     const int d0 = member * DPW;
@@ -260,6 +267,7 @@
 
 #define RSTAMP(i) do { if (timing && member == 1 && tid == 0 && kb < P) timing[(int64_t)kb * 16 + (i)] = (long long)wall_clock64(); } while (0)
     for (int kb = kfirst; kb <= P; ++kb) {
+        if constexpr (NS > 1) timing = a.timing;
         const bool first = (kb == kfirst);
         const bool last = (kb == P);
         const bool nyq = (kb == P - 1);
@@ -273,6 +281,14 @@
             else synth_units<GA, GB - 1, NUL, NT>(xcol, E, O, bs, nord_pad);
             __builtin_amdgcn_sched_barrier(0);
         }
+#pragma unroll 1
+        for (int s = 0; s < nset; ++s) {
+        if constexpr (NS > 1) {
+            const HalfSweepArgs& as = args[g0 + s];
+            Winit = RG_GLOBAL(const double, as.Winit); Uout = RG_GLOBAL(cplx, as.U);
+            timing = as.timing; abort_flag = as.abort_flag; part_ll = RG_GLOBAL(u64, as.ll);
+        }
+        const bool tail = NS == 1 || s == nset - 1;
         RSTAMP(0);
         if (launder(tid) < RG_SVC) {
             const int t = launder(tid);
@@ -286,16 +302,16 @@
                 const bool alive = ll_wait([&] {
                     bool ok = true;
                     double s = 0.0;
-                    for (int base = half; base < nWG; base += 2 * RG_POLL) {
-                        u32x4_t g[RG_POLL];
-#pragma unroll
-                        for (int i = 0; i < RG_POLL; ++i) {
+                    for (int base = half; base < nWG; base += 2 * NPOLL) {
+                        u32x4_t g[NPOLL];
+#pragma unroll
+                        for (int i = 0; i < NPOLL; ++i) {
                             const int w = base + 2 * i < nWG ? base + 2 * i : half;
                             gll_load16_async(g[i], src + (size_t)w * RG_NEX * 2);
                         }
                         rg_wait_loads(g);
 #pragma unroll
-                        for (int i = 0; i < RG_POLL; ++i) {
+                        for (int i = 0; i < NPOLL; ++i) {
                             ok = ok && g[i].y == tag && g[i].w == tag;
                             if (base + 2 * i < nWG) s += __hiloint2double((int)g[i].z, (int)g[i].x);
                         }
@@ -309,7 +325,10 @@
         }
         RSTAMP(2);
         __syncthreads();
-        if (s_abort) break;
+        if (s_abort) {
+            if constexpr (NS > 1) { if (tid < nset) __hip_atomic_store(args[g0 + tid].abort_flag, 1, __ATOMIC_RELAXED, __HIP_MEMORY_SCOPE_AGENT); }
+            return;
+        }
         if (launder(tid) < RG_SVC) {
             const int t = launder(tid);
             const int part = t & 3, pair = t >> 2, e = pair >> 5, c = pair & 31;
@@ -337,10 +356,14 @@
                 }
             }
         }
-        if (last) break;
+        if (last) {
+            if (tail) return;
+            __syncthreads();
+            continue;
+        }
         __syncthreads();
         RSTAMP(3);
-        const bool svc = launder(tid) < RG_SVC;
+        const bool svc = launder(tid) < RG_SVC && tail;
         if (svc) fetch_m(kb, launder(tid));
         cplx ts[2];
         {
@@ -385,8 +408,11 @@
         }
         {
             const int t = launder(tid);
-            fetch_h(kb + 1, hNext, t);
-            if (t < nord_pad) ring[(kb & 1) * SY_NORD + t] = ldg(bsc + (int64_t)(kb + 2 < P ? kb + 2 : P - 1) * nord_pad + t);
+            if constexpr (NS > 1) {
+                Habs = RG_GLOBAL(const double, args[g0 + (tail ? 0 : s + 1)].Habs);
+                fetch_h(tail ? kb + 1 : kb, hNext, t);
+            } else fetch_h(kb + 1, hNext, t);
+            if (tail && t < nord_pad) ring[(kb & 1) * SY_NORD + t] = ldg(bsc + (int64_t)(kb + 2 < P ? kb + 2 : P - 1) * nord_pad + t);
         }
         __syncthreads();
         RSTAMP(4);
@@ -410,6 +436,7 @@
         }
         RSTAMP(5);
         hCur[0] = hNext[0]; hCur[1] = hNext[1];
+        }
     }
 #undef RSTAMP
 }
@@ -444,38 +471,129 @@
            sizeof(double) * (2 * RG_NEX + (size_t)nw * nvw + (size_t)nul * 64 * nw);
 }
 constexpr int RG_WAVES[] = {4, 6, 8, 10, 12};
-const void* reg_kernel_ptr(int nw) {
+constexpr int RG_SETS[] = {1, 2, 4};
+constexpr int RG_NWV = 5, RG_NST = 3;
+bool reg_has_kernel(int nw, int ns) { return ns == 1 ? (nw >= 4 && nw <= 12 && nw % 2 == 0) : ((ns == 2 || ns == 4) && (nw == 4 || nw == 8 || nw == 12)); }
+template <int NS> const void* reg_kernel_ptr_sets(int nw) {
     switch (nw) {
-        case 4: return reinterpret_cast<const void*>(sweep_reg_kernel<RG_NUL, 4>);
-        case 6: return reinterpret_cast<const void*>(sweep_reg_kernel<RG_NUL, 6>);
-        case 8: return reinterpret_cast<const void*>(sweep_reg_kernel<RG_NUL, 8>);
-        case 10: return reinterpret_cast<const void*>(sweep_reg_kernel<RG_NUL, 10>);
-        default: return reinterpret_cast<const void*>(sweep_reg_kernel<RG_NUL, 12>);
+        case 4: return reinterpret_cast<const void*>(sweep_reg_kernel<RG_NUL, 4, NS>);
+        case 8: return reinterpret_cast<const void*>(sweep_reg_kernel<RG_NUL, 8, NS>);
+        default: return reinterpret_cast<const void*>(sweep_reg_kernel<RG_NUL, 12, NS>);
+    }
+}
+const void* reg_kernel_ptr(int nw, int ns = 1) {
+    if (ns == 2) return reg_kernel_ptr_sets<2>(nw);
+    if (ns == 4) return reg_kernel_ptr_sets<4>(nw);
+    switch (nw) {
+        case 4: return reinterpret_cast<const void*>(sweep_reg_kernel<RG_NUL, 4, 1>);
+        case 6: return reinterpret_cast<const void*>(sweep_reg_kernel<RG_NUL, 6, 1>);
+        case 8: return reinterpret_cast<const void*>(sweep_reg_kernel<RG_NUL, 8, 1>);
+        case 10: return reinterpret_cast<const void*>(sweep_reg_kernel<RG_NUL, 10, 1>);
+        default: return reinterpret_cast<const void*>(sweep_reg_kernel<RG_NUL, 12, 1>);
     }
 }
 void reg_set_attributes() {
     static PerDeviceOnce attr_once;
     if (attr_once.first())
-        for (int nw : RG_WAVES) HIP_CHECK(hipFuncSetAttribute(reg_kernel_ptr(nw), hipFuncAttributeMaxDynamicSharedMemorySize, 150 * 1024));
+        for (int ns : RG_SETS)
+            for (int nw : RG_WAVES)
+                if (reg_has_kernel(nw, ns)) HIP_CHECK(hipFuncSetAttribute(reg_kernel_ptr(nw, ns), hipFuncAttributeMaxDynamicSharedMemorySize, 150 * 1024));
 }
 int reg_nwg(int D, int nw) { return (int)ceil_div(D, 32 * nw); }
-int reg_occupancy(int nw) {
+int reg_occupancy(int nw, int ns = 1) {
     static std::mutex mu;
     static std::map<std::pair<int, int>, int> cache;
     int dev = 0;
     HIP_CHECK(hipGetDevice(&dev));
     std::lock_guard<std::mutex> lk(mu);
-    auto it = cache.find({dev, nw});
+    auto it = cache.find({dev, 16 * ns + nw});
     if (it != cache.end()) return it->second;
     reg_set_attributes();
     int nb = 0;
-    if (hipOccupancyMaxActiveBlocksPerMultiprocessor(&nb, reg_kernel_ptr(nw), 64 * nw, reg_dyn_bytes(RG_NUL, nw)) != hipSuccess) { (void)hipGetLastError(); nb = 0; }
-    cache[{dev, nw}] = nb;
+    if (hipOccupancyMaxActiveBlocksPerMultiprocessor(&nb, reg_kernel_ptr(nw, ns), 64 * nw, reg_dyn_bytes(RG_NUL, nw)) != hipSuccess) { (void)hipGetLastError(); nb = 0; }
+    cache[{dev, 16 * ns + nw}] = nb;
     return nb;
 }
 int reg_wg_cost(int nw) { return nw == 4 ? 1 : 3; }
 
-}
+int occ_of(const RegSweepEnv& e, int nw, int ns) {
+    for (int i = 0; i < RG_NST; ++i)
+        for (int j = 0; j < RG_NWV; ++j) if (RG_SETS[i] == ns && RG_WAVES[j] == nw) return e.occ[i][j];
+    return 0;
+}
+int pick_waves(const RegSweepEnv& e, int D, int ndesigns) {
+    if (ndesigns < 1 || ndesigns > REG_SWEEP_MAX) return 0;
+    const int nsub = (int)ceil_div(ndesigns, 8), cus = e.cus / 8;
+    if (const int nw = e.waves) {
+        if ((nw == 4 || nw == 6 || nw == 8 || nw == 10 || nw == 12) && nsub * reg_nwg(D, nw) * reg_wg_cost(nw) <= 3 * cus && occ_of(e, nw, 1) >= (nw == 4 ? 3 : 1)) return nw;
+    }
+    for (int nw : RG_WAVES) if (nsub * reg_nwg(D, nw) <= cus && occ_of(e, nw, 1) >= 1) return nw;
+    return (nsub * reg_nwg(D, 4) <= 3 * cus && occ_of(e, 4, 1) >= 3) ? 4 : 0;
+}
+int spread_waves(const RegSweepEnv& e, int D, int ndesigns) {
+    const int mode = e.spread;
+    if (mode == 0 || ndesigns < 1 || ndesigns > REG_SWEEP_MAX || e.waves != 0) return 0;
+    const int cus = e.cus, local = pick_waves(e, D, ndesigns);
+    for (int nw : RG_WAVES)
+        if (ndesigns * reg_nwg(D, nw) <= cus && occ_of(e, nw, 1) >= 1) return (mode == 1 || local == 0 || nw < local) ? nw : 0;
+    return 0;
+}
+int pick_waves_sets(const RegSweepEnv& e, int D, int ndesigns, int ns) {
+    const int nsub = (int)ceil_div(ceil_div(ndesigns, ns), 8), cus = e.cus / 8;
+    int nw = e.waves;
+    if (!nw) { nw = spread_waves(e, D, ndesigns); if (!nw) nw = pick_waves(e, D, ndesigns); }
+    return (reg_has_kernel(nw, ns) && nsub * reg_nwg(D, nw) * reg_wg_cost(nw) <= 3 * cus && occ_of(e, nw, ns) >= (nw == 4 ? 3 : 1)) ? nw : 0;
+}
+RegSweepEnv reg_env() {
+    static std::mutex mu;
+    static std::map<int, RegSweepEnv> per_device;
+    int dev = 0;
+    HIP_CHECK(hipGetDevice(&dev));
+    RegSweepEnv e{};
+    {
+        std::unique_lock<std::mutex> lk(mu);
+        auto it = per_device.find(dev);
+        if (it == per_device.end()) {
+            lk.unlock();
+            for (int i = 0; i < RG_NST; ++i)
+                for (int j = 0; j < RG_NWV; ++j) e.occ[i][j] = reg_has_kernel(RG_WAVES[j], RG_SETS[i]) ? reg_occupancy(RG_WAVES[j], RG_SETS[i]) : 0;
+            lk.lock();
+            per_device[dev] = e;
+        } else e = it->second;
+    }
+    e.cus = sweep_cu_budget();
+    e.waves = sw_int<Sw::REG_WAVES>(); e.spread = sw_int<Sw::REG_SPREAD>(); e.sets = sw_int<Sw::REG_SETS>();
+    return e;
+}
+
+}
+
+RegSweepForm reg_sweep_layout(const RegSweepEnv& e, int D, int n, int hint) {
+    RegSweepForm f{};
+    if (n < 1 || n > REG_SWEEP_MAX || D < 1) return f;
+    if (hint >= 1) {
+        const int want = (e.sets == 1 || e.sets == 2 || e.sets == 4) ? e.sets : (hint >= 4 ? 4 : hint >= 2 ? 2 : 1);
+        for (int ns = want; ns > 1; ns /= 2) {
+            const int groups = (int)ceil_div(n, ns);
+            const int nw = pick_waves_sets(e, D, n, ns);
+            if (!nw || (e.sets == 0 && nw != 12)) continue;
+            f.ns = ns; f.nw = nw; f.spread = 0; f.groups = groups; f.nwg = reg_nwg(D, nw);
+            f.wg_per_xcd = (int)ceil_div(groups, 8) * f.nwg;
+            f.blocks = 8 * f.wg_per_xcd;
+            f.gate = f.wg_per_xcd * reg_wg_cost(nw);
+            return f;
+        }
+    }
+    const int sp = spread_waves(e, D, n);
+    const int nw = sp ? sp : pick_waves(e, D, n);
+    if (!nw) return f;
+    f.ns = 1; f.nw = nw; f.spread = sp ? 1 : 0; f.groups = n; f.nwg = reg_nwg(D, nw);
+    f.wg_per_xcd = sp ? (int)ceil_div((int64_t)n * f.nwg, 8) : (int)ceil_div(n, 8) * f.nwg;
+    f.blocks = sp ? n * f.nwg : 8 * f.wg_per_xcd;
+    f.gate = f.wg_per_xcd * reg_wg_cost(nw);
+    return f;
+}
+RegSweepForm reg_sweep_form(int D, int n, int hint) { return reg_sweep_layout(reg_env(), D, n, hint); }
 
 int reg_sweep_max_units() { return 2 * RG_NUL; }
 bool reg_sweep_supported(int D, int nmics, int nunits, int nOrd) {
@@ -487,28 +605,9 @@
     return sizeof(u64) * ((size_t)2 * nwg * RG_NEX * 2 + nwg + 64);
 }
 int reg_sweep_slots_per_xcd() { return 3 * (sweep_cu_budget() / 8); }
-int reg_sweep_pick_waves(int D, int ndesigns) {
-    if (ndesigns < 1 || ndesigns > REG_SWEEP_MAX) return 0;
-    const int nsub = (int)ceil_div(ndesigns, 8), cus = sweep_cu_budget() / 8;
-    if (const int nw = sw_int<Sw::REG_WAVES>()) {
-        if ((nw == 4 || nw == 6 || nw == 8 || nw == 10 || nw == 12) && nsub * reg_nwg(D, nw) * reg_wg_cost(nw) <= 3 * cus && reg_occupancy(nw) >= (nw == 4 ? 3 : 1)) return nw;
-    }
-    for (int nw : RG_WAVES) if (nsub * reg_nwg(D, nw) <= cus && reg_occupancy(nw) >= 1) return nw;
-    return (nsub * reg_nwg(D, 4) <= 3 * cus && reg_occupancy(4) >= 3) ? 4 : 0;
-}
-int reg_sweep_spread_waves(int D, int ndesigns) {
-    const int mode = sw_int<Sw::REG_SPREAD>();
-    if (mode == 0 || ndesigns < 1 || ndesigns > REG_SWEEP_MAX || sw_int<Sw::REG_WAVES>() != 0) return 0;
-    const int cus = sweep_cu_budget(), local = reg_sweep_pick_waves(D, ndesigns);
-    for (int nw : RG_WAVES)
-        if (ndesigns * reg_nwg(D, nw) <= cus && reg_occupancy(nw) >= 1) return (mode == 1 || local == 0 || nw < local) ? nw : 0;
-    return 0;
-}
-int reg_sweep_gate_cost(int D, int ndesigns) {
-    if (const int ns = reg_sweep_spread_waves(D, ndesigns)) return (int)ceil_div((int64_t)ndesigns * reg_nwg(D, ns), 8) * reg_wg_cost(ns);
-    const int nw = reg_sweep_pick_waves(D, ndesigns);
-    return nw ? (int)ceil_div(ndesigns, 8) * reg_nwg(D, nw) * reg_wg_cost(nw) : 0;
-}
+int reg_sweep_pick_waves(int D, int ndesigns) { return pick_waves(reg_env(), D, ndesigns); }
+int reg_sweep_spread_waves(int D, int ndesigns) { return spread_waves(reg_env(), D, ndesigns); }
+int reg_sweep_gate_cost(int D, int ndesigns, int hint) { return reg_sweep_form(D, ndesigns, hint).gate; }
 int reg_sweep_capacity(int D) {
     int n = 0;
     for (int k = 8; k <= REG_SWEEP_MAX; k += 8) if (reg_sweep_pick_waves(D, k)) n = k;
@@ -518,24 +617,39 @@
     return reg_sweep_supported(D, nmics, nunits, nOrd) && reg_sweep_pick_waves(D, ndesigns) != 0;
 }
 
-void launch_sweep_reg(const HalfSweepArgs* args_dev, const HalfSweepArgs& a0, int n, hipStream_t st) {
-    const int ns = reg_sweep_spread_waves(a0.D, n);
-    const int nw = ns ? ns : reg_sweep_pick_waves(a0.D, n);
+namespace {
+std::atomic<long long> g_reg_launches[3];
+template <int NS> void launch_reg_sets(int nw, unsigned nblocks, size_t dyn, hipStream_t st, const HalfSweepArgs* args_dev, int n, int nWG, int spread, int prio) {
+    switch (nw) {
+        case 4: sweep_reg_kernel<RG_NUL, 4, NS><<<dim3(nblocks), 256, dyn, st>>>(args_dev, n, nWG, spread, prio); break;
+        case 8: sweep_reg_kernel<RG_NUL, 8, NS><<<dim3(nblocks), 512, dyn, st>>>(args_dev, n, nWG, spread, prio); break;
+        default: sweep_reg_kernel<RG_NUL, 12, NS><<<dim3(nblocks), 768, dyn, st>>>(args_dev, n, nWG, spread, prio); break;
+    }
+}
+}
+
+void launch_sweep_reg(const HalfSweepArgs* args_dev, const HalfSweepArgs& a0, int n, hipStream_t st, int hint) {
+    const RegSweepForm f = reg_sweep_form(a0.D, n, hint);
+    const int nw = f.nw;
     if (!nw) throw Error(2, "register-resident sweep: the launch cannot be resident");
-    const int nWG = reg_nwg(a0.D, nw), spread = ns ? 1 : 0;
-    const unsigned nblocks = spread ? (unsigned)(n * nWG) : 8u * (unsigned)nWG * (unsigned)ceil_div(n, 8);
+    const int nWG = f.nwg, spread = f.spread;
+    const unsigned nblocks = (unsigned)f.blocks;
     const size_t dyn = reg_dyn_bytes(RG_NUL, nw);
     reg_set_attributes();
     const int prio = sw_int<Sw::REG_PRIO>();
-    switch (nw) {
-        case 4: sweep_reg_kernel<RG_NUL, 4><<<dim3(nblocks), 256, dyn, st>>>(args_dev, n, nWG, spread, prio); break;
-        case 6: sweep_reg_kernel<RG_NUL, 6><<<dim3(nblocks), 384, dyn, st>>>(args_dev, n, nWG, spread, prio); break;
-        case 8: sweep_reg_kernel<RG_NUL, 8><<<dim3(nblocks), 512, dyn, st>>>(args_dev, n, nWG, spread, prio); break;
-        case 10: sweep_reg_kernel<RG_NUL, 10><<<dim3(nblocks), 640, dyn, st>>>(args_dev, n, nWG, spread, prio); break;
-        default: sweep_reg_kernel<RG_NUL, 12><<<dim3(nblocks), 768, dyn, st>>>(args_dev, n, nWG, spread, prio); break;
+    if (f.ns == 4) launch_reg_sets<4>(nw, nblocks, dyn, st, args_dev, n, nWG, spread, prio);
+    else if (f.ns == 2) launch_reg_sets<2>(nw, nblocks, dyn, st, args_dev, n, nWG, spread, prio);
+    else switch (nw) {
+        case 4: sweep_reg_kernel<RG_NUL, 4, 1><<<dim3(nblocks), 256, dyn, st>>>(args_dev, n, nWG, spread, prio); break;
+        case 6: sweep_reg_kernel<RG_NUL, 6, 1><<<dim3(nblocks), 384, dyn, st>>>(args_dev, n, nWG, spread, prio); break;
+        case 8: sweep_reg_kernel<RG_NUL, 8, 1><<<dim3(nblocks), 512, dyn, st>>>(args_dev, n, nWG, spread, prio); break;
+        case 10: sweep_reg_kernel<RG_NUL, 10, 1><<<dim3(nblocks), 640, dyn, st>>>(args_dev, n, nWG, spread, prio); break;
+        default: sweep_reg_kernel<RG_NUL, 12, 1><<<dim3(nblocks), 768, dyn, st>>>(args_dev, n, nWG, spread, prio); break;
     }
     KERNEL_CHECK();
-}
+    g_reg_launches[f.ns == 4 ? 2 : f.ns == 2 ? 1 : 0].fetch_add(1, std::memory_order_relaxed);
+}
+void reg_sweep_launch_counts(long long (&out)[3]) { for (int i = 0; i < 3; ++i) out[i] = g_reg_launches[i].load(std::memory_order_relaxed); }
 
 double reg_contract_selftest() {
     constexpr int ND = 32, NU = 2 * RG_NUL, NO = 8 * NU;
diff --git a/emagls_amd/csrc/switches.hpp b/emagls_amd/csrc/switches.hpp
--- a/emagls_amd/csrc/switches.hpp
+++ b/emagls_amd/csrc/switches.hpp
@@ -30,7 +30,8 @@
     X(SWEEP_REG,         INT,  1,     0, 2,         CALL,    "register-resident sweep: 0 never (the slab form), 1 for launches of more than 8 designs, 2 always") \
     X(REG_WAVES,         INT,  0,     INT_MIN, INT_MAX, CALL, "waves per workgroup of the register-resident sweep (4, 6, 8, 10, 12 whenever it fits; 0: the smallest count with which every workgroup owns a CU)") \
     X(REG_SPREAD,        INT,  2,     0, 2,         CALL,    "a launch's designs spread over all XCDs: 0 never, 1 whenever it fits, 2 when it needs fewer waves per workgroup than the one-XCD layout") \
-    X(REG_PRIO,          INT,  1,     INT_MIN, INT_MAX, PROCESS, "=0: the register-resident sweep's waves at the default issue priority") \
+    X(REG_SETS,          INT,  0,     0, 4,         CALL,    "HRIR sets of one geometry per group of workgroups of the register-resident sweep (1, 2, 4; 0: by the chunks the list keeps in flight)") \
+    X(REG_PRIO,         INT,  1,     INT_MIN, INT_MAX, PROCESS, "=0: the register-resident sweep's waves at the default issue priority") \
     X(SWEEP_FETCH,       INT,  0,     0, 4,         PROCESS, "where the persistent sweep requests the next bin's operands") \
     X(SWEEP_WAIT_MS,     INT,  20,    1, INT_MAX,   PROCESS, "wall-clock limit of a wait for peers inside a resident sweep, in ms") \
     X(SWEEP_TIMING,      ON1,  0,     0, 1,         CALL,    "=1: in-kernel wall-clock stamps of the persistent sweep (when a plan is created)") \
diff --git a/include/emagls.h b/include/emagls.h
--- a/include/emagls.h
+++ b/include/emagls.h
@@ -347,6 +347,8 @@
 int emagls_plan_get_filters(emagls_plan* plan, void* wL, void* wR);
 int emagls_plan_get_info(emagls_plan* plan, emagls_plan_info* info);
 int emagls_plan_sweep_form_in_batch(emagls_plan* plan, int designs, int* form);
+int emagls_reg_sweep_layout(int ndirs, int designs, int hint, int sets, int waves, int spread, int cus, int wg_per_cu_four, int wg_per_cu_large, int* out);
+int emagls_reg_sweep_launch_counts(long long* counts);
 int emagls_plan_set_streams(emagls_plan* plan, int nstreams);
 int emagls_plan_set_profiling(emagls_plan* plan, int level);
 int emagls_plan_num_stages(emagls_plan* plan);
```

Result: slower. 3881 filter sets/s (-1.3%).
